# cvYouTian/Dedark-YOLO

Hardware: AMD Instinct MI355X
Metric: training img/s at 640x640 (higher is better)
Workload: dtype bf16

## Files before the change

dedark_yolo_amd/_C.py:

```python
import ctypes as C
import os

_HERE = os.path.dirname(os.path.abspath(__file__))
LIB_PATH = os.path.join(os.environ.get("DY_LIB_DIR") or os.path.join(_HERE, "lib"), "libdedark_yolo.so")

DY_F32, DY_BF16, DY_F16 = 0, 1, 2
ACT_NONE, ACT_SILU, ACT_LEAKY = 0, 1, 2
OPT_RULES = dict(Adam=0, Adamax=1, NAdam=2, RAdam=3, RMSProp=4)
STATS_REPLICAS = 64
BN_BWD_REPLICAS = 8

vp, i32, i64, f32, f64 = C.c_void_p, C.c_int, C.c_int64, C.c_float, C.c_double


class ConvDesc(C.Structure):
    _fields_ = [("src", vp), ("src_ld", i64), ("N", i32), ("Hs", i32), ("Ws", i32), ("Cs", i32), ("w", vp), ("dst", vp),
                ("dst_ld", i64), ("Hd", i32), ("Wd", i32), ("Cd", i32), ("KH", i32), ("KW", i32), ("stride", i32),
                ("pad", i32), ("dil", i32), ("scale", vp), ("shift", vp), ("act", i32), ("stats", vp), ("accumulate", i32),
                ("dtype", i32), ("dst_row_stride", i64), ("dst_img_stride", i64), ("KHf", i32), ("KWf", i32), ("kh0", i32),
                ("kh_step", i32), ("kw0", i32), ("kw_step", i32), ("dst_valid_channels", i32), ("dst_planar", vp),
                ("add_src", vp), ("add_src_ld", i64)]


class PackItem(C.Structure):
    _fields_ = [("w", vp), ("packed", vp), ("Cout", i32), ("Cout_pad", i32), ("Cin", i32), ("Cin_pad", i32), ("KH", i32),
                ("KW", i32), ("transposed", i32), ("dtype", i32), ("first_block", i64)]


class DetMaps(C.Structure):
    _fields_ = [("map", vp * 3), ("map_ld", i64 * 3), ("h", i32 * 3), ("w", i32 * 3), ("stride", f32 * 3), ("B", i32),
                ("nc", i32), ("n_levels", i32), ("dtype", i32)]


class DetMaps4(DetMaps):
    _fields_ = [("map3", vp), ("map_ld3", i64), ("h3", i32), ("w3", i32), ("stride3", f32)]


class AugSample(C.Structure):
    _fields_ = [("src", vp * 4), ("sh", i32 * 4), ("sw", i32 * 4), ("pitch", i64 * 4), ("rect", (i32 * 6) * 4), ("n_src", i32),
                ("canvas_h", i32), ("canvas_w", i32), ("hsv", i32), ("flipud", i32), ("fliplr", i32), ("minv", C.c_double * 6),
                ("lut", (C.c_uint8 * 256) * 3)]


class AugMixSample(C.Structure):
    _fields_ = [("a", AugSample), ("b", AugSample), ("r", C.c_double), ("r1", C.c_double), ("mix", i32)]


class SegDesc(C.Structure):
    _fields_ = [("mc", vp), ("mc_ld", i64), ("proto", vp), ("proto_ld", i64), ("B", i32), ("A", i32), ("nm", i32), ("mh", i32),
                ("mw", i32), ("target_gt_idx", vp), ("fg_mask", vp), ("target_box", vp), ("masks", vp), ("mask_dtype", i32),
                ("mask_h", i32), ("mask_w", i32), ("overlap", i32), ("gt_rows", vp), ("n_max", i32), ("img_h", f32), ("img_w", f32),
                ("pos", vp), ("npos", vp), ("dtype", i32)]


BIAS_GRAD_CHUNKS = 2048
LN_MAX_C = 2048
LN_MAX_PARTS = 512

POSE_MAX_LEVELS = 4


class PoseDesc(C.Structure):
    _fields_ = [("kpt", vp * POSE_MAX_LEVELS), ("kpt_ld", i64 * POSE_MAX_LEVELS), ("h", i32 * POSE_MAX_LEVELS), ("w", i32 * POSE_MAX_LEVELS),
                ("stride", f32 * POSE_MAX_LEVELS), ("n_levels", i32), ("B", i32), ("A", i32), ("K", i32), ("ndim", i32), ("dtype", i32),
                ("target_gt_idx", vp), ("fg_mask", vp), ("target_box", vp), ("keypoints", vp), ("n_targets", i32), ("gt_rows", vp),
                ("n_max", i32), ("img_h", f32), ("img_w", f32), ("sigma", vp), ("pos", vp), ("npos", vp)]


_SIGS = {
    "dy_version": [],
    "dy_frontend_init": [],
    "dy_conv2d_fwd": [C.POINTER(ConvDesc), vp],
    "dy_conv2d_dgrad": [C.POINTER(ConvDesc), vp],
    "dy_conv2d_wgrad": [vp, i64, i32, i32, i32, i32, vp, i64, i32, i32, i32, i32, i32, i32, i32, i32, i32, i32, vp, i64, vp,
                        i32, vp],
    "dy_conv2d_wgrad_forked": [vp, vp, i64, i32, i32, i32, i32, vp, i64, i32, i32, i32, i32, i32, i32, i32, i32, i32, i32, vp, i64,
                               vp, i32, vp],
    "dy_conv2d_bn_act_fwd": [C.POINTER(ConvDesc), i64, vp, vp, vp, vp, f32, f32, vp, i32, vp, i64, vp, i64, vp],
    "dy_bn_act_bwd": [vp, i64, vp, i64, vp, vp, i32, vp, vp, i64, vp, vp, i64, i32, i32, vp],
    "dy_conv2d_bn_act_fwd_valid": [C.POINTER(ConvDesc), i64, vp, vp, vp, vp, f32, f32, vp, i32, vp, i64, vp, i64, i32, vp],
    "dy_bn_act_bwd_valid": [vp, i64, vp, i64, vp, vp, i32, vp, vp, i64, vp, vp, i64, i32, i32, i32, vp],
    "dy_pack_weight": [vp, vp, i32, i32, i32, i32, i32, i32, i32, i32, vp],
    "dy_pack_item_blocks": [i32, i32, i32, i32],
    "dy_pack_weights_multi": [vp, i32, i64, vp],
    "dy_bn_finalize": [vp, i64, vp, vp, vp, vp, f32, f32, vp, vp, vp, vp, i32, vp],
    "dy_bn_fold_eval": [vp, vp, vp, vp, f32, vp, vp, i32, vp],
    "dy_bn_finalize_valid": [vp, i64, vp, vp, vp, vp, f32, f32, vp, vp, vp, vp, i32, i32, vp],
    "dy_bn_fold_eval_valid": [vp, vp, vp, vp, f32, vp, vp, i32, i32, vp],
    "dy_bn_act_fwd": [vp, i64, vp, vp, i32, vp, i64, vp, i64, i64, i32, i32, vp],
    "dy_bn_act_bwd_reduce": [vp, i64, vp, i64, vp, vp, vp, vp, i32, i32, vp, i64, i32, i32, vp],
    "dy_bn_act_bwd_apply": [vp, i64, vp, i64, vp, vp, vp, vp, vp, i32, i32, vp, vp, i64, vp, vp, i64, i32, i32, vp],
    "dy_bn_act_bwd_apply_valid": [vp, i64, vp, i64, vp, vp, vp, vp, vp, i32, i32, vp, vp, i64, vp, vp, i64, i32, i32, i32, vp],
    "dy_bn2_act_fwd": [vp, i64, vp, i64, vp, vp, vp, vp, i32, vp, i64, i64, i32, i32, vp],
    "dy_bn2_act_bwd_workspace": [i64, i32, i32],
    "dy_bn2_act_bwd": [vp, i64, vp, i64, vp, i64, vp, vp, vp, vp, vp, vp, vp, vp, vp, vp, i32, vp, i64, vp, i64, vp, vp, vp, vp, vp, i64,
                       i64, i32, i32, vp],
    "dy_maxpool_fwd": [vp, i64, vp, i64, vp, i32, i32, i32, i32, i32, i32, i32, i32, i32, i32, vp],
    "dy_maxpool_bwd": [vp, i64, vp, vp, i64, i32, i32, i32, i32, i32, i32, i32, i32, i32, i32, i32, vp],
    "dy_upsample_nearest_fwd": [vp, i64, vp, i64, i32, i32, i32, i32, i32, i32, vp],
    "dy_upsample_nearest_bwd": [vp, i64, vp, i64, i32, i32, i32, i32, i32, i32, i32, vp],
    "dy_copy2d": [vp, i64, vp, i64, i64, i32, i32, i32, vp],
    "dy_cast": [vp, i32, vp, i32, i64, vp],
    "dy_pconv_pack": [vp, vp, i32, i32, i32, vp],
    "dy_pconv_fwd": [vp, i64, vp, i64, vp, vp, i32, i32, i32, i32, i32, i32, vp],
    "dy_pconv_dgrad": [vp, i64, vp, i64, vp, vp, i32, i32, i32, i32, i32, i32, vp, i64, i32, vp],
    "dy_pconv_wgrad": [vp, i64, vp, i64, vp, i32, i32, i32, i32, vp, i64, i32, vp],
    "dy_dwconv_fwd": [vp, i64, vp, i64, vp, i32, i32, i32, i32, i32, i32, vp, vp, i32, vp, i32, i32, vp],
    "dy_dwconv_dgrad": [vp, i64, vp, i64, vp, i32, i32, i32, i32, i32, i32, i32, vp, i64, i32, vp],
    "dy_dwconv_wgrad": [vp, i64, vp, i64, vp, i32, i32, i32, i32, i32, i32, vp, i64, i32, vp],
    "dy_copy2d_exact": [vp, i64, vp, i64, i64, i32, i32, i32, vp],
    "dy_asff_fuse_fwd": [vp, i64, vp, i64, vp, i64, vp, i64, vp, i64, i64, i32, i32, vp],
    "dy_asff_fuse_bwd": [vp, i64, vp, i64, vp, i64, vp, i64, vp, i64, vp, i64, vp, i64, vp, i64, vp, i64, i64, i32, i32, i32,
                         i32, i32, vp],
    "dy_image_to_nhwc8": [vp, i32, i32, i32, vp, i32, i32, i32, vp],
    "dy_resize_bwd": [vp, i32, i32, i32, i32, i32, i32, vp, vp],
    "dy_filter_params_fwd": [vp, i32, vp, i32, vp],
    "dy_filter_params_bwd": [vp, i32, vp, vp, i32, vp],
    "dy_filters_pointwise_fwd": [vp, vp, vp, vp, vp, i32, i32, i32, i32, vp],
    "dy_filters_pointwise_bwd": [vp, vp, vp, vp, vp, vp, vp, i32, i32, i32, i32, i32, vp],
    "dy_usm_fwd": [vp, vp, vp, vp, vp, i32, i32, i32, i32, vp],
    "dy_usm_bwd": [vp, vp, i32, vp, vp, vp, vp, i32, i32, i32, i32, vp],
    "dy_loss_prepare_targets": [vp, vp, vp, i32, i32, i32, f32, f32, vp, vp, vp],
    "dy_loss_decode": [C.POINTER(DetMaps), vp, vp],
    "dy_tal_assign": [C.POINTER(DetMaps), vp, vp, vp, i32, vp, vp, vp, vp, vp, vp, vp, vp, vp],
    "dy_tal_assign_decoded": [vp, vp, vp, vp, vp, i32, i32, i32, i32, vp, vp, vp, vp, vp, vp, vp, vp, vp],
    "dy_chan_moments": [vp, i64, i32, i64, i32, vp, i32, vp],
    "dy_sru_fwd": [vp, i64, vp, i64, i32, i64, i32, i32, vp, vp, vp, f32, i32, vp],
    "dy_sru_bwd": [vp, i64, vp, i64, vp, i64, i32, i64, i32, i32, vp, vp, vp, f32, vp, i32, vp],
    "dy_cru_fuse_fwd": [vp, i64, vp, i64, i32, i64, i32, vp, i32, vp],
    "dy_cru_fuse_bwd": [vp, i64, vp, i64, vp, i64, i32, i64, i32, vp, vp, i32, vp],
    "dy_cru_conv_pack": [vp, vp, vp, i32, i32, i32, i32, i32, i32, vp],
    "dy_cru_conv_fwd": [vp, i64, vp, vp, vp, i64, i32, i32, i32, i32, i32, i32, i32, i32, vp],
    "dy_cru_conv_dgrad": [vp, i64, vp, vp, i64, i32, i32, i32, i32, i32, i32, i32, i32, i32, vp],
    "dy_cru_conv_wgrad": [vp, i64, vp, i64, vp, vp, vp, i32, i32, i32, i32, i32, i32, i32, vp, i64, i32, vp],
    "dy_attn_fwd": [vp, i64, vp, i64, vp, i64, vp, i64, vp, i32, i32, i32, i32, f32, i32, vp],
    "dy_attn_bwd": [vp, i64, vp, i64, vp, i64, vp, i64, vp, i64, vp, vp, i64, vp, i64, vp, i64, i32, i32, i32, i32, f32, i32, vp],
    "dy_add_layernorm_fwd": [vp, i64, vp, i64, vp, vp, vp, i64, vp, i64, i32, f32, i32, vp],
    "dy_add_layernorm_bwd": [vp, i64, vp, i64, vp, vp, vp, i64, vp, i64, i32, vp, vp, vp, i64, i64, i32, i32, vp],
    "dy_gelu_fwd": [vp, i64, vp, i64, i64, i32, i32, vp],
    "dy_gelu_bwd": [vp, i64, vp, i64, vp, i64, i64, i32, i32, vp],
    "dy_add_pos": [vp, i64, vp, vp, i64, i32, i32, i32, i32, vp],
    "dy_bbox_ciou": [vp, vp, i64, vp, vp, vp],
    "dy_bbox_iou": [vp, vp, i64, i32, i32, f32, vp, vp, vp],
    "dy_aug_resize_u8": [vp, i32, i32, i64, vp, i32, i32, i64, vp],
    "dy_aug_resize_area_u8": [vp, i32, i32, i64, vp, i32, i32, i64, vp],
    "dy_aug_letterbox": [vp, i32, i32, i64, i32, i32, i32, i32, i32, i32, vp, vp],
    "dy_aug_mosaic_warp": [vp, i32, i32, i32, vp, vp],
    "dy_aug_mosaic_warp_mix": [vp, i32, i32, i32, vp, vp],
    "dy_dark_channel_prior": [vp, i32, i32, i32, vp, vp, vp],
    "dy_dfl_loss": [vp, vp, i64, vp, vp, vp],
    "dy_loss_fwd": [C.POINTER(DetMaps), vp, vp, vp, vp, vp, vp, vp],
    "dy_loss_finish": [vp, vp, f32, f32, f32, f32, i32, vp, vp, vp],
    "dy_loss_bwd": [C.POINTER(DetMaps), C.POINTER(vp), C.POINTER(i64), vp, vp, vp, vp, vp, vp, vp, f32, f32, f32, vp],
    "dy_detect_decode": [C.POINTER(DetMaps), vp, vp],
    "dy_detect_decode_rows": [C.POINTER(DetMaps), vp, i32, vp],
    "dy_detect_decode_tta": [C.POINTER(DetMaps), vp, i64, i32, i32, i32, f32, i32, f32, f32, vp],
    "dy_tta_scale_img": [vp, i32, i32, i32, i32, i32, i32, i32, i32, i32, vp, vp],
    "dy_nms_candidates": [vp, i32, i32, i32, f32, i32, vp, vp, i64, vp],
    "dy_nms_sort": [vp, vp, vp, i32, i64, vp, vp, vp],
    "dy_nms_greedy": [vp, vp, vp, i32, i32, i32, i64, C.c_double, i32, i32, f32, i32, vp, vp, vp, vp, vp, vp],
    "dy_preprocess_batch": [vp, vp, vp, f32, i32, i32, vp, i64, vp],
    "dy_sumsq": [vp, i64, vp, vp],
    "dy_sgd_step": [vp, vp, vp, vp, vp, f32, f32, f32, f32, f32, f32, f32, i32, f32, vp, f32, f32, i64, vp],
    "dy_sgd_step_scaled": [vp, vp, vp, vp, vp, f32, f32, f32, f32, f32, f32, f32, i32, f32, vp, f32, f32, vp, i64, vp],
    "dy_adamw_step_scaled": [vp, vp, vp, vp, vp, vp, f32, f32, f32, f32, f32, f32, f32, f32, f32, i32, f32, vp, f32, f32, vp, i64, vp],
    "dy_loss_scale_update": [vp, vp, f32, f32, i32, vp],
    "dy_optim_step": [i32, vp, vp, vp, vp, vp, vp, f32, f32, f32, f32, f32, f32, f64, f64, f64, f64, f32, vp, f32, f32, vp, vp, i64, vp],
    "dy_adamw_step": [vp, vp, vp, vp, vp, vp, f32, f32, f32, f32, f32, f32, f32, f32, f32, i32, f32, vp, f32, f32, i64, vp],
    "dy_ema_lerp": [vp, vp, f32, i64, vp],
    "dy_grad_accumulate": [vp, vp, i64, vp],
    "dy_stream_fork": [vp, vp],
    "dy_seg_positives": [vp, i32, i32, vp, vp, vp],
    "dy_seg_gt_rows": [vp, i32, i32, i32, vp, vp],
    "dy_seg_loss_fwd": [C.POINTER(SegDesc), f32, vp, vp, vp, vp],
    "dy_seg_loss_bwd": [C.POINTER(SegDesc), vp, f32, vp, i64, vp, i64, vp],
    "dy_bias_add": [vp, i64, vp, i64, i32, i32, vp],
    "dy_bias_grad": [vp, i64, i64, i32, i32, vp, i64, vp, vp],
    "dy_seg_mask_decode": [vp, i64, i32, i32, i32, vp, i64, vp, i32, f32, f32, i32, vp, vp],
    "dy_seg_crop_mask": [vp, vp, i32, i32, i32, vp],
    "dy_seg_mask_iou": [vp, i32, vp, i32, i32, i32, i64, vp, vp, vp],
    "dy_seg_mask_upsample": [vp, i64, i32, i32, i32, i32, vp, i64, vp, vp, i32, i32, i32, i32, f32, f32, i32, i32, i32, i32, i32, i32, i32,
                             vp, vp],
    "dy_mask_resize": [vp, i32, i32, i32, i32, i32, i32, i32, i32, vp, i32, i32, i32, vp],
    "dy_pose_loss_fwd": [C.POINTER(PoseDesc), f32, f32, vp, vp, vp, vp],
    "dy_pose_loss_bwd": [C.POINTER(PoseDesc), vp, vp, f32, f32, C.POINTER(vp), i64, vp],
    "dy_pose_kpt_decode": [C.POINTER(PoseDesc), i32, vp, vp],
    "dy_kpt_oks": [vp, i32, vp, i32, i32, vp, vp, i32, f32, vp, vp],
    "dy_polymask_raster": [vp, i32, i32, i32, i32, i32, vp, vp, vp],
    "dy_polymask_compose": [vp, vp, vp, i32, i32, i32, i32, vp, vp, vp, vp, vp],
    "dy_gap_fwd": [vp, i64, i32, i32, i32, i32, vp, i64, vp],
    "dy_gap_bwd": [vp, i64, i32, i32, i32, i32, vp, i64, vp],
    "dy_cls_xent_fwd": [vp, i64, i32, vp, i32, i32, vp, vp, vp],
    "dy_cls_xent_bwd": [vp, i64, i32, vp, vp, vp, i32, i32, vp, i64, vp],
    "dy_cls_softmax": [vp, i64, i32, i32, i32, vp, vp],
    "dy_cls_topk": [vp, i64, i32, i32, i32, i32, vp, vp],
    "dy_cls_metrics_update": [vp, i32, vp, i32, i32, vp, vp, vp],
    "dy_val_box_match": [vp, i32, vp, i32, i32, vp, vp, vp, i32, i32, i32, vp, vp, i32, i32, f32, f32, i32, vp, vp, vp, vp, vp, vp],
    "dy_val_iou_match": [vp, i64, vp, vp, i32, vp, i32, i32, vp, vp, i32, vp, i32, i32, vp, vp, vp],
}

_lib = None


def lib():
    global _lib
    if _lib is None:
        if not os.path.exists(LIB_PATH):
            raise RuntimeError(f"dedark_yolo_amd: HIP library not built: {LIB_PATH} (run __graft_entry__.build()); "
                               "there is no CPU fallback")
        L = C.CDLL(LIB_PATH)
        L.dy_last_error.restype = C.c_char_p
        L.dy_last_error.argtypes = []
        L.dy_last_kernel.restype = C.c_char_p
        L.dy_last_kernel.argtypes = []
        L.dy_clear_last_kernel.restype = None
        L.dy_clear_last_kernel.argtypes = []
        for name, sig in _SIGS.items():
            fn = getattr(L, name)
            fn.argtypes = sig
            fn.restype = C.c_int64 if name in ("dy_pack_item_blocks", "dy_bn2_act_bwd_workspace") else C.c_int
        _lib = L
    return _lib


def exported_symbols():
    return ["dy_last_error", "dy_last_kernel", "dy_clear_last_kernel"] + list(_SIGS)


_prof = None
_next_meta = None
_UNTIMED = frozenset(["dy_stream_fork"])


def call(name, *args):
    global _next_meta
    L = lib()
    if _prof is None or name in _UNTIMED:
        rc = getattr(L, name)(*args)
    else:
        import torch
        e0, e1 = torch.cuda.Event(enable_timing=True), torch.cuda.Event(enable_timing=True)
        L.dy_clear_last_kernel()
        e0.record()
        rc = getattr(L, name)(*args)
        e1.record()
        kern = L.dy_last_kernel().decode()
        _prof.append((name, e0, e1, _next_meta, kern))
        _next_meta = None
    if rc != 0:
        raise RuntimeError(f"{name} failed (rc={rc}): {L.dy_last_error().decode()}")


def set_meta(**kw):
    global _next_meta
    if _prof is not None:
        _next_meta = kw
```

dedark_yolo_amd/csrc/conv.hip:

```cpp
#include <stdlib.h>
#include "dy_host.h"
#include "conv_epilogue.h"
#include "../../include/dedark_yolo.h"
#include "conv_route.h"

namespace {

constexpr int ROWB = 144;
constexpr int NTHREADS = 256;

struct ConvP {
  const char* src;
  long src_ld;
  int N, Hs, Ws, Cs;
  const char* w;
  char* dst;
  long dst_ld;
  int Hd, Wd, Cd;
  int KH, KW, stride, pad, dil;
  const float* scale;
  const float* shift;
  int act;
  double* stats;
  int accumulate;
// ... 696 lines not shown
    if (!it.transposed) {
      const int co = co0 + a, ci = ci0 + g * VE;
#pragma unroll
      for (int e = 0; e < 8; ++e) v[e] = e < VE ? tile[a][(g * VE + e) * PACK_TAPS + t] : 0.f;
      ok = co < it.Cout_pad && ci < it.Cin_pad;
      o = ((long)co * T + t0 + t) * it.Cin_pad + ci;
    } else {
      const int ci = ci0 + a, co = co0 + g * VE;
#pragma unroll
      for (int e = 0; e < 8; ++e) v[e] = e < VE ? tile[g * VE + e][a * PACK_TAPS + t] : 0.f;
      ok = co < it.Cout_pad && ci < it.Cin_pad;
      o = ((long)ci * T + t0 + t) * it.Cout_pad + co;
    }
    if (!ok) continue;
    if (it.dtype == DY_F32) stvec<float>((float*)it.packed + o, v);
    else if (it.dtype == DY_F16) stvec<f16_t>((f16_t*)it.packed + o, v);
    else stvec<bf16_t>((bf16_t*)it.packed + o, v);
  }
  __syncthreads();
}

__global__ __launch_bounds__(256) void pack_multi_kernel(const dy_pack_item* __restrict__ items, int n_items) {
  __shared__ float tile[PACK_TILE][PACK_TILE * PACK_TAPS + 1];
  __shared__ long fb[1024];
  const long b = blockIdx.x;
  const bool cached = n_items <= 1024;
  if (cached) {
    for (int i = threadIdx.x; i < n_items; i += 256) fb[i] = items[i].first_block;
    __syncthreads();
  }
  int lo = 0, hi = n_items - 1;
  while (lo < hi) {
    const int mid = (lo + hi + 1) >> 1;
    if ((cached ? fb[mid] : items[mid].first_block) <= b) lo = mid; else hi = mid - 1;
  }
  const dy_pack_item it = items[lo];
  const int tiles_ci = (it.Cin_pad + PACK_TILE - 1) / PACK_TILE;
  const int tb = (int)(b - it.first_block);
  const int co0 = (tb / tiles_ci) * PACK_TILE, ci0 = (tb % tiles_ci) * PACK_TILE;
  const int T = it.KH * it.KW;
  if (T == 9) pack_chunk<9>(it, tile, co0, ci0, 9, 0, 9);
  else if (T == 1) pack_chunk<1>(it, tile, co0, ci0, 1, 0, 1);
  else
    for (int t0 = 0; t0 < T; t0 += PACK_TAPS) pack_chunk<0>(it, tile, co0, ci0, T, t0, T - t0 < PACK_TAPS ? T - t0 : PACK_TAPS);
}

template <typename T, int MODE>
int launch_conv(const dy_conv_desc* d, hipStream_t st, const dy_conv_desc* classes, int ncls) {
  ConvP p;
  dy_route::fill_parity_classes(p, classes, ncls);
  dy_route::fill_gather(p, d);
  constexpr int BM = 128;
  const int tiles_m = dy_cdiv(p.M, BM);
  auto blocks = [&](int bn) {
    p.tiles_n = dy_cdiv(d->Cd, bn);
    p.nblk = tiles_m * p.tiles_n;
    if (p.ncls > 1) p.nblk = dy_route::number_parity_blocks(p, BM, dy_route::CLS_SEQUENTIAL);
  };
  dy_note_kernel(d->Cd <= 32 ? "conv_igemm_kernel<BN=32>" : (d->Cd <= 64 ? "conv_igemm_kernel<BN=64>" : "conv_igemm_kernel<BN=128>"));
  if (d->Cd <= 32) {
    blocks(32);
    conv_igemm_kernel<T, BM, 32, 4, 1, MODE><<<p.nblk, NTHREADS, 0, st>>>(p);
  } else if (d->Cd <= 64) {
    blocks(64);
    conv_igemm_kernel<T, BM, 64, 2, 2, MODE><<<p.nblk, NTHREADS, 0, st>>>(p);
  } else {
    blocks(128);
    conv_igemm_kernel<T, BM, 128, 2, 2, MODE><<<p.nblk, NTHREADS, 0, st>>>(p);
  }
  DY_LAUNCH_CHECK();
  return 0;
}

bool thin_eligible(const dy_conv_desc* d, int mode, bool parity_class = false) {
  static const bool off = dy_env("DY_NO_CONV_THIN") != nullptr;
  static const bool all_shapes = getenv("DY_CONV_THIN_ALL") != nullptr;
  if (off || d->dtype != DY_BF16) return false;
  if (!all_shapes && !parity_class && !(d->Cs == 16 && d->KH * d->KW > 1)) return false;
  if (!(d->Cs == 16 || d->Cs == 32 || d->Cs == 48) || d->Cd > 32 || d->Cd % 8 != 0) return false;
  if (d->KH > 3 || d->KW > 3 || d->dil != 1 || (mode == 1 && d->stride != 1)) return false;
  if ((d->src_ld * 2) % 16 != 0 || (d->dst_ld * 2) % 16 != 0 || (long)d->N * d->Hd * d->Wd < 1024) return false;
  return true;
}

int launch_thin(const dy_conv_desc* d, int mode, hipStream_t st, const dy_conv_desc* classes = nullptr, int ncls = 0) {
  ConvP p;
  dy_route::fill_parity_classes(p, classes, ncls);
  dy_route::fill_gather(p, d);
  p.tiles_n = 1;
  p.nblk = dy_cdiv(p.M, THIN_BM);
  if (p.ncls > 1) p.nblk = dy_route::number_parity_blocks(p, THIN_BM, dy_route::CLS_SEQUENTIAL);
  dy_note_kernel("conv_thin_kernel");
#define THIN(C_, M_) conv_thin_kernel<C_, M_><<<p.nblk, NTHREADS, 0, st>>>(p)
  const int c16 = d->Cs / 16;
  if (mode == 0) { if (c16 == 1) THIN(1, 0); else if (c16 == 2) THIN(2, 0); else THIN(3, 0); }
  else { if (c16 == 1) THIN(1, 1); else if (c16 == 2) THIN(2, 1); else THIN(3, 1); }
#undef THIN
  DY_LAUNCH_CHECK();
  return 0;
}

int launch_generic(const dy_conv_desc* d, int mode, hipStream_t st, const dy_conv_desc* classes = nullptr, int ncls = 0) {
  if (mode == 0)
    return d->dtype == DY_F32 ? launch_conv<float, 0>(d, st, classes, ncls)
                              : (d->dtype == DY_F16 ? launch_conv<f16_t, 0>(d, st, classes, ncls) : launch_conv<bf16_t, 0>(d, st, classes, ncls));
  return d->dtype == DY_F32 ? launch_conv<float, 1>(d, st, classes, ncls)
                            : (d->dtype == DY_F16 ? launch_conv<f16_t, 1>(d, st, classes, ncls) : launch_conv<bf16_t, 1>(d, st, classes, ncls));
}

int check_conv(const dy_conv_desc* d, const char* who) {
  DY_CHECK(d && d->src && d->w && (d->dst || d->dst_planar), "%s: null pointer", who);
  DY_CHECK(d->dtype == DY_F32 || d->dtype == DY_BF16 || d->dtype == DY_F16, "%s: bad dtype %d", who, d->dtype);
  const int ve = d->dtype == DY_F32 ? 4 : 8, es = d->dtype == DY_F32 ? 4 : 2;
  DY_CHECK(d->Cs > 0 && d->Cs % ve == 0, "%s: Cs=%d must be a positive multiple of %d", who, d->Cs, ve);
  DY_CHECK(d->src_ld >= d->Cs && (d->src_ld * es) % 16 == 0, "%s: src_ld=%ld not 16-byte aligned", who, (long)d->src_ld);
  DY_CHECK(((uintptr_t)d->src) % 16 == 0 && ((uintptr_t)d->w) % 16 == 0, "%s: src/w pointer not 16-byte aligned", who);
  DY_CHECK(d->dst_ld >= d->Cd && d->Cd > 0, "%s: dst_ld=%ld < Cd=%d", who, (long)d->dst_ld, d->Cd);
  DY_CHECK(d->N > 0 && d->Hs > 0 && d->Ws > 0 && d->Hd > 0 && d->Wd > 0, "%s: empty geometry", who);
  DY_CHECK(d->KH > 0 && d->KW > 0 && d->stride > 0 && d->dil > 0 && d->pad >= 0, "%s: bad window", who);
  DY_CHECK(d->act >= 0 && d->act <= 2, "%s: bad act", who);
  return 0;
}

enum : unsigned {
  SITE_FWD = 1,
  SITE_DGRAD_HEAD = 2,
  SITE_DGRAD = 4,
  SITE_CLASS = 8,
};

struct Route {
  bool (*eligible)(const dy_conv_desc* d, int mode);
  int (*launch)(const dy_conv_desc* d, int mode, void* stream);
  unsigned sites;
  bool fuses_add;
};

const Route kRoutes[] = {
    {dy_dense_fwd_eligible, dy_dense_fwd_launch, SITE_FWD, false},
    {dy_conv_stem_fwd_eligible, dy_conv_stem_fwd_launch, SITE_FWD, false},
    {dy_dense_dgrad_eligible, dy_dense_dgrad_launch, SITE_DGRAD_HEAD, false},
    {dy_conv_small_dgrad_eligible, dy_conv_small_dgrad_launch, SITE_DGRAD_HEAD, false},
    {dy_conv_px_eligible, dy_conv_px_launch, SITE_FWD | SITE_DGRAD, true},
    {dy_conv_v4_eligible, dy_conv_v4_launch, SITE_FWD | SITE_DGRAD | SITE_CLASS, true},
    {dy_conv_v5_eligible, dy_conv_v5_launch, SITE_FWD | SITE_DGRAD | SITE_CLASS, true},
    {dy_conv_v3_eligible, dy_conv_v3_launch, SITE_FWD | SITE_DGRAD, false},
    {dy_conv_v2_eligible, dy_conv_v2_launch, SITE_FWD | SITE_DGRAD | SITE_CLASS, false},
    {[](const dy_conv_desc* d, int mode) { return thin_eligible(d, mode); },
     [](const dy_conv_desc* d, int mode, void* stream) { return launch_thin(d, mode, (hipStream_t)stream); }, SITE_FWD | SITE_DGRAD, false},
    {[](const dy_conv_desc*, int) { return true; },
     [](const dy_conv_desc* d, int mode, void* stream) { return launch_generic(d, mode, (hipStream_t)stream); },
     SITE_FWD | SITE_DGRAD | SITE_CLASS, false},
};

const Route* pick_route(const dy_conv_desc* d, unsigned site) {
  const int mode = (site & (SITE_DGRAD_HEAD | SITE_DGRAD)) ? 1 : 0;
  for (const Route& r : kRoutes)
    if ((r.sites & site) && r.eligible(d, mode)) return &r;
  return nullptr;
}

}

extern "C" int dy_conv2d_fwd(const dy_conv_desc* d, void* stream) {
  if (int e = check_conv(d, "dy_conv2d_fwd")) return e;
  const int ho = (d->Hs + 2 * d->pad - d->dil * (d->KH - 1) - 1) / d->stride + 1;
  const int wo = (d->Ws + 2 * d->pad - d->dil * (d->KW - 1) - 1) / d->stride + 1;
  DY_CHECK(ho == d->Hd && wo == d->Wd, "dy_conv2d_fwd: dst %dx%d does not match conv output %dx%d", d->Hd, d->Wd, ho, wo);
  return pick_route(d, SITE_FWD)->launch(d, 0, stream);
}

static int dgrad_dispatch(const dy_conv_desc* d, void* stream, bool* added) {
  if (int e = check_conv(d, "dy_conv2d_dgrad")) return e;
  const int ho = (d->Hd + 2 * d->pad - d->dil * (d->KH - 1) - 1) / d->stride + 1;
  const int wo = (d->Wd + 2 * d->pad - d->dil * (d->KW - 1) - 1) / d->stride + 1;
  DY_CHECK(ho == d->Hs && wo == d->Ws, "dy_conv2d_dgrad: dz %dx%d does not match conv output %dx%d", d->Hs, d->Ws, ho, wo);
  DY_CHECK(d->stats == nullptr, "dy_conv2d_dgrad: stats unsupported");
  DY_CHECK(d->KHf == 0 && d->dst_row_stride == 0, "dy_conv2d_dgrad: tap subsets / strided destinations are forward-only");
  if (const Route* r = pick_route(d, SITE_DGRAD_HEAD)) return r->launch(d, 1, stream);
  DY_CHECK(d->dst_planar == nullptr, "dy_conv2d_dgrad: dst_planar is only supported by the direct stem kernel (bf16, 3x3 s2 p1, Cd == 8)");
  static const bool no_parity = dy_env("DY_NO_PARITY_DGRAD") != nullptr;
  if (d->stride == 2 && d->dil == 1 && !no_parity) {
    dy_conv_desc c[4];
    int nc = 0;
    bool ok = true;
    for (int ph = 0; ph < 2 && ok; ++ph)
      for (int pw = 0; pw < 2 && ok; ++pw) {
        int geo[2][4];
        for (int ax = 0; ax < 2; ++ax) {
          const int par = ax == 0 ? ph : pw, K = ax == 0 ? d->KH : d->KW, ext = ax == 0 ? d->Hd : d->Wd;
          const int first = (par + d->pad) & 1;
          const int n = first < K ? (K - 1 - first) / 2 + 1 : 0;
          const int last = first + 2 * (n - 1);
          const int omin = (par + d->pad - last) / 2;
          geo[ax][0] = n; geo[ax][1] = last; geo[ax][2] = -omin; geo[ax][3] = (ext - par + 1) / 2;
        }
        if (geo[0][3] <= 0 || geo[1][3] <= 0) continue;
        if (geo[0][0] == 0 || geo[1][0] == 0 || geo[0][2] != geo[1][2] || geo[0][2] < 0) { ok = false; break; }
        dy_conv_desc& q = c[nc++];
        q = *d;
        const long es = d->dtype == DY_F32 ? 4 : 2;
        q.dst = (char*)d->dst + ((long)ph * d->Wd + pw) * d->dst_ld * es;
        q.dst_ld = 2 * d->dst_ld;
        q.dst_row_stride = 2L * d->Wd * d->dst_ld;
        q.dst_img_stride = (long)d->Hd * d->Wd * d->dst_ld;
        q.Hd = geo[0][3]; q.Wd = geo[1][3];
        q.KHf = d->KH; q.KWf = d->KW;
        q.KH = geo[0][0]; q.KW = geo[1][0];
        q.kh0 = geo[0][1]; q.kh_step = -2; q.kw0 = geo[1][1]; q.kw_step = -2;
        q.stride = 1; q.pad = geo[0][2];
      }
    if (ok) {
      static const bool multi = !(dy_env("DY_PARITY_MULTI") && atoi(dy_env("DY_PARITY_MULTI")) == 0);
      if (multi && nc > 1) {
        dy_conv_desc r[4];
        bool all_v2 = true, none_v2 = true;
        for (int i = 0; i < nc; ++i) {
          r[i] = c[nc - 1 - i];
          const bool e2 = dy_conv_v2_eligible(&r[i], 0);
          all_v2 = all_v2 && e2;
          none_v2 = none_v2 && !e2;
        }
        const long class_tiles = dy_cdiv((long)r[0].N * r[0].Hd * r[0].Wd, 256);
        if (dy_conv_v4_classes_eligible(r, nc)) return dy_conv_v4_launch_classes(r, nc, stream);
        if (dy_conv_v5_classes_eligible(r, nc)) return dy_conv_v5_launch_classes(r, nc, stream);
        if (all_v2 && class_tiles <= 256) return dy_conv_v2_launch_classes(r, nc, stream);
        if (none_v2) {
          bool thin = true;
          for (int i = 0; i < nc; ++i) thin = thin && thin_eligible(&r[i], 0, true);
          if (thin) return launch_thin(&r[0], 0, (hipStream_t)stream, r, nc);
          if (class_tiles <= 256) return launch_generic(&r[0], 0, (hipStream_t)stream, r, nc);
        }
      }
      for (int i = nc - 1; i >= 0; --i) {
        if (int e = pick_route(&c[i], SITE_CLASS)->launch(&c[i], 0, stream)) return e;
      }
      return 0;
    }
  }
  const Route* r = pick_route(d, SITE_DGRAD);
  *added = r->fuses_add;
  return r->launch(d, 1, stream);
}

extern "C" int dy_conv2d_dgrad(const dy_conv_desc* d, void* stream) {
  bool added = false;
  if (int e = dgrad_dispatch(d, stream, &added)) return e;
  if (d->add_src && !added) {
    DY_CHECK(d->dst && d->dst_planar == nullptr, "dy_conv2d_dgrad: add_src needs an NHWC destination");
    return dy_copy2d(d->add_src, d->add_src_ld, d->dst, d->dst_ld, (int64_t)d->N * d->Hd * d->Wd, d->Cd, 1, d->dtype, stream);
  }
  return 0;
}

namespace {
template <typename T>
int launch_wgrad(const DyWgradArgs& a, hipStream_t st) {
  WgP p;
  dy_route::fill_wgrad_problem(p, a);
  constexpr int MK = 8 * DT<T>::VE;
  int bm, bn;
  bn = p.Ktot <= 32 ? 32 : (p.Ktot <= 64 ? 64 : 128);
  if (bn == 32) bm = 128;
  else if (bn == 64) bm = p.Cout <= 64 ? 64 : 128;
  else bm = p.Cout <= 32 ? 32 : (p.Cout <= 64 ? 64 : 128);
  const int tiles_c = dy_cdiv(p.Cout, bm);
  p.tiles_k = dy_cdiv(p.Ktot, bn);
  const int tiles = tiles_c * p.tiles_k;
  p.tiles = tiles;
  static const int env_blocks = dy_env("DY_WGRAD_BLOCKS") ? atoi(dy_env("DY_WGRAD_BLOCKS")) : 0;
  static const int env_steps = dy_env("DY_WGRAD_STEPS") ? atoi(dy_env("DY_WGRAD_STEPS")) : 0;
  const long fit = a.scratch_elems / ((long)tiles * bm * bn);
  DY_CHECK(fit >= 1, "dy_conv2d_wgrad: scratch too small (%ld floats, need %ld)", a.scratch_elems, (long)tiles * bm * bn);
  const long want = ((env_blocks > 0 ? env_blocks : 2048) + tiles - 1) / tiles;
  const dy_route::WgradSplits plan =
      dy_route::plan_wgrad_splits(p.M, want, (long)(env_steps > 0 ? env_steps : 4) * MK, MK, fit, dy_route::kGridDimYCap);
  p.chunk = plan.chunk;
  dim3 grid(tiles, (unsigned)plan.splits);
  dy_note_kernel("conv_wgrad_kernel+wgrad_reduce_kernel");
#define WG(BM_, BN_, WM_, WN_) conv_wgrad_kernel<T, BM_, BN_, WM_, WN_><<<grid, NTHREADS, 0, st>>>(p)
  if (bm == 128 && bn == 128) WG(128, 128, 2, 2);
  else if (bm == 64 && bn == 128) WG(64, 128, 1, 4);
  else if (bm == 32 && bn == 128) WG(32, 128, 1, 4);
  else if (bm == 128 && bn == 64) WG(128, 64, 4, 1);
  else if (bm == 64 && bn == 64) WG(64, 64, 2, 2);
  else WG(128, 32, 4, 1);
#undef WG
  DY_LAUNCH_CHECK();
  wgrad_reduce_kernel<<<dim3(a.Cout, dy_cdiv(p.Ktot, 32)), 256, 0, st>>>(a.scratch, (int)plan.splits, tiles, p.tiles_k, bm, bn, a.Cin, p.Cin,
                                                                         p.KH, p.KW, p.Ktot, a.g_oihw);
  DY_LAUNCH_CHECK();
  return 0;
}

int wgrad_generic(const DyWgradArgs& a, void* stream) {
  int rc = 0;
  DY_DISPATCH_DTYPE("dy_conv2d_wgrad", a.dtype, rc = launch_wgrad<T>(a, (hipStream_t)stream));
  return rc;
}

struct WgradRoute {
  bool (*eligible)(const DyWgradArgs& a);
  int (*launch)(const DyWgradArgs& a, void* stream);
};

const WgradRoute kWgradRoutes[] = {
    {dy_dense_wgrad_eligible, dy_dense_wgrad_launch},
    {dy_wgrad_v3_eligible, dy_wgrad_v3_launch},
    {dy_wgrad_v4_eligible, dy_wgrad_v4_launch},
    {dy_wgrad_v2_eligible, dy_wgrad_v2_launch},
    {[](const DyWgradArgs&) { return true; }, wgrad_generic},
};
}

int dy_wgrad_reduce_co_slabs(const float* part, int splits, const DyCoSlabs& L, int Cout, int Cin, float* g_oihw, void* stream) {
  wgrad_reduce_co_kernel<<<dim3(dy_cdiv(Cout, 32), L.KH * L.KW * L.Cin_pad), 256, 0, (hipStream_t)stream>>>(
      part, splits, L.co_tile, L.k_tile, L.Cin_pad, L.KH, L.KW, Cout, Cin, L.co_stride, L.k_stride, L.split_stride, g_oihw);
  DY_LAUNCH_CHECK();
  return 0;
}

extern "C" int dy_conv2d_wgrad(const void* x, int64_t x_ld, int N, int Hi, int Wi, int Cin_pad, const void* dz, int64_t dz_ld,
                               int Ho, int Wo, int Cout_pad, int KH, int KW, int stride, int pad, int dil, int Cout, int Cin,
                               float* scratch, int64_t scratch_elems, float* g_oihw, int dtype, void* stream) {
  DY_CHECK(x && dz && scratch && g_oihw, "dy_conv2d_wgrad: null pointer");
  DY_CHECK(dtype == DY_F32 || dtype == DY_BF16 || dtype == DY_F16, "dy_conv2d_wgrad: bad dtype");
  const int ve = dtype == DY_F32 ? 4 : 8, es = dtype == DY_F32 ? 4 : 2;
  DY_CHECK(Cin_pad % ve == 0 && Cout_pad % ve == 0, "dy_conv2d_wgrad: Cin=%d / Cout=%d must be multiples of %d", Cin_pad, Cout_pad, ve);
  DY_CHECK(Cout > 0 && Cout <= Cout_pad && Cin > 0 && Cin <= Cin_pad, "dy_conv2d_wgrad: bad real channel counts");
  DY_CHECK((x_ld * es) % 16 == 0 && (dz_ld * es) % 16 == 0, "dy_conv2d_wgrad: ld not 16-byte aligned");
  DY_CHECK(((uintptr_t)x) % 16 == 0 && ((uintptr_t)dz) % 16 == 0, "dy_conv2d_wgrad: pointer not 16-byte aligned");
  const int ho = (Hi + 2 * pad - dil * (KH - 1) - 1) / stride + 1, wo = (Wi + 2 * pad - dil * (KW - 1) - 1) / stride + 1;
  DY_CHECK(ho == Ho && wo == Wo, "dy_conv2d_wgrad: dz %dx%d does not match conv output %dx%d", Ho, Wo, ho, wo);
  const DyWgradArgs a = {x, x_ld, N, Hi, Wi, Cin_pad, dz, dz_ld, Ho, Wo, Cout_pad, KH, KW, stride, pad, dil, Cout, Cin,
                         scratch, scratch_elems, g_oihw, dtype};
  for (const WgradRoute& r : kWgradRoutes)
    if (r.eligible(a)) return r.launch(a, stream);
  return 0;
}

extern "C" int dy_pack_weight(const float* w, void* packed, int Cout, int Cout_pad, int Cin, int Cin_pad, int KH, int KW,
                              int transposed, int dtype, void* stream) {
  DY_CHECK(w && packed && Cin_pad >= Cin && Cout_pad >= Cout, "dy_pack_weight: bad args");
  long total = (long)Cout_pad * KH * KW * Cin_pad;
  int blocks = (int)((total + 255) / 256);
  if (blocks > 4096) blocks = 4096;
  hipStream_t st = (hipStream_t)stream;
  DY_DISPATCH_DTYPE("dy_pack_weight", dtype,
                    pack_weight_kernel<T><<<blocks, 256, 0, st>>>(w, (T*)packed, Cout, Cout_pad, Cin, Cin_pad, KH, KW, transposed));
  DY_LAUNCH_CHECK();
  return 0;
}

extern "C" int64_t dy_pack_item_blocks(int Cout_pad, int Cin_pad, int KH, int KW) {
  (void)KH; (void)KW;
  return (int64_t)((Cout_pad + PACK_TILE - 1) / PACK_TILE) * ((Cin_pad + PACK_TILE - 1) / PACK_TILE);
}

extern "C" int dy_pack_weights_multi(const dy_pack_item* items_dev, int n_items, int64_t n_blocks, void* stream) {
  DY_CHECK(items_dev && n_items > 0 && n_blocks > 0 && n_blocks < (1LL << 31), "dy_pack_weights_multi: bad args");
  pack_multi_kernel<<<(unsigned)n_blocks, 256, 0, (hipStream_t)stream>>>(items_dev, n_items);
  DY_LAUNCH_CHECK();
  return 0;
}

extern "C" int dy_conv2d_bn_act_fwd_valid(const dy_conv_desc* d, int64_t count, const float* gamma, const float* beta,
                                          float* running_mean, float* running_var, float momentum, float eps, float* aff, int act,
                                          const void* residual, int64_t res_ld, void* y, int64_t y_ld, int C_valid, void* stream) {
  DY_CHECK(d && d->stats && d->dst && aff, "dy_conv2d_bn_act_fwd: needs a raw-output buffer, statistics and the affine buffer");
  DY_CHECK(C_valid > 0 && C_valid <= d->Cd, "dy_conv2d_bn_act_fwd: C_valid=%d outside 1..Cd=%d", C_valid, d->Cd);
  if (int e = dy_conv2d_fwd(d, stream)) return e;
  const int C = d->Cd;
  if (int e = dy_bn_finalize_valid(d->stats, count, gamma, beta, running_mean, running_var, momentum, eps, aff, aff + C, aff + 2 * C,
                                   aff + 3 * C, C, C_valid, stream))
    return e;
  return dy_bn_act_fwd(d->dst, d->dst_ld, aff, aff + C, act, residual, res_ld, y, y_ld, (int64_t)d->N * d->Hd * d->Wd, C, d->dtype, stream);
}

extern "C" int dy_conv2d_bn_act_fwd(const dy_conv_desc* d, int64_t count, const float* gamma, const float* beta, float* running_mean,
                                    float* running_var, float momentum, float eps, float* aff, int act, const void* residual,
                                    int64_t res_ld, void* y, int64_t y_ld, void* stream) {
  DY_CHECK(d, "dy_conv2d_bn_act_fwd: null descriptor");
  return dy_conv2d_bn_act_fwd_valid(d, count, gamma, beta, running_mean, running_var, momentum, eps, aff, act, residual, res_ld, y, y_ld,
                                    d->Cd, stream);
}

extern "C" int dy_conv2d_wgrad_forked(void* wait_for, const void* x, int64_t x_ld, int N, int Hi, int Wi, int Cin_pad, const void* dz,
                                      int64_t dz_ld, int Ho, int Wo, int Cout_pad, int KH, int KW, int stride, int pad, int dil,
                                      int Cout, int Cin, float* scratch, int64_t scratch_elems, float* g_oihw, int dtype,
                                      void* stream) {
  if (wait_for != stream)
    if (int e = dy_stream_fork(wait_for, stream)) return e;
  return dy_conv2d_wgrad(x, x_ld, N, Hi, Wi, Cin_pad, dz, dz_ld, Ho, Wo, Cout_pad, KH, KW, stride, pad, dil, Cout, Cin, scratch,
                         scratch_elems, g_oihw, dtype, stream);
}
```

dedark_yolo_amd/csrc/conv_route.h:

```cpp
#pragma once
#include <type_traits>
#include <utility>
#include "dy_common.h"
#include "../../include/dedark_yolo.h"

namespace dy_route {

__device__ inline int xcd_remap(int bid, int nblk) {
  int q = nblk >> 3, r = nblk & 7, x = bid & 7;
  int base = (x < r) ? x * (q + 1) : r * (q + 1) + (x - r) * q;
  return base + (bid >> 3);
}

template <typename P>
__device__ inline long dst_offset(const P& p, long m) {
  if (p.dst_row == 0) return m * p.dst_ld;
  const long HWd = (long)p.Hd * p.Wd;
  const long img = m / HWd;
  const int rem = (int)(m - img * HWd);
  const int oh = rem / p.Wd, ow = rem - oh * p.Wd;
  return img * p.dst_img + (long)oh * p.dst_row + (long)ow * p.dst_ld;
}

template <typename P>
inline void fill_weight_taps(P& p, const dy_conv_desc* d) {
  if (d->KHf > 0) {
    p.kh0 = d->kh0; p.khs = d->kh_step; p.kw0 = d->kw0; p.kws = d->kw_step; p.KWf = d->KWf;
    p.w_row = (long)d->KHf * d->KWf * d->Cs;
  } else {
    p.kh0 = 0; p.khs = 1; p.kw0 = 0; p.kws = 1; p.KWf = d->KW;
    p.w_row = (long)d->KH * d->KW * d->Cs;
  }
}

template <typename P>
inline void fill_dst_strides(P& p, const dy_conv_desc* d) {
  p.dst_row = d->dst_row_stride;
  p.dst_img = d->dst_img_stride ? d->dst_img_stride : (long)d->Hd * d->dst_row_stride;
}

template <typename P>
inline void fill_gather(P& p, const dy_conv_desc* d) {
  p.src = (const char*)d->src; p.src_ld = d->src_ld; p.N = d->N; p.Hs = d->Hs; p.Ws = d->Ws; p.Cs = d->Cs;
  p.w = (const char*)d->w; p.dst = (char*)d->dst; p.dst_ld = d->dst_ld; p.Hd = d->Hd; p.Wd = d->Wd; p.Cd = d->Cd;
  p.KH = d->KH; p.KW = d->KW; p.stride = d->stride; p.pad = d->pad; p.dil = d->dil;
  p.scale = d->scale; p.shift = d->shift; p.act = d->act; p.stats = d->stats; p.accumulate = d->accumulate;
  p.M = (long)d->N * d->Hd * d->Wd;
  p.Ktot = d->KH * d->KW * d->Cs;
  static const int ablate = dy_env("DY_ABLATE") ? atoi(dy_env("DY_ABLATE")) : 0;
  p.ablate = ablate;
  fill_dst_strides(p, d);
  fill_weight_taps(p, d);
}

template <typename P>
inline void fill_taps_extents(P& p, const dy_conv_desc* d, int mode) {
  p.src = (const char*)d->src; p.w = (const char*)d->w; p.dst = (char*)d->dst;
  p.src_ld = d->src_ld; p.dst_ld = d->dst_ld;
  p.src_bytes = (unsigned)((((long)d->N * d->Hs * d->Ws - 1) * d->src_ld + d->Cs) * 2);
  p.Hs = d->Hs; p.Ws = d->Ws; p.Cs = d->Cs; p.Hd = d->Hd; p.Wd = d->Wd; p.Cd = d->Cd;
  p.KH = d->KH; p.KW = d->KW;
  if (mode == 0) {
    p.stride = d->stride; p.dh0 = -d->pad; p.dhs = d->dil; p.dw0 = -d->pad; p.dws = d->dil;
  } else {
    p.stride = 1; p.dh0 = d->pad; p.dhs = -d->dil; p.dw0 = d->pad; p.dws = -d->dil;
  }
  fill_weight_taps(p, d);
  p.w_bytes = (unsigned)((long)d->Cd * p.w_row * 2);
  {
    const int dh_lo = p.dhs < 0 ? p.dh0 + p.dhs * (p.KH - 1) : p.dh0, dw_lo = p.dws < 0 ? p.dw0 + p.dws * (p.KW - 1) : p.dw0;
    const long lo = ((long)dh_lo * p.Ws + dw_lo) * p.src_ld * 2;
    p.a_min = lo < 0 ? (int)lo : 0;
  }
  p.scale = d->scale; p.shift = d->shift; p.act = d->act; p.stats = d->stats; p.accumulate = d->accumulate;
  if ((long)d->N * d->Hd * d->Wd * d->Cd * 2 > (128L << 20)) p.accumulate |= 2;
  p.M = (long)d->N * d->Hd * d->Wd;
  p.add_src = mode == 1 ? (const char*)d->add_src : nullptr; p.add_src_ld = d->add_src_ld;
  fill_dst_strides(p, d);
}

template <typename P>
inline void fill_parity_classes(P& p, const dy_conv_desc* classes, int ncls) {
  p.ncls = ncls > 1 ? ncls : 0;
  for (int c = 0; c < p.ncls; ++c) {
    const dy_conv_desc& q = classes[c];
    DyParityCls& k = p.cls[c];
    k.dst = (char*)q.dst; k.M = (long)q.N * q.Hd * q.Wd; k.Hd = q.Hd; k.Wd = q.Wd; k.KH = q.KH; k.KW = q.KW; k.pad = q.pad;
    k.kh0 = q.kh0; k.kw0 = q.kw0; k.Ktot = q.KH * q.KW * q.Cs; k.blk0 = 0; k._r = 0;
  }
}

enum ClsOrder { CLS_SEQUENTIAL, CLS_XCD_SLOTS };
template <typename P>
inline int number_parity_blocks(P& p, int bm, ClsOrder order) {
  int next = 0;
  for (int c = 0; c < p.ncls; ++c) {
    DyParityCls& k = p.cls[c];
    const int tiles = dy_cdiv(k.M, bm) * p.tiles_n;
    k.blk0 = next;
    k._r = order == CLS_XCD_SLOTS ? dy_cdiv(tiles, 8) : 0;
    next += order == CLS_XCD_SLOTS ? k._r : tiles;
  }
  return order == CLS_XCD_SLOTS ? 8 * next : next;
}

inline bool dma_extents_ok(const dy_conv_desc* d, int KH, int KW, int dil) {
  const long src_bytes = (((long)d->N * d->Hs * d->Ws - 1) * d->src_ld + d->Cs) * 2;
  const long w_row = d->KHf > 0 ? (long)d->KHf * d->KWf * d->Cs : (long)d->KH * d->KW * d->Cs;
  const long w_bytes = (long)d->Cd * w_row * 2;
  const long halo = ((long)KH * dil * d->Ws + (long)KW * dil) * d->src_ld * 2;
  return src_bytes + halo <= 0x7fffffffL && w_bytes <= 0x3fffffffL;
}

inline bool parity_classes_uniform(const dy_conv_desc* c, int ncls) {
  const dy_conv_desc* d = &c[0];
  for (int i = 0; i < ncls; ++i) {
    const dy_conv_desc& q = c[i];
    if (q.src != d->src || q.w != d->w || q.Cs != d->Cs || q.Cd != d->Cd || q.dtype != d->dtype || q.stride != 1 || q.dil != 1 || q.KHf != d->KHf ||
        q.KWf != d->KWf || q.kh_step != d->kh_step || q.kw_step != d->kw_step || q.dst_ld != d->dst_ld || q.dst_row_stride != d->dst_row_stride ||
        q.dst_img_stride != d->dst_img_stride || q.src_ld != d->src_ld || q.accumulate != d->accumulate || q.scale || q.shift || q.stats ||
        q.act != DY_ACT_NONE)
      return false;
    if ((q.dst_ld * 2) % 16 != 0 || ((uintptr_t)q.dst) % 16 != 0 || (q.src_ld * 2) % 16 != 0) return false;
  }
  return true;
}

}

bool dy_dense_fwd_eligible(const dy_conv_desc* d, int mode);
int dy_dense_fwd_launch(const dy_conv_desc* d, int mode, void* stream);
bool dy_dense_dgrad_eligible(const dy_conv_desc* d, int mode);
int dy_dense_dgrad_launch(const dy_conv_desc* d, int mode, void* stream);
bool dy_conv_stem_fwd_eligible(const dy_conv_desc* d, int mode);
int dy_conv_stem_fwd_launch(const dy_conv_desc* d, int mode, void* stream);
bool dy_conv_small_dgrad_eligible(const dy_conv_desc* d, int mode);
int dy_conv_small_dgrad_launch(const dy_conv_desc* d, int mode, void* stream);
bool dy_conv_px_eligible(const dy_conv_desc* d, int mode);
int dy_conv_px_launch(const dy_conv_desc* d, int mode, void* stream);
bool dy_conv_v4_eligible(const dy_conv_desc* d, int mode);
int dy_conv_v4_launch(const dy_conv_desc* d, int mode, void* stream);
bool dy_conv_v4_classes_eligible(const dy_conv_desc* classes, int ncls);
int dy_conv_v4_launch_classes(const dy_conv_desc* classes, int ncls, void* stream);
bool dy_conv_v5_eligible(const dy_conv_desc* d, int mode);
int dy_conv_v5_launch(const dy_conv_desc* d, int mode, void* stream);
bool dy_conv_v5_classes_eligible(const dy_conv_desc* classes, int ncls);
int dy_conv_v5_launch_classes(const dy_conv_desc* classes, int ncls, void* stream);
bool dy_conv_v3_eligible(const dy_conv_desc* d, int mode);
int dy_conv_v3_launch(const dy_conv_desc* d, int mode, void* stream);
bool dy_conv_v2_eligible(const dy_conv_desc* d, int mode);
int dy_conv_v2_launch(const dy_conv_desc* d, int mode, void* stream);
int dy_conv_v2_launch_classes(const dy_conv_desc* classes, int ncls, void* stream);
bool dy_conv_prefers_256(const dy_conv_desc* d);

struct DyWgradArgs {
  const void* x;
  long x_ld;
  int N, Hi, Wi, Cin_pad;
  const void* dz;
  long dz_ld;
  int Ho, Wo, Cout_pad, KH, KW, stride, pad, dil, Cout, Cin;
  float* scratch;
  long scratch_elems;
  float* g_oihw;
  int dtype;
};

namespace dy_route {

template <typename P, typename = void> struct HasPointwise : std::false_type {};
template <typename P> struct HasPointwise<P, std::void_t<decltype(std::declval<P&>().pointwise)>> : std::true_type {};

template <typename P>
inline void fill_wgrad_problem(P& p, const DyWgradArgs& a) {
  p.x = (const char*)a.x; p.x_ld = a.x_ld; p.N = a.N; p.Hi = a.Hi; p.Wi = a.Wi; p.Cin = a.Cin_pad;
  p.dz = (const char*)a.dz; p.dz_ld = a.dz_ld; p.Ho = a.Ho; p.Wo = a.Wo; p.Cout = a.Cout_pad;
  p.KH = a.KH; p.KW = a.KW; p.stride = a.stride; p.pad = a.pad; p.dil = a.dil; p.part = a.scratch;
  p.M = (long)a.N * a.Ho * a.Wo;
  p.Ktot = a.KH * a.KW * a.Cin_pad;
  if constexpr (HasPointwise<P>::value) p.pointwise = (a.KH == 1 && a.KW == 1 && a.stride == 1 && a.pad == 0) ? 1 : 0;
}

struct WgradSplits {
  long splits, chunk;
};
constexpr long kGridDimYCap = 65535, kNoGridCap = 1L << 40;
inline WgradSplits plan_wgrad_splits(long M, long want, long min_pixels, long step, long fit, long grid_cap) {
  const long max_splits = (M + min_pixels - 1) / min_pixels;
  long splits = want < max_splits ? want : max_splits;
  if (splits > fit) splits = fit;
  if (splits < 1) splits = 1;
  if (splits > grid_cap) splits = grid_cap;
  long chunk = (M + splits - 1) / splits;
  chunk = (chunk + step - 1) / step * step;
  return {(M + chunk - 1) / chunk, chunk};
}

}

struct DyCoSlabs {
  int co_tile;
  long co_stride;
  int k_tile;
  long k_stride;
  long split_stride;
  int Cin_pad, KH, KW;
};
int dy_wgrad_reduce_co_slabs(const float* part, int splits, const DyCoSlabs& L, int Cout, int Cin, float* g_oihw, void* stream);

bool dy_dense_wgrad_eligible(const DyWgradArgs& a);
int dy_dense_wgrad_launch(const DyWgradArgs& a, void* stream);
bool dy_wgrad_v3_eligible(const DyWgradArgs& a);
int dy_wgrad_v3_launch(const DyWgradArgs& a, void* stream);
bool dy_wgrad_v4_eligible(const DyWgradArgs& a);
int dy_wgrad_v4_launch(const DyWgradArgs& a, void* stream);
bool dy_wgrad_v2_eligible(const DyWgradArgs& a);
int dy_wgrad_v2_launch(const DyWgradArgs& a, void* stream);
```

dedark_yolo_amd/csrc/wgrad_v4.hip:

```cpp
#include <stdlib.h>
#include <type_traits>
#include "dy_host.h"
#include "../../include/dedark_yolo.h"
#include "conv_route.h"

namespace wg4 {

constexpr int BP = 256, BQ = 256, BKP = 64;
constexpr int UNIT = 64 * 256;
constexpr int OFF_A0 = 0, OFF_A1 = UNIT, OFF_B0 = 2 * UNIT, OFF_B1 = 3 * UNIT, BUF = 4 * UNIT;
constexpr unsigned A_OOB = 0x80000000u;
constexpr unsigned B_COL_OOB = 0x40000000u;

typedef __attribute__((address_space(3))) void* lds_ptr_t;
typedef __attribute__((ext_vector_type(4))) short s16x4;
typedef __attribute__((ext_vector_type(8))) short s16x8;
typedef __attribute__((address_space(3))) s16x4* lds_s16x4_ptr;
typedef __attribute__((ext_vector_type(8))) __bf16 bf16x8;

struct P {
  const char* x;
  const char* dz;
  unsigned x_bytes, dz_bytes;
  long x_ld, dz_ld;
  int N, Hi, Wi, Cin;
  int Ho, Wo, Cout;
  int KH, KW, stride, pad, dil;
  float* part;
  long M;
  int Ktot, tiles_q, tiles, nblk;
  long chunk;
  int q64_w, r64_w;
  int q_h, r_h;
};

using dy_route::xcd_remap;

template <bool POINTWISE, typename T = bf16_t>
__global__ __launch_bounds__(512) void wgrad_kernel(const P p) {
  extern __shared__ __attribute__((aligned(16))) char smem[];
  const int tid = threadIdx.x, lane = tid & 63;
  const int wave = __builtin_amdgcn_readfirstlane(tid >> 6);
  const int wr = wave >> 2, wc = wave & 3;
  const int bid = xcd_remap(blockIdx.x, p.nblk);
  const int split = bid / p.tiles, tile = bid - split * p.tiles;
  const int tile_p = tile / p.tiles_q, tile_q = tile - tile_p * p.tiles_q;
  const int kp0 = tile_p * BP, q0 = tile_q * BQ;
  const bool has_b1 = q0 + 128 < p.Cout;
  const bool has_a1 = kp0 + 128 < p.Ktot;
  const long m_begin = (long)split * p.chunk;
  const long m_end = (m_begin + p.chunk < p.M) ? m_begin + p.chunk : p.M;
  const int nk = m_begin < m_end ? (int)((m_end - m_begin + BKP - 1) / BKP) : 0;

  unsigned nrec_a = nk > 0 ? p.x_bytes : 0, nrec_b = nk > 0 ? p.dz_bytes : 0;

  const int lrow = lane >> 4, slot = lane & 15;
  const int chunk = slot ^ ((lrow << 2) | (wave & 3));
  int a_dh[2], a_dw[2];
  unsigned a_tap[2];
#pragma unroll
  for (int u = 0; u < 2; ++u) {
    const int k = kp0 + 128 * u + 8 * chunk;
    const bool kok = k < p.Ktot;
    const int kk = kok ? k : 0;
    const int tap = kk / p.Cin, ci = kk - tap * p.Cin;
    const int kh = tap / p.KW, kw = tap - kh * p.KW;
    a_dh[u] = kh * p.dil - p.pad;
    a_dw[u] = kw * p.dil - p.pad;
    a_tap[u] = (unsigned)(((long)a_dh[u] * p.Wi + a_dw[u]) * p.x_ld * 2 + ci * 2);
    if (!kok) a_dh[u] = 0x40000000;
  }
  int ph[2], pw[2];
  unsigned a_pix[2];
#pragma unroll
  for (int j = 0; j < 2; ++j) {
    const long m = m_begin + 4 * (wave + 8 * j) + lrow;
    if (POINTWISE) {
      a_pix[j] = (unsigned)(m * p.x_ld * 2);
      ph[j] = pw[j] = 0;
    } else {
      const unsigned mu = (unsigned)m;
      const unsigned HWo = (unsigned)(p.Ho * p.Wo);
      const int pn = (int)(mu / HWo);
      const unsigned rem = mu - (unsigned)pn * HWo;
      const int oh = (int)(rem / (unsigned)p.Wo), ow = (int)(rem - (unsigned)oh * (unsigned)p.Wo);
      ph[j] = oh * p.stride;
      pw[j] = ow * p.stride;
      a_pix[j] = (unsigned)((((long)pn * p.Hi + ph[j]) * p.Wi + pw[j]) * p.x_ld * 2);
    }
  }
  unsigned b_off[2][2];
#pragma unroll
  for (int u = 0; u < 2; ++u) {
    const int co = q0 + 128 * u + 8 * chunk;
#pragma unroll
    for (int j = 0; j < 2; ++j)
      b_off[u][j] = co < p.Cout ? (unsigned)((long)(4 * (wave + 8 * j) + lrow) * p.dz_ld * 2 + co * 2) : B_COL_OOB;
  }
  int b_koff = nk > 0 ? (int)(m_begin * p.dz_ld * 2) : 0;
  if (nk > 0) nrec_b -= (unsigned)b_koff;
  int sk = 0;
  auto advance_scalar = [&]() {
    ++sk;
    b_koff += (int)(BKP * p.dz_ld * 2);
    const unsigned step = (unsigned)(BKP * p.dz_ld * 2);
    nrec_b = nrec_b > step ? nrec_b - step : 0;
    if (sk >= nk) { nrec_a = 0; nrec_b = 0; b_koff = 0; }
  };
  const int e_w = p.stride * (int)p.x_ld * 2, e_h = p.stride * p.Wi * (int)p.x_ld * 2, e_n = p.Hi * p.Wi * (int)p.x_ld * 2;
  const int d_base = p.q_h * e_n + p.r_h * e_h + p.r64_w * e_w, d_cw = e_h - p.Wo * e_w, d_ch = e_n - p.Ho * e_h;
  const int s_rw = p.r64_w * p.stride, s_rh = p.r_h * p.stride, s_Wo = p.Wo * p.stride, s_Ho = p.Ho * p.stride;
  auto advance_rows = [&]() {
    if (POINTWISE) {
#pragma unroll
      for (int j = 0; j < 2; ++j) a_pix[j] += (unsigned)(BKP * p.x_ld * 2);
      return;
    }
#pragma unroll
    for (int j = 0; j < 2; ++j) {
      int w = pw[j] + s_rw, h = ph[j] + s_rh;
      const bool cw = w >= s_Wo;
      w -= cw ? s_Wo : 0;
      h += cw ? p.stride : 0;
      int d = d_base + (cw ? d_cw : 0);
      const bool c1 = h >= s_Ho;
      h -= c1 ? s_Ho : 0;
      d += c1 ? d_ch : 0;
      const bool c2 = h >= s_Ho;
      h -= c2 ? s_Ho : 0;
      d += c2 ? d_ch : 0;
      pw[j] = w; ph[j] = h;
      a_pix[j] += (unsigned)d;
    }
  };
  unsigned a_v[2][2];
  auto offsets_of = [&](int u) {
#pragma unroll
    for (int j = 0; j < 2; ++j) {
      bool ok = a_dh[u] < 0x40000000;
      if (!POINTWISE) {
        const int ih = ph[j] + a_dh[u], iw = pw[j] + a_dw[u];
        ok = ((unsigned)ih < (unsigned)p.Hi) & ((unsigned)iw < (unsigned)p.Wi);
      }
      a_v[u][j] = ok ? a_pix[j] + a_tap[u] : A_OOB;
    }
  };
  auto stage_a = [&](int buf, int u) {
    const __amdgpu_buffer_rsrc_t rs = __builtin_amdgcn_make_buffer_rsrc((void*)p.x, 0, nrec_a, 0x00020000);
#pragma unroll
    for (int j = 0; j < 2; ++j)
      __builtin_amdgcn_raw_ptr_buffer_load_lds(rs, (lds_ptr_t)(smem + buf * BUF + (u ? OFF_A1 : OFF_A0) + (wave + 8 * j) * 1024), 16,
                                               (int)a_v[u][j], 0, 0, 0);
  };
  auto stage_b = [&](int buf, int u) {
    const __amdgpu_buffer_rsrc_t rs = __builtin_amdgcn_make_buffer_rsrc((void*)(p.dz + b_koff), 0, nrec_b, 0x00020000);
#pragma unroll
    for (int j = 0; j < 2; ++j)
      __builtin_amdgcn_raw_ptr_buffer_load_lds(rs, (lds_ptr_t)(smem + buf * BUF + (u ? OFF_B1 : OFF_B0) + (wave + 8 * j) * 1024), 16,
                                               (int)b_off[u][j], 0, 0, 0);
  };

  const int gg = lane >> 4, tq = (lane & 15) >> 2, tp = lane & 3;
  int a_adr[2][4], b_adr[2][2];
#pragma unroll
  for (int t = 0; t < 2; ++t) {
    const int row = 8 * gg + 4 * t + tq;
    const int key = (tq << 2) | ((2 * gg + t) & 3);
    const int base = row * 256 + 8 * (tp & 1);
#pragma unroll
    for (int i = 0; i < 4; ++i) a_adr[t][i] = base + 16 * ((2 * (4 * wr + i) + (tp >> 1)) ^ key);
#pragma unroll
    for (int j = 0; j < 2; ++j) b_adr[t][j] = base + 16 * ((2 * (2 * wc + j) + (tp >> 1)) ^ key);
  }

  f32x4 acc[2][2][4][2];
#pragma unroll
  for (int a = 0; a < 2; ++a)
#pragma unroll
    for (int b = 0; b < 2; ++b)
#pragma unroll
      for (int i = 0; i < 4; ++i)
#pragma unroll
        for (int j = 0; j < 2; ++j) acc[a][b][i][j] = f32x4{0.f, 0.f, 0.f, 0.f};
  u32x4 afr[4][2], bfr[2][2][2];

  const unsigned lds0 = (unsigned)(uintptr_t)(lds_ptr_t)smem;
  unsigned a_vad[2][4], b_vad[2][2];
#pragma unroll
  for (int t = 0; t < 2; ++t) {
#pragma unroll
    for (int i = 0; i < 4; ++i) a_vad[t][i] = lds0 + (unsigned)a_adr[t][i];
#pragma unroll
    for (int j = 0; j < 2; ++j) b_vad[t][j] = lds0 + (unsigned)b_adr[t][j];
  }
#define WG4_TR(dst, vaddr, OFF) asm volatile("ds_read_b64_tr_b16 %0, %1 offset:%2" : "=v"(dst) : "v"(vaddr), "n"(OFF) : "memory")
#define WG4_FRAG(fr, vad0, vad1, OFF)                      \
  do {                                                      \
    uint2 lo_, hi_;                                         \
    WG4_TR(lo_, vad0, OFF);                                 \
    WG4_TR(hi_, vad1, OFF);                                 \
    fr = u32x4{lo_.x, lo_.y, hi_.x, hi_.y};                 \
  } while (0)
#define WG4_READ_A2(BASE, I0)                                                         \
  do {                                                                                \
    WG4_FRAG(afr[I0][0], a_vad[0][I0], a_vad[1][I0], (BASE));                          \
    WG4_FRAG(afr[I0][1], a_vad[0][I0], a_vad[1][I0], (BASE) + 8192);                   \
    WG4_FRAG(afr[I0 + 1][0], a_vad[0][I0 + 1], a_vad[1][I0 + 1], (BASE));              \
    WG4_FRAG(afr[I0 + 1][1], a_vad[0][I0 + 1], a_vad[1][I0 + 1], (BASE) + 8192);       \
  } while (0)
#define WG4_READ_B(BASE, U)                                                           \
  do {                                                                                \
    WG4_FRAG(bfr[U][0][0], b_vad[0][0], b_vad[1][0], (BASE));                          \
    WG4_FRAG(bfr[U][0][1], b_vad[0][0], b_vad[1][0], (BASE) + 8192);                   \
    WG4_FRAG(bfr[U][1][0], b_vad[0][1], b_vad[1][1], (BASE));                          \
    WG4_FRAG(bfr[U][1][1], b_vad[0][1], b_vad[1][1], (BASE) + 8192);                   \
  } while (0)
  auto mma = [&](int ah, int bh, auto livec, auto gapc, auto mid) {
    constexpr bool LIVE = decltype(livec)::value;
    constexpr int GAP = decltype(gapc)::value;
    asm volatile("s_waitcnt lgkmcnt(0)" ::: "memory");
    __builtin_amdgcn_sched_barrier(0);
    __builtin_amdgcn_s_setprio(1);
    if constexpr (LIVE) {
#pragma unroll
      for (int kb = 0; kb < 2; ++kb) {
#pragma unroll
        for (int i = 0; i < 4; ++i)
#pragma unroll
          for (int j = 0; j < 2; ++j)
            acc[ah][bh][i][j] = mfma_16x16x32<T>(afr[i][kb], bfr[bh][j][kb], acc[ah][bh][i][j]);
        if (kb == 0) mid();
      }
      if constexpr (GAP > 0) {
#pragma unroll
        for (int g = 0; g < 16; ++g) {
          __builtin_amdgcn_sched_group_barrier(0x008, 1, 0);
          __builtin_amdgcn_sched_group_barrier(0x002, GAP, 0);
        }
      }
    } else {
      mid();
    }
    __builtin_amdgcn_s_setprio(0);
    __builtin_amdgcn_sched_barrier(0);
  };
  auto pin_rows = [&]() {
#pragma unroll
    for (int j = 0; j < 2; ++j) asm volatile("" : "+v"(pw[j]), "+v"(ph[j]), "+v"(a_pix[j]));
  };
  auto pin_offsets = [&](int u) {
#pragma unroll
    for (int j = 0; j < 2; ++j) asm volatile("" : "+v"(a_v[u][j]));
  };

  offsets_of(0); offsets_of(1);
  stage_b(0, 0); stage_a(0, 0); stage_b(0, 1); stage_a(0, 1);
  advance_scalar();
  advance_rows();
  offsets_of(0); offsets_of(1);
  stage_b(1, 0); stage_a(1, 0); stage_b(1, 1);
  asm volatile("s_waitcnt vmcnt(6)" ::: "memory");
  __builtin_amdgcn_s_barrier();
  if (wr == 1) __builtin_amdgcn_s_barrier();

  int cur = 0;
  using yes = std::true_type;
  auto kloop = [&](auto a1c, auto b1c) {
  constexpr bool A1 = decltype(a1c)::value, B1 = decltype(b1c)::value;
  for (int kt = 0; kt < nk; ++kt) {
    const int b = cur, bo = cur ^ 1;
    WG4_READ_B(OFF_B0, 0);
    WG4_READ_A2(OFF_A0, 0);
    __builtin_amdgcn_sched_barrier(0);
    stage_a(bo, 1);
    __builtin_amdgcn_sched_barrier(0);
    asm volatile("s_waitcnt lgkmcnt(8)" ::: "memory");
    __builtin_amdgcn_sched_barrier(0);
    WG4_READ_A2(OFF_A0, 2);
    __builtin_amdgcn_sched_barrier(0);
    __builtin_amdgcn_s_barrier();
    mma(0, 0, yes{}, std::integral_constant<int, 0>{}, [&]() { advance_scalar(); });
    __builtin_amdgcn_s_barrier();
    if (B1) WG4_READ_B(OFF_B1, 1);
    __builtin_amdgcn_sched_barrier(0);
    stage_b(b, 0);
    __builtin_amdgcn_sched_barrier(0);
    __builtin_amdgcn_s_barrier();
    mma(0, 1, std::bool_constant<B1>{}, std::integral_constant<int, POINTWISE ? 1 : 3>{},
        [&]() { pin_rows(); advance_rows(); offsets_of(0); pin_rows(); pin_offsets(0); });
    __builtin_amdgcn_s_barrier();
    if (A1) {
      WG4_READ_A2(OFF_A1, 0);
      WG4_READ_A2(OFF_A1, 2);
    }
    __builtin_amdgcn_sched_barrier(0);
    stage_a(b, 0);
    __builtin_amdgcn_sched_barrier(0);
    __builtin_amdgcn_s_barrier();
    mma(1, 1, std::bool_constant<A1 && B1>{}, std::integral_constant<int, 1>{}, [&]() { pin_rows(); offsets_of(1); pin_offsets(1); });
    __builtin_amdgcn_s_barrier();
    stage_b(b, 1);
    __builtin_amdgcn_sched_barrier(0);
    asm volatile("s_waitcnt vmcnt(6)" ::: "memory");
    __builtin_amdgcn_s_barrier();
    {
      const int delta = cur ? -BUF : BUF;
      auto mid = [&]() {
#pragma unroll
        for (int t = 0; t < 2; ++t) {
#pragma unroll
          for (int i = 0; i < 4; ++i) { a_vad[t][i] += delta; asm volatile("" : "+v"(a_vad[t][i])); }
#pragma unroll
          for (int j = 0; j < 2; ++j) { b_vad[t][j] += delta; asm volatile("" : "+v"(b_vad[t][j])); }
        }
      };
      mma(1, 0, std::bool_constant<A1>{}, std::integral_constant<int, 1>{}, mid);
    }
    __builtin_amdgcn_s_barrier();
    cur ^= 1;
  }
  };
  if (has_a1) {
    if (has_b1) kloop(std::true_type{}, std::true_type{});
    else kloop(std::true_type{}, std::false_type{});
  } else {
    if (has_b1) kloop(std::false_type{}, std::true_type{});
    else kloop(std::false_type{}, std::false_type{});
  }
  if (wr == 0) __builtin_amdgcn_s_barrier();

  float* out = p.part + (long)bid * (BP * BQ);
  const int cl = lane & 15, g = lane >> 4;
#pragma unroll
  for (int bh = 0; bh < 2; ++bh)
#pragma unroll
    for (int j = 0; j < 2; ++j) {
      if (bh == 1 && !has_b1) continue;
      const int co = 128 * bh + 32 * wc + 16 * j + cl;
#pragma unroll
      for (int ah = 0; ah < 2; ++ah)
#pragma unroll
        for (int i = 0; i < 4; ++i) {
          if (ah == 1 && !has_a1) continue;
          const int k = 128 * ah + 64 * wr + 16 * i + 4 * g;
          *reinterpret_cast<f32x4*>(out + (long)co * BP + k) = acc[ah][bh][i][j];
        }
    }
}

__global__ __launch_bounds__(256) void reduce_kernel(const float* __restrict__ part, int splits, int tiles, int tiles_q, int Cout, int Cin,
                                                     int Cin_pad, int taps, float* __restrict__ g) {
  const int ci = blockIdx.x * 256 + threadIdx.x;
  const int co = blockIdx.y;
  const int t = blockIdx.z;
  if (ci >= Cin) return;
  const int tq = co / BQ, cq = co - tq * BQ;
  const long sstride = (long)tiles * BP * BQ;
  const int k = t * Cin_pad + ci;
  const float* src = part + ((long)((k / BP) * tiles_q + tq) * BQ + cq) * BP + (k % BP);
  float a0 = 0.f, a1 = 0.f, a2 = 0.f, a3 = 0.f;
  int s = 0;
  for (; s + 3 < splits; s += 4) {
    a0 += src[(long)s * sstride];
    a1 += src[(long)(s + 1) * sstride];
    a2 += src[(long)(s + 2) * sstride];
    a3 += src[(long)(s + 3) * sstride];
  }
  for (; s < splits; ++s) a0 += src[(long)s * sstride];
  g[((long)co * Cin + ci) * taps + t] = (a0 + a1) + (a2 + a3);
}

}

bool dy_wgrad_v4_eligible(const DyWgradArgs& a) {
  const long M = (long)a.N * a.Ho * a.Wo;
  static const bool off = dy_env("DY_NO_WGRAD_V4") != nullptr;
  if (off || (a.dtype != DY_BF16 && a.dtype != DY_F16)) return false;
  if (a.Cin_pad % 8 != 0 || a.Cout_pad % 8 != 0 || (a.x_ld * 2) % 16 != 0 || (a.dz_ld * 2) % 16 != 0) return false;
  const long Ktot = (long)a.KH * a.KW * a.Cin_pad;
  const long tq = (a.Cout_pad + 255) / 256, tp = (Ktot + 255) / 256;
  const bool tight = a.Cout_pad >= 192 && tq * 256 * 4 <= (long)a.Cout_pad * 5 && tp * 256 * 4 <= Ktot * 5;
  const bool long_loop = a.Cout_pad >= 64 && M >= 65536 && Ktot * a.Cout_pad * 4 >= tp * 256 * tq * 256;
  if (!(Ktot >= 192 && (tight || long_loop))) return false;
  if (M < 16384 || M >= (1L << 31)) return false;
  const long x_bytes = (((long)a.N * a.Hi * a.Wi - 1) * a.x_ld + a.Cin_pad) * 2, dz_bytes = ((M - 1) * a.dz_ld + a.Cout_pad) * 2;
  if (x_bytes > 0x7fffffffL || dz_bytes > 0x3fffffffL) return false;
  return a.scratch_elems >= tp * tq * 65536L * 2;
}

int dy_wgrad_v4_launch(const DyWgradArgs& a, void* stream) {
  using namespace wg4;
  P p;
  dy_route::fill_wgrad_problem(p, a);
  p.x_bytes = (unsigned)((((long)a.N * a.Hi * a.Wi - 1) * a.x_ld + a.Cin_pad) * 2);
  p.dz_bytes = (unsigned)(((p.M - 1) * a.dz_ld + a.Cout_pad) * 2);
  p.tiles_q = dy_cdiv(a.Cout_pad, BQ);
  p.tiles = dy_cdiv(p.Ktot, BP) * p.tiles_q;
  const long fit = a.scratch_elems / ((long)p.tiles * BP * BQ);
  const dy_route::WgradSplits plan = dy_route::plan_wgrad_splits(p.M, 256 / p.tiles, 8L * BKP, BKP, fit, dy_route::kNoGridCap);
  p.chunk = plan.chunk;
  p.nblk = (int)(plan.splits * p.tiles);
  p.q64_w = BKP / a.Wo; p.r64_w = BKP % a.Wo;
  p.q_h = p.q64_w / a.Ho; p.r_h = p.q64_w % a.Ho;
  const bool pointwise = a.KH == 1 && a.KW == 1 && a.stride == 1 && a.pad == 0;
  constexpr int SHMEM = 2 * BUF;
  if (int e = dy_raise_lds_limit("wgrad_v4", {{&wgrad_kernel<false, bf16_t>, SHMEM}, {&wgrad_kernel<true, bf16_t>, SHMEM},
                                              {&wgrad_kernel<false, f16_t>, SHMEM}, {&wgrad_kernel<true, f16_t>, SHMEM}}))
    return e;
  hipStream_t st = (hipStream_t)stream;
  dy_note_kernel("wg4::wgrad_kernel+reduce_kernel");
  if (int e = dy_dispatch_16bit("wgrad_v4", a.dtype, [&](auto tag) {
        using T = typename decltype(tag)::type;
        if (pointwise) wgrad_kernel<true, T><<<p.nblk, 512, SHMEM, st>>>(p);
        else wgrad_kernel<false, T><<<p.nblk, 512, SHMEM, st>>>(p);
        DY_LAUNCH_CHECK();
        return 0;
      }))
    return e;
  reduce_kernel<<<dim3(dy_cdiv(a.Cin, 256), a.Cout, a.KH * a.KW), 256, 0, st>>>(a.scratch, (int)plan.splits, p.tiles, p.tiles_q, a.Cout, a.Cin, a.Cin_pad, a.KH * a.KW, a.g_oihw);
  DY_LAUNCH_CHECK();
  return 0;
}
```

dedark_yolo_amd/engine/trainer.py:

```python
import contextlib
import math
import os
from pathlib import Path
from types import SimpleNamespace

import torch
import torch.distributed as dist
import yaml

from .. import ops
from .._C import OPT_RULES, call
from ..nn.modules import DyModule
from ..nn.tasks import DetectionModel, all_tasks, guess_model_task
from ..ops import ptr, stream

DEFAULT_CFG_PATH = Path(__file__).resolve().parent.parent / "cfg" / "default.yaml"


def get_cfg(overrides=None):
    with open(DEFAULT_CFG_PATH) as f:
        d = yaml.safe_load(f)
    for k, v in (overrides or {}).items():
        d[k] = v
    return SimpleNamespace(**d)


OPTIMIZERS = ("SGD", "Adam", "Adamax", "AdamW", "NAdam", "RAdam", "RMSProp")
ADAM_FAMILY = ("Adam", "Adamax", "NAdam", "RAdam")
STATE_KEYS = dict(SGD=("momentum_buffer", None), AdamW=("exp_avg", "exp_avg_sq"), Adam=("exp_avg", "exp_avg_sq"),
                  Adamax=("exp_avg", "exp_inf"), NAdam=("exp_avg", "exp_avg_sq"), RAdam=("exp_avg", "exp_avg_sq"),
                  RMSProp=("square_avg", "momentum_buffer"))


def resolve_optimizer(name, lr0, momentum, nc=10, total_iterations=None):
    if name == "auto":
        lr_fit = round(0.002 * 5 / (4 + nc), 6)
        iters = total_iterations if total_iterations is not None else 1e9
        return ("SGD", 0.01, 0.9) if iters > 10000 else ("AdamW", lr_fit, 0.9)
    if name not in OPTIMIZERS:
        raise NotImplementedError(f"Optimizer '{name}' not found in list of available optimizers [{', '.join(OPTIMIZERS)}, auto].")
    return name, lr0, momentum


def optimizer_of_state_dict(opt, opt_name=None):
    keys = set()
    for st in opt.get("state", {}).values():
        keys |= set(st)
    grp = (opt.get("param_groups") or [{}])[0]
    if not keys:
        keys = ({"momentum_buffer"} if "nesterov" in grp else {"square_avg"} if "alpha" in grp else {"mu_product"} if "momentum_decay" in grp
                else {"exp_avg_sq"} if "amsgrad" in grp or "decoupled_weight_decay" in grp else {"exp_inf"} if "betas" in grp else set())
        if not keys:
            return set(OPTIMIZERS)
    if "exp_inf" in keys:
        return {"Adamax"}
    if "mu_product" in keys:
        return {"NAdam"}
    if "square_avg" in keys:
        return {"RMSProp"}
    if "exp_avg_sq" in keys:
        if opt_name in ("Adam", "RAdam", "AdamW"):
            return {opt_name}
        if "amsgrad" not in grp:
            return {"RAdam"}
        if "decoupled_weight_decay" not in grp:
            return {"Adam", "AdamW"}
        return {"AdamW"} if grp["decoupled_weight_decay"] else {"Adam"}
    return {"SGD"} if "momentum_buffer" in keys else set()


class FlatState:

    def __init__(self, model, with_ema=True):
        import torch.nn as nn
        params, gids = [], []
        bn_types = tuple(v for k, v in nn.__dict__.items() if "Norm" in k and isinstance(v, type))
        seen = set()
        self.layer_ranges = []
        off = 0
        slots = []
        for li, layer in enumerate(model.model):
            start = off
            for mod in layer.modules():
                for name, p in mod.named_parameters(recurse=False):
                    if not p.requires_grad or id(p) in seen:
                        continue
                    seen.add(id(p))
                    g = 2 if "bias" in name else (1 if isinstance(mod, bn_types) else 0)
                    n = p.numel()
                    slots.append((p, off, n, g))
                    off += ops.round_up(n, 4)
            self.layer_ranges.append((li, start, off))
        self.n = off
        dev = next(model.parameters()).device
        f32 = torch.float32
        self.p = torch.zeros(off, dtype=f32, device=dev)
        self.g = torch.zeros(off, dtype=f32, device=dev)
        self.m = torch.zeros(off, dtype=f32, device=dev)
        self.m2 = None
        self.opt_state = None
        self.gid = torch.zeros(off, dtype=torch.uint8, device=dev)
        for p, o, n, g in slots:
            self.p[o:o + n].copy_(p.data.reshape(-1))
            p.data = self.p[o:o + n].view(p.shape)
            p.grad = self.g[o:o + n].view(p.shape)
            p._dy_direct = True
            self.gid[o:o + n] = g
        self.slots = slots
        self.ema = self.p.clone() if with_ema else None
        bufs = [b for b in model.buffers() if b.dtype.is_floating_point and b.numel() > 0 and b.is_cuda]
        self.buf_list = bufs
        nb = sum(ops.round_up(b.numel(), 4) for b in bufs)
        self.buf_flat = torch.zeros(nb, dtype=f32, device=dev)
        o = 0
        for b in bufs:
            n = b.numel()
            self.buf_flat[o:o + n].copy_(b.reshape(-1))
            b.data = self.buf_flat[o:o + n].view(b.shape)
            o += ops.round_up(n, 4)
        self.buf_ema = self.buf_flat.clone() if with_ema else None
        self.sumsq = torch.zeros(1, dtype=torch.float64, device=dev)
        ops.bump_weights_epoch()

    def alloc_optimizer(self, name):
        if STATE_KEYS[name][1] is not None:
            self.m2 = torch.zeros_like(self.m)
        if name in OPT_RULES:
            self.opt_state = torch.zeros(8, dtype=torch.float64, device=self.m.device)
            self.opt_state[1] = 1.0

    def ema_state_dict(self, model):
        sd = {}
        names = {id(p): k for k, p in model.named_parameters()}
        for p, o, n, _ in self.slots:
            sd[names[id(p)]] = self.ema[o:o + n].view(p.shape).clone()
        bnames = {id(b): k for k, b in model.named_buffers()}
        o = 0
        for b in self.buf_list:
            n = b.numel()
            sd[bnames[id(b)]] = self.buf_ema[o:o + n].view(b.shape).clone()
            o += ops.round_up(n, 4)
        return sd


class EarlyStopping:

    def __init__(self, patience=50):
        self.best_fitness, self.best_epoch = 0.0, 0
        self.patience = patience or float("inf")
        self.possible_stop = False

    def __call__(self, epoch, fitness):
        if fitness is None:
            return False
        if fitness >= self.best_fitness:
            self.best_epoch, self.best_fitness = epoch, fitness
        delta = epoch - self.best_epoch
        self.possible_stop = delta >= (self.patience - 1)
        return delta >= self.patience


class GradBuckets:

    def __init__(self, flat, model, bucket_bytes=None):
        if bucket_bytes is None:
            bucket_bytes = min(32 << 20, max(1 << 20, flat.n * 4 // 6))
        self.flat = flat
        self.works = []
        self.buckets = []
        cur_end, layers = flat.n, []
        for li, s, e in reversed(flat.layer_ranges):
            if e > s:
                layers.append(li)
            if (cur_end - s) * 4 >= bucket_bytes or li == 0:
                if cur_end > s:
                    self.buckets.append(dict(start=s, end=cur_end, layers=set(layers)))
                cur_end, layers = s, []
        self.owner = {li: b for b in self.buckets for li in b["layers"]}
        self._reset()
        for li, layer in enumerate(model.model):
            if li in self.owner:
                layer._dy_after_backward = (lambda idx: (lambda: self._layer_done(idx)))(li)

    def _reset(self):
        for b in self.buckets:
            b["left"] = len(b["layers"])

    def _layer_done(self, li):
        b = self.owner[li]
        b["left"] -= 1
        if b["left"] == 0:
            g = self.flat.g[b["start"]:b["end"]]
            side = ops.wgrad_side_stream() if ops.wgrad_pending() else None
            if side is None:
                self.works.append(dist.all_reduce(g, op=dist.ReduceOp.SUM, async_op=True))
            else:
                ops._side_wait_main()
                with torch.cuda.stream(side):
                    self.works.append(dist.all_reduce(g, op=dist.ReduceOp.SUM, async_op=True))

    def finish(self):
        for b in self.buckets:
            if b["left"] > 0:
                self.works.append(dist.all_reduce(self.flat.g[b["start"]:b["end"]], op=dist.ReduceOp.SUM, async_op=True))
        ev = self.exposed_events
        if ev is not None:
            e0, e1 = torch.cuda.Event(enable_timing=True), torch.cuda.Event(enable_timing=True)
            e0.record()
        for w in self.works:
            w.wait()
        if ev is not None:
            e1.record()
            ev.append((e0, e1))
        self.works.clear()
        self._reset()

    exposed_events = None


class DevicePrefetcher:

    def __init__(self, loader, device):
        self.it = iter(loader)
        self.device = device
        self.stream = torch.cuda.Stream(device=device)
        self.nxt = None
        self._load()

    def _load(self):
        try:
            b = next(self.it)
        except StopIteration:
            self.nxt = None
            return
        bi = b.get("batch_idx")
        if "n_max" not in b and torch.is_tensor(bi) and not bi.is_cuda and torch.is_tensor(b.get("img")):
            from ..utils.loss import n_max_of
            b = dict(b, n_max=n_max_of(bi, int(b["img"].shape[0])))
        with torch.cuda.stream(self.stream):
            self.nxt = {k: (v.to(self.device, non_blocking=True) if torch.is_tensor(v) and not v.is_cuda else v) for k, v in b.items()}

    def __iter__(self):
        return self

    def __next__(self):
        if self.nxt is None:
            raise StopIteration
        cur = torch.cuda.current_stream()
        cur.wait_stream(self.stream)
        b = self.nxt
        for v in b.values():
            if torch.is_tensor(v) and v.is_cuda:
                v.record_stream(cur)
        self._load()
        return b


class DetectionTrainer:

    def __init__(self, cfg=None, overrides=None):
        self.args = cfg if cfg is not None else get_cfg(overrides)
        self.rank = int(os.environ.get("RANK", -1))
        self.local_rank = int(os.environ.get("LOCAL_RANK", 0))
        self.world_size = int(os.environ.get("WORLD_SIZE", 1))
        self.device = torch.device("cuda", self.local_rank)
        self.model = None
        self.validator = None
        self.flat = None
        self.buckets = None
        self.updates = 0
        self.step_count = 0
        self.mse_acc = None
        self.pack_plan = ops.PackPlan()

    def get_model(self, cfg=None, weights=None, nc=None):
        model = DetectionModel(cfg or self.args.model, nc=nc)
        if weights is not None:
            model.load(weights)
        return model

    resolve_optimizer = staticmethod(resolve_optimizer)

    def setup(self, model=None, nc=None, total_iterations=None):
        torch.cuda.set_device(self.device)
        dt = str(getattr(self.args, "dtype", "fp32"))
        self.compute_dtype = (torch.bfloat16 if dt in ("bf16", "bfloat16") else
                              torch.float16 if dt in ("fp16", "float16", "half") else torch.float32)
        ops.set_compute_dtype(self.compute_dtype)
        self.loss_scale = (torch.tensor([65536.0, 0.0, 0.0], dtype=torch.float32, device=self.device)
                           if self.compute_dtype == torch.float16 else None)
        self.model = (model if model is not None else self.get_model(nc=nc)).to(self.device)
        self.model.args = self.args
        self.classify = guess_model_task(self.model) == "classify"
        if self.classify:
            if float(getattr(self.args, "dropout", 0.0) or 0.0) > 0.0:
                raise NotImplementedError("classify: dropout > 0 is not implemented (torch's Philox order cannot be matched)")
        self.model.train()
        if self.world_size > 1:
            if not dist.is_initialized():
                dist.init_process_group(os.environ.get("DY_DIST_BACKEND", "nccl" if dist.is_nccl_available() else "gloo"))
            for t in list(self.model.parameters()) + list(self.model.buffers()):
                dist.broadcast(t.data, src=0)
        self.flat = FlatState(self.model, with_ema=True)
        det = bool(getattr(self.args, "deterministic", False))
        ops.enable_wgrad_stream(not det)
        ops.enable_branch_streams(not det)
        if self.world_size > 1:
            self.buckets = GradBuckets(self.flat, self.model)
        a = self.args
        self.opt_name, self.lr0, self.momentum = self.resolve_optimizer(a.optimizer, a.lr0, a.momentum,
                                                                        getattr(self.model.model[-1], "nc", 10), total_iterations)
        if a.optimizer == "auto":
            a.warmup_bias_lr = 0.0
        self.flat.alloc_optimizer(self.opt_name)
        self.mse_acc = torch.zeros(1, dtype=torch.float64, device=self.device)
        nbs, bs = float(getattr(a, "nbs", 64)), max(int(getattr(a, "batch", 64)), 1)
        self.accumulate = max(round(nbs / bs), 1)
        self.weight_decay = a.weight_decay * bs * self.accumulate / nbs
        self.last_opt_step = -1
        self.acc_count = 0
        return self

    def preprocess_batch(self, batch):
        a = self.args
        img = batch["img"]
        if getattr(self, "classify", False):
            return self._preprocess_classify(batch)
        if img.dtype != torch.uint8:
            raise RuntimeError("preprocess_batch expects the dataloader's uint8 image tensor")
        bi = batch.get("batch_idx")
        if "n_max" not in batch and torch.is_tensor(bi) and not bi.is_cuda:
            from ..utils.loss import n_max_of
            batch["n_max"] = n_max_of(bi, int(img.shape[0]))
        img = img.to(self.device, non_blocking=True).contiguous()
        n = img.numel()
        out = torch.empty(img.shape, dtype=torch.float32, device=self.device)
        low, ded = bool(getattr(a, "lowlight_FLAG", False)), bool(getattr(a, "dedark_FLAG", False))
        both = low and ded
        clean = out if both else torch.empty_like(out)
        self.mse_acc.zero_()
        call("dy_preprocess_batch", ptr(img), ptr(out), None if both else ptr(clean), float(a.dark_param), int(low), int(ded),
             ptr(self.mse_acc), n, stream())
        batch["img"] = out
        batch["clean_img"] = clean
        batch["recovery_loss_batch"] = (self.mse_acc / n).float().reshape(())
        if both and getattr(a, "dark_channel_prior", False):
            from ..data.augment import dark_channel_prior
            batch["dedark_A"], batch["IcA"] = dark_channel_prior(out)
        return batch

    def _preprocess_classify(self, batch):
        from ..utils.loss import classify_batch_to_device
        return classify_batch_to_device(batch, self.device, self.mse_acc, nc=int(self.model.yaml["nc"]))

    def lr_factors(self, ni, nw, epoch, epochs):
        a = self.args
        lf = ((1 - math.cos(epoch * math.pi / epochs)) / 2) * (a.lrf - 1) + 1 if a.cos_lr else (1 - epoch / epochs) * (1.0 - a.lrf) + a.lrf
        lr = [self.lr0 * lf] * 3
        mom = self.momentum
        if ni <= nw:
            xi = ni / max(nw, 1)
            lr = [self.lr0 * lf * xi, self.lr0 * lf * xi, a.warmup_bias_lr + (self.lr0 * lf - a.warmup_bias_lr) * xi]
            if getattr(self, "opt_name", None) not in ADAM_FAMILY:
                mom = a.warmup_momentum + (self.momentum - a.warmup_momentum) * xi
        return lr, mom

    def optimizer_step(self, lr, mom):
        f = self.flat
        st = stream()
        g = f.g
        if self.acc_count > 0:
            call("dy_grad_accumulate", ptr(f.g_acc), ptr(f.g), f.n, st)
            g = f.g_acc
        f.sumsq.zero_()
        call("dy_sumsq", ptr(g), f.n, ptr(f.sumsq), st)
        self.updates += 1
        d = 0.9999 * (1 - math.exp(-self.updates / 2000))
        wd = self.weight_decay
        ls = getattr(self, "loss_scale", None)
        if self.opt_name == "AdamW":
            call("dy_adamw_step_scaled", ptr(f.p), ptr(g), ptr(f.m), ptr(f.m2), ptr(f.ema), ptr(f.gid), lr[0], lr[1], lr[2], wd, 0.0, 0.0,
                 mom, 0.999, 1e-8, self.updates, d, ptr(f.sumsq), 10.0, 1.0, ptr(ls), f.n, st)
        elif self.opt_name == "SGD":
            call("dy_sgd_step_scaled", ptr(f.p), ptr(g), ptr(f.m), ptr(f.ema), ptr(f.gid), lr[0], lr[1], lr[2], wd, 0.0, 0.0, mom, 1, d,
                 ptr(f.sumsq), 10.0, 1.0, ptr(ls), f.n, st)
        else:
            call("dy_optim_step", OPT_RULES[self.opt_name], ptr(f.p), ptr(g), ptr(f.m), ptr(f.m2), ptr(f.ema), ptr(f.gid), lr[0], lr[1],
                 lr[2], wd, 0.0, 0.0, mom, 0.99 if self.opt_name == "RMSProp" else 0.999, 1e-8, 0.004, d, ptr(f.sumsq), 10.0, 1.0, ptr(ls),
                 ptr(f.opt_state), f.n, st)
        if ls is not None:
            call("dy_loss_scale_update", ptr(ls), ptr(f.sumsq), 2.0, 0.5, 2000, st)
        if f.buf_ema is not None and f.buf_flat.numel():
            call("dy_ema_lerp", ptr(f.buf_ema), ptr(f.buf_flat), d, f.buf_flat.numel(), st)
        if self.acc_count > 0:
            f.g_acc.zero_()
            self.acc_count = 0
        ops.bump_weights_epoch()
        self.pack_plan.repack(self.model)

    def accumulate_gradients(self):
        f = self.flat
        if getattr(f, "g_acc", None) is None:
            f.g_acc = torch.zeros_like(f.g)
        call("dy_grad_accumulate", ptr(f.g_acc), ptr(f.g), f.n, stream())
        self.acc_count += 1

    def train_step(self, batch, lr=None, mom=None, step_optimizer=True):
        batch = self.preprocess_batch(batch)
        loss, items = self.model(batch)
        if getattr(self, "loss_scale", None) is not None:
            (loss * self.loss_scale[0]).backward()
        else:
            loss.backward()
        ops.wgrad_join()
        if self.buckets is not None:
            self.buckets.finish()
        if lr is None:
            lr, mom = [self.lr0] * 3, self.momentum
        if step_optimizer:
            self.optimizer_step(lr, mom)
        else:
            self.accumulate_gradients()
        self.step_count += 1
        return loss.detach(), items

    def _param_order(self):
        f = self.flat
        order = [[], [], []]
        for p, o, n, g in f.slots:
            order[{2: 0, 0: 1, 1: 2}[g]].append((o, n, tuple(p.shape)))
        return order[0] + order[1] + order[2], [len(x) for x in order]

    def optimizer_state_dict(self):
        f = self.flat
        name = self.opt_name
        flat, sizes = self._param_order()
        m, m2 = f.m.detach().cpu(), None if f.m2 is None else f.m2.detach().cpu()
        k1, k2 = STATE_KEYS[name]
        fused = name in OPT_RULES
        if fused:
            step, mu_product = (float(v) for v in f.opt_state[:2].cpu())
            if name == "RMSProp" and not float(self.momentum) > 0:
                k2 = None
        state = {}
        for i, (o, n, shape) in enumerate(flat):
            if name == "AdamW":
                state[i] = dict(step=torch.tensor(float(self.updates)), exp_avg=m[o:o + n].view(shape).clone(),
                                exp_avg_sq=m2[o:o + n].view(shape).clone())
            elif name == "SGD":
                state[i] = dict(momentum_buffer=m[o:o + n].view(shape).clone())
            elif step > 0:
                st = dict(step=torch.tensor(step, dtype=torch.float32))
                if name == "NAdam":
                    st["mu_product"] = torch.tensor(mu_product, dtype=torch.float32)
                st[k1] = m[o:o + n].view(shape).clone()
                if k2 is not None:
                    st[k2] = m2[o:o + n].view(shape).clone()
                state[i] = st
        groups, k = [], 0
        betas = dict(betas=(float(self.momentum), 0.999), eps=1e-8)
        extra = dict(SGD=dict(momentum=float(self.momentum), dampening=0, nesterov=True, fused=None),
                     AdamW=dict(betas, amsgrad=False, capturable=False, fused=None),
                     Adam=dict(betas, amsgrad=False, capturable=False, fused=None, decoupled_weight_decay=False),
                     Adamax=dict(betas, capturable=False),
                     NAdam=dict(betas, momentum_decay=0.004, decoupled_weight_decay=False, capturable=False),
                     RAdam=dict(betas, capturable=False, decoupled_weight_decay=False),
                     RMSProp=dict(momentum=float(self.momentum), alpha=0.99, eps=1e-8, centered=False, capturable=False))[name]
        for gi, cnt in enumerate(sizes):
            common = dict(lr=float(self.lr0), initial_lr=float(self.lr0), weight_decay=float(self.weight_decay) if gi == 1 else 0.0,
                          maximize=False, foreach=None, differentiable=False, params=list(range(k, k + cnt)))
            common.update(extra)
            groups.append(common)
            k += cnt
        return dict(state=state, param_groups=groups)

    def load_optimizer_state_dict(self, opt, opt_name=None):
        f = self.flat
        flat, sizes = self._param_order()
        groups = opt.get("param_groups", [])
        if [len(g["params"]) for g in groups] != sizes:
            raise RuntimeError(f"resume: optimizer groups {[len(g['params']) for g in groups]} do not match this model's {sizes}")
        name = self.opt_name
        if name not in optimizer_of_state_dict(opt, opt_name):
            raise RuntimeError(f"resume: checkpoint optimizer state does not belong to {name}")
        k1, k2 = STATE_KEYS[name]
        f.m.zero_()
        if f.m2 is not None:
            f.m2.zero_()
        step, mu_product = 0.0, 1.0
        for i, (o, n, shape) in enumerate(flat):
            st = opt["state"].get(i)
            if not st:
                continue
            if st.get(k1) is not None:
                f.m[o:o + n].copy_(st[k1].reshape(-1).float())
# ... 142 lines not shown
```

dedark_yolo_amd/ops.py:

```python
import ctypes as C
import math
import os
import weakref

import torch

from . import _C
from ._C import ACT_LEAKY, ACT_NONE, ACT_SILU, ConvDesc, DetMaps, DetMaps4, call

_compute_dtype = torch.float32
_pack_generation = 0
_weights_epoch = 0


def set_compute_dtype(dt):
    global _compute_dtype
    if dt not in (torch.float32, torch.bfloat16, torch.float16):
        raise ValueError(f"dedark_yolo_amd: unsupported compute dtype {dt}")
    _compute_dtype = dt


def get_compute_dtype():
    return _compute_dtype


_emulate_storage = None


def set_storage_emulation(dt):
    global _emulate_storage
    if dt not in (None, torch.bfloat16, torch.float16):
        raise ValueError("storage emulation: bf16 / fp16 / None")
    _emulate_storage = dt


def emu_round(*tensors):
    if _emulate_storage is not None:
        for t in tensors:
            if t is not None and t.dtype == torch.float32:
                t.copy_(t.to(_emulate_storage))


def bump_weights_epoch():
    global _weights_epoch
    _weights_epoch += 1


def dt_id(dtype):
    if dtype == torch.float32:
        return _C.DY_F32
    if dtype == torch.bfloat16:
        return _C.DY_BF16
    if dtype == torch.float16:
        return _C.DY_F16
    raise RuntimeError(f"dedark_yolo_amd: unsupported dtype {dtype}")


def vec_elems(dtype):
    return 4 if dtype == torch.float32 else 8


def round_up(c, m):
    return (c + m - 1) // m * m


_raw_stream = getattr(torch._C, "_cuda_getCurrentRawStream", None)
_cur_device = getattr(torch._C, "_cuda_getDevice", None)


def stream():
    if _raw_stream is not None and _cur_device is not None:
        return _raw_stream(_cur_device())
    return torch.cuda.current_stream().cuda_stream


def ptr(t):
    return None if t is None else t.data_ptr()


def require_gpu(t):
    if not t.is_cuda:
        raise RuntimeError("dedark_yolo_amd: the HIP path needs tensors on the GPU (there is no CPU fallback)")


def empty_nhwc(B, C_, H, W, dtype, device):
    return torch.empty((B, C_, H, W), dtype=dtype, device=device, memory_format=torch.channels_last)


def zeros_nhwc(B, C_, H, W, dtype, device):
    return torch.zeros((B, H, W, C_), dtype=dtype, device=device).permute(0, 3, 1, 2)


def ld_of(t):
    B, Cc, H, W = t.shape
    sb, sc, sh, sw = t.stride()
    if Cc > 1 and sc != 1:
        raise RuntimeError(f"dedark_yolo_amd: expected an NHWC (channels_last) view, got strides {t.stride()} for {tuple(t.shape)}")
    if W > 1:
        ld = sw
    elif H > 1:
        ld = sh
    elif B > 1:
        ld = sb
    else:
        ld = Cc
    if not (ld >= Cc and (W == 1 or sw == ld) and (H == 1 or sh == W * ld) and (B == 1 or sb == H * W * ld)):
        raise RuntimeError(f"dedark_yolo_amd: not a dense NHWC view: shape {tuple(t.shape)} strides {t.stride()}")
    return ld


def is_nhwc_view(t):
    try:
        ld_of(t)
        return True
    except RuntimeError:
        return False


def as_nhwc(t, dtype=None):
    dtype = dtype or _compute_dtype
    require_gpu(t)
    if t.dtype != dtype:
        t = t.to(dtype)
    ve = vec_elems(dtype)
    if is_nhwc_view(t) and (ld_of(t) >= round_up(t.shape[1], ve)) and (ld_of(t) * t.element_size()) % 16 == 0 \
            and t.data_ptr() % 16 == 0:
        return t
    Cc = t.shape[1]
    Cp = round_up(Cc, ve)
    if Cp == Cc:
        return t.contiguous(memory_format=torch.channels_last)
    buf = torch.zeros((t.shape[0], t.shape[2], t.shape[3], Cp), dtype=dtype, device=t.device)
    buf[..., :Cc] = t.permute(0, 2, 3, 1)
    return buf.permute(0, 3, 1, 2)[:, :Cc]


def padded_channels(t):
    ve = vec_elems(t.dtype)
    Cp = round_up(t.shape[1], ve)
    if Cp != t.shape[1] and ld_of(t) < Cp:
        raise RuntimeError("dedark_yolo_amd: channel count needs zero padding to a 16-byte multiple")
    return Cp


def vec_ok(t):
    return t.shape[1] % vec_elems(t.dtype) == 0 and t.data_ptr() % 16 == 0 and (ld_of(t) * t.element_size()) % 16 == 0


def copy_exact(src, dst, accumulate=False):
    B, Cc, H, W = src.shape
    if tuple(dst.shape) != (B, Cc, H, W) or dst.dtype != src.dtype:
        raise RuntimeError("copy_exact: views differ in shape or dtype")
    call("dy_copy2d_exact", ptr(src), ld_of(src), ptr(dst), ld_of(dst), B * H * W, Cc, 1 if accumulate else 0, dt_id(src.dtype), stream())


class _Arena:

    def __init__(self):
        self.buf = None
        self.off = 0
        self.used = 0
        self.chunks = 0
        self.retired = []
        self.main_raw = None

    def _new_chunk(self, cap, device):
        cur = stream()
        main_raw = self.main_raw if self.main_raw is not None else cur
        if cur == main_raw:
            buf = torch.zeros(cap, dtype=torch.float64, device=device)
        else:
            with torch.cuda.stream(torch.cuda.ExternalStream(main_raw, device=device)):
                buf = torch.zeros(cap, dtype=torch.float64, device=device)
        others = [s.cuda_stream for s in _branch["streams"]]
        if _wg_side.raw is not None:
            others.append(_wg_side.raw)
        if cur != main_raw and cur not in others:
            others.append(cur)
        for raw in others:
            call("dy_stream_fork", main_raw, raw)
        return buf

    def alloc(self, n, device):
        n = round_up(n, 2)
        self.used += n
        if self.buf is None or self.buf.device != device or self.off + n > self.buf.numel():
            cap = max(1 << 18, 4 * n)
            if self.buf is not None:
                self.retired.append(self.buf)
            self.buf = self._new_chunk(cap, device)
            self.off = 0
            self.chunks += 1
        out = self.buf[self.off:self.off + n]
        self.off += n
        return out

    def reset(self):
        self.main_raw = stream() if torch.cuda.is_available() else None
        self.retired.clear()
        if self.chunks > 1 and self.buf is not None:
            self.buf = torch.zeros(int(self.used * 1.25) + 1024, dtype=torch.float64, device=self.buf.device)
        elif self.buf is not None and self.off:
            self.buf[:self.off].zero_()
        self.off = 0
        self.used = 0
        self.chunks = 1 if self.buf is not None else 0


arena = _Arena()


def _w32(weight):
    w = weight.detach()
    if w.dtype != torch.float32 or not w.is_contiguous():
        w = w.float().contiguous()
    return w


def _pack(weight, cout_pad, cin_pad, transposed, dtype):
    key = (cout_pad, cin_pad, transposed, dtype)
    cache = weight.__dict__.setdefault("_dy_pack", {})
    hit = cache.get(key)
    tag = (_weights_epoch, weight._version)
    if hit is not None and hit[0] == tag:
        return hit[1]
    Co, Ci, KH, KW = weight.shape
    if hit is None:
        global _pack_generation
        _pack_generation += 1
    out = hit[1] if hit is not None else torch.empty(cout_pad * KH * KW * cin_pad, dtype=dtype, device=weight.device)
    w32 = _w32(weight)
    call("dy_pack_weight", ptr(w32), ptr(out), Co, cout_pad, Ci, cin_pad, KH, KW, 1 if transposed else 0, dt_id(dtype), stream())
    cache[key] = (tag, out)
    return out


_extra_pack_views = []


def register_pack_view(t):
    _extra_pack_views.append(weakref.ref(t))


class PackPlan:

    def __init__(self):
        self.sig = None
        self.table = None
        self.n_blocks = 0
        self._ent_key = None
        self._ent = []
        self._ent_sig = ()

    def _collect(self, model):
        ent = []
        _extra_pack_views[:] = [r for r in _extra_pack_views if r() is not None]
        for w in list(model.parameters()) + [r() for r in _extra_pack_views]:
            cache = w.__dict__.get("_dy_pack")
            if not cache or w.dtype != torch.float32 or not w.is_contiguous() or w.dim() != 4:
                continue
            for key, (tag, out) in cache.items():
                ent.append((w, key, out))
        return ent

    def repack(self, model):
        key = (id(model), _pack_generation)
        if key != self._ent_key:
            self._ent = self._collect(model)
            self._ent_sig = tuple((w.data_ptr(), out.data_ptr(), k) for w, k, out in self._ent)
            self._ent_key = key
        ent = self._ent
        if not ent:
            return
        sig = self._ent_sig
        if any(w.data_ptr() != sg[0] for (w, _, _), sg in zip(ent[:4], sig[:4])):
            self._ent_key = None
            return self.repack(model)
        if sig != self.sig:
            items = (_C.PackItem * len(ent))()
            blk = 0
            lib = _C.lib()
            for it, (w, (cout_pad, cin_pad, transposed, dtype), out) in zip(items, ent):
                Co, Ci, KH, KW = w.shape
                it.w, it.packed = w.data_ptr(), out.data_ptr()
                it.Cout, it.Cout_pad, it.Cin, it.Cin_pad, it.KH, it.KW = Co, cout_pad, Ci, cin_pad, KH, KW
                it.transposed, it.dtype, it.first_block = int(transposed), dt_id(dtype), blk
                blk += lib.dy_pack_item_blocks(cout_pad, cin_pad, KH, KW)
            raw = torch.frombuffer(bytearray(bytes(items)), dtype=torch.uint8)
            self.table = raw.to(ent[0][0].device)
            self.n_blocks, self.sig = blk, sig
        call("dy_pack_weights_multi", ptr(self.table), len(ent), self.n_blocks, stream())
        for w, key, out in ent:
            w.__dict__["_dy_pack"][key] = ((_weights_epoch, w._version), out)


def _padded_vec(v, n):
    if v is None:
        return None
    v = v.detach()
    if v.numel() == n and v.dtype == torch.float32:
        return v
    out = torch.zeros(n, dtype=torch.float32, device=v.device)
    out[:v.numel()] = v
    return out


def bn_fold(bn, cout_pad):
    tag = (_weights_epoch, bn.weight._version, bn.bias._version, bn.running_mean._version, bn.running_var._version,
           bn.weight.data_ptr(), bn.running_mean.data_ptr(), cout_pad)
    hit = bn.__dict__.get("_dy_fold")
    if hit is not None and hit[0] == tag:
        return hit[1]
    aff = hit[1] if (hit is not None and hit[1].shape[1] == cout_pad and hit[1].device == bn.weight.device) else \
        torch.empty((2, cout_pad), dtype=torch.float32, device=bn.weight.device)
    call("dy_bn_fold_eval_valid", ptr(bn.weight), ptr(bn.bias), ptr(bn.running_mean), ptr(bn.running_var), float(bn.eps),
         ptr(aff[0]), ptr(aff[1]), cout_pad, bn.weight.numel(), stream())
    bn.__dict__["_dy_fold"] = (tag, aff)
    return aff


def bn_fold_is_current(bn):
    hit = bn.__dict__.get("_dy_fold")
    return hit is not None and hit[0][:7] == (_weights_epoch, bn.weight._version, bn.bias._version, bn.running_mean._version,
                                               bn.running_var._version, bn.weight.data_ptr(), bn.running_mean.data_ptr())


class ConvCtx:
    __slots__ = ("x", "z", "aff", "weight", "bias", "bn", "act", "k", "stride", "pad", "dil", "cout", "cout_pad", "cin_pad",
                 "has_bn", "y", "owner", "shared")


def _conv_desc(src, w, dst, N, Hs, Ws, Cs, Hd, Wd, Cd, KH, KW, stride, pad, dil, scale, shift, act, stats, accumulate, dtype):
    if dst is not None:
        dptr, dld = dst.data_ptr(), ld_of(dst)
    else:
        dptr, dld = None, Cd
    return ConvDesc(src.data_ptr(), ld_of(src), N, Hs, Ws, Cs, w.data_ptr(), dptr, dld, Hd, Wd, Cd, KH, KW, stride, pad, dil,
                    None if scale is None else scale.data_ptr(), None if shift is None else shift.data_ptr(), act,
                    None if stats is None else stats.data_ptr(), 1 if accumulate else 0, dt_id(dtype))


_bn_pending = {}


def flush_bn_counters():
    for bn, n in _bn_pending.items():
        bn.num_batches_tracked += n
    _bn_pending.clear()


def _conv_meta(Cin, Cout, KH, KW, stride, B, H, W, pixels, note=""):
    return dict(shape=f"{Cin}->{Cout} k{KH} s{stride} in {B}x{H}x{W}{note}", flops=2.0 * pixels * Cout * KH * KW * Cin)


def _bn_train_begin(bn, C, dev):
    _bn_pending[bn] = _bn_pending.get(bn, 0) + 1
    bn.__dict__.pop("_dy_fold", None)
    return torch.empty((4, C), dtype=torch.float32, device=dev)


def _bn_train_tail(z, stats, bn, act, residual, y, pixels, C, C_valid, did, st):
    aff = _bn_train_begin(bn, C, z.device)
    pa, sa = aff.data_ptr(), 4 * C
    call("dy_bn_finalize_valid", ptr(stats), pixels, ptr(bn.weight), ptr(bn.bias), ptr(bn.running_mean), ptr(bn.running_var),
         float(bn.momentum), float(bn.eps), pa, pa + sa, pa + 2 * sa, pa + 3 * sa, C, C_valid, st)
    rp, rld = (residual.data_ptr(), ld_of(residual)) if residual is not None else (None, 0)
    _C._prof is not None and _C.set_meta(kind="bn_act_fwd", shape=f"{C}ch {y.shape[0]}x{y.shape[2]}x{y.shape[3]}", dtype=str(z.dtype), flops=0.0,
                                         bytes=float(pixels * C * z.element_size() * (3 if residual is not None else 2)))
    call("dy_bn_act_fwd", ptr(z), ld_of(z), pa, pa + sa, act, rp, rld, ptr(y), ld_of(y), pixels, C, did, st)
    emu_round(y)
    return aff


def conv_forward(tape, x, weight, bias=None, bn=None, act=ACT_NONE, stride=1, pad=0, dil=1, training=False, out=None,
                 residual=None, owner=None, shared=False):
    dtype = x.dtype
    B, Cin, H, W = x.shape
    Cout, Cw, KH, KW = weight.shape
    if Cw != Cin:
        raise RuntimeError(f"conv: weight expects {Cw} input channels, got {Cin}")
    ve = vec_elems(dtype)
    cin_pad = padded_channels(x)
    cout_pad = round_up(Cout, ve)
    Ho = (H + 2 * pad - dil * (KH - 1) - 1) // stride + 1
    Wo = (W + 2 * pad - dil * (KW - 1) - 1) // stride + 1
    wp = _pack(weight, cout_pad, cin_pad, False, dtype)
    dev = x.device
    has_bn = bn is not None
    batch_stats = has_bn and training
    ctx = None
    if tape is not None:
        ctx = ConvCtx()
        ctx.x, ctx.weight, ctx.bias, ctx.bn, ctx.act = x, weight, bias, bn, act
        ctx.owner = owner if owner is not None else weight
        ctx.shared = shared
        ctx.k, ctx.stride, ctx.pad, ctx.dil = (KH, KW), stride, pad, dil
        ctx.cout, ctx.cout_pad, ctx.cin_pad, ctx.has_bn = Cout, cout_pad, cin_pad, has_bn
    if batch_stats:
        z = empty_nhwc(B, cout_pad, Ho, Wo, dtype, dev)
        stats = arena.alloc(2 * cout_pad * _C.STATS_REPLICAS, dev)
        d = _conv_desc(x, wp, z, B, H, W, cin_pad, Ho, Wo, cout_pad, KH, KW, stride, pad, dil, None, None, ACT_NONE, stats,
                       False, dtype)
        pixels = B * Ho * Wo
        y = out if out is not None else empty_nhwc(B, cout_pad, Ho, Wo, dtype, dev)
        st = stream()
        if _C._prof is None and _emulate_storage is None:
            aff = _bn_train_begin(bn, cout_pad, dev)
            rp, rld = (residual.data_ptr(), ld_of(residual)) if residual is not None else (None, 0)
            bp = bn._parameters
            call("dy_conv2d_bn_act_fwd_valid", C.byref(d), pixels, ptr(bp["weight"]), ptr(bp["bias"]), ptr(bn.running_mean), ptr(bn.running_var),
                 float(bn.momentum), float(bn.eps), aff.data_ptr(), act, rp, rld, y.data_ptr(), ld_of(y), Cout, st)
        else:
            _C._prof is not None and _C.set_meta(kind="conv_fwd", dtype=str(dtype), **_conv_meta(Cin, Cout, KH, KW, stride, B, H, W, pixels),
                                                 bytes=float((B * H * W * Cin + pixels * Cout + Cout * KH * KW * Cin) * x.element_size()))
            call("dy_conv2d_fwd", C.byref(d), st)
            emu_round(z)
            aff = _bn_train_tail(z, stats, bn, act, residual, y, pixels, cout_pad, Cout, dt_id(dtype), st)
        if ctx is not None:
            ctx.z, ctx.aff, ctx.y = z, aff, None
    else:
        if has_bn:
            aff = bn_fold(bn, cout_pad)
            scale, shift = aff[0], aff[1]
        else:
            scale, shift = None, _padded_vec(bias, cout_pad)
        direct = residual is None
        y = out if (out is not None and direct) else empty_nhwc(B, cout_pad, Ho, Wo, dtype, dev)
        d = _conv_desc(x, wp, y, B, H, W, cin_pad, Ho, Wo, cout_pad, KH, KW, stride, pad, dil, scale, shift, act, None, False,
                       dtype)
        _C._prof is not None and _C.set_meta(kind="conv_fwd", dtype=str(dtype), **_conv_meta(Cin, Cout, KH, KW, stride, B, H, W, B * Ho * Wo),
                                             bytes=float((B * H * W * Cin + B * Ho * Wo * Cout + Cout * KH * KW * Cin) * x.element_size()))
        call("dy_conv2d_fwd", C.byref(d), stream())
        if not direct:
            tgt = out if out is not None else y
            if tgt is not y:
                call("dy_copy2d", ptr(y), ld_of(y), ptr(tgt), ld_of(tgt), B * Ho * Wo, cout_pad, 0, dt_id(dtype), stream())
            call("dy_copy2d", ptr(residual), ld_of(residual), ptr(tgt), ld_of(tgt), B * Ho * Wo, cout_pad, 1, dt_id(dtype),
                 stream())
            y = tgt
        emu_round(y)
        if ctx is not None:
            if has_bn:
                raise RuntimeError("conv: gradients through an eval-mode BatchNorm are not supported")
            ctx.z, ctx.aff, ctx.y = None, None, y
    if tape is not None:
        tape.push(ctx)
    return y if cout_pad == Cout else y[:, :Cout]


def _add_pgrad(tape, p, g):
    if p is None or not p.requires_grad:
        return
    if p in tape.pgrads:
        tape.pgrads[p] = tape.pgrads[p] + g
    else:
        tape.pgrads[p] = g


_wg_scratch = {}


def wgrad_scratch(device, elems=32 << 20, tag=0):
    t = _wg_scratch.get((device, tag))
    if t is None or t.numel() < elems:
        t = torch.empty(elems, dtype=torch.float32, device=device)
        _wg_scratch[(device, tag)] = t
    return t


class _WgradSide:
    GROUP = 8

    def __init__(self):
        self.on = False
        self.stream = None
        self.raw = None
        self.cur = []
        self.groups = []
        self.free_events = []
        self.cb_queued = False


_wg_side = _WgradSide()


def enable_wgrad_stream(on=True):
    _wg_side.on = bool(on) and os.environ.get("DY_WGRAD_STREAM", "1") != "0"


def wgrad_stream_enabled():
    return bool(_wg_side.on)


def wgrad_side_stream(device=None):
    s = _wg_side
    if not s.on:
        return None
    if s.stream is None:
        prio = int(os.environ.get("DY_WGRAD_PRIO", "0"))
        s.stream = torch.cuda.Stream(device=device, priority=prio)
        s.raw = s.stream.cuda_stream
    return s.stream


def _side_wait_main():
    call("dy_stream_fork", stream(), _wg_side.raw)


def _wg_track(x, dz):
    s = _wg_side
    s.cur.append((x, dz))
    if len(s.cur) < s.GROUP or torch.cuda.is_current_stream_capturing():
        return
    ev = s.free_events.pop() if s.free_events else torch.cuda.Event()
    ev.record(s.stream)
    s.groups.append((ev, s.cur))
    s.cur = []
    while s.groups and s.groups[0][0].query():
        s.free_events.append(s.groups.pop(0)[0])


def wgrad_pending():
    return bool(_wg_side.cur or _wg_side.groups)


def wgrad_join():
    s = _wg_side
    if s.cur or s.groups:
        call("dy_stream_fork", s.raw, stream())
        s.free_events.extend(g[0] for g in s.groups)
        s.groups.clear()
        s.cur = []
    s.cb_queued = False


_branch = {"on": False, "streams": [], "by_device": {}}


def enable_branch_streams(on=True):
    _branch["on"] = bool(on) and os.environ.get("DY_BRANCH_STREAMS", "1") != "0"


def branch_streams(n, device):
    if not _branch["on"] or n <= 0:
        return None
    dev = torch.device(device)
    key = dev.index if dev.index is not None else torch.cuda.current_device()
    mine = _branch["by_device"].setdefault(key, [])
    while len(mine) < n:
        s = torch.cuda.Stream(device=device)
        mine.append(s)
        _branch["streams"].append(s)
    return mine[:n]


def _grad_dst(p):
    if p is not None and p.requires_grad and getattr(p, "_dy_direct", False) and p.grad is not None:
        return p.grad
    return None


def _grad_sink(p, shape, dev, shared=False):
    gd = None if shared else _grad_dst(p)
    if gd is not None:
        return gd, True
    return torch.empty(shape, dtype=torch.float32, device=dev), False


def _bn_backward(tape, dy, z, aff, bn, act, dz, pixels, C, C_valid, did, st, dev, shared):
    sums = arena.alloc(2 * C * _C.BN_BWD_REPLICAS, dev)
    pa = aff.data_ptr()
    gb_ = None if shared else _grad_dst(bn.bias)
    gw_, direct = _grad_sink(bn.weight, (2, C_valid), dev, gb_ is None)
    if not direct:
        gw_, gb_ = gw_[0], gw_[1]
    if _C._prof is None or _emulate_storage is not None:
        call("dy_bn_act_bwd_valid", dy.data_ptr(), ld_of(dy), z.data_ptr(), ld_of(z), pa, ptr(bn._parameters["weight"]), act,
             sums.data_ptr(), dz.data_ptr(), ld_of(dz), gw_.data_ptr(), gb_.data_ptr(), pixels, C, C_valid, did, st)
    else:
        sa, nb = 4 * C, float(pixels * C * dy.element_size())
        _C.set_meta(kind="bn_act_bwd_reduce", shape=f"{C}ch {pixels}px", dtype=str(dy.dtype), flops=0.0, bytes=nb * 2)
        call("dy_bn_act_bwd_reduce", ptr(dy), ld_of(dy), ptr(z), ld_of(z), pa, pa + sa, pa + 2 * sa, pa + 3 * sa,
             act, 1, ptr(sums), pixels, C, did, st)
        _C.set_meta(kind="bn_act_bwd_apply", shape=f"{C}ch {pixels}px", dtype=str(dy.dtype), flops=0.0, bytes=nb * 3)
        call("dy_bn_act_bwd_apply_valid", ptr(dy), ld_of(dy), ptr(z), ld_of(z), pa, pa + sa, pa + 2 * sa, pa + 3 * sa,
             ptr(bn.weight), act, 1, ptr(sums), ptr(dz), ld_of(dz), ptr(gw_), ptr(gb_), pixels, C, C_valid, did, st)
    emu_round(dz)
    if not direct:
        _add_pgrad(tape, bn.weight, gw_)
        _add_pgrad(tape, bn.bias, gb_)


def _act_backward(tape, dy, y, bias, act, dz, pixels, C, C_valid, did, st, dev, shared):
    need_bias = bias is not None and bias.requires_grad
    if dz is dy and not need_bias:
        return
    sums = arena.alloc(2 * C * _C.BN_BWD_REPLICAS, dev)
    pdy, ldy, py, ly = dy.data_ptr(), ld_of(dy), y.data_ptr(), ld_of(y)
    call("dy_bn_act_bwd_reduce", pdy, ldy, py, ly, None, None, None, None, act, 0, ptr(sums), pixels, C, did, st)
    db, direct = _grad_sink(bias, C, dev, shared or C != C_valid)
    pdz, ldz, n = (pdy, ldy, 0) if dz is dy else (dz.data_ptr(), ld_of(dz), pixels)
    call("dy_bn_act_bwd_apply_valid", pdy, ldy, py, ly, None, None, None, None, None, act, 0, ptr(sums), pdz, ldz, None, ptr(db),
         n, C, C_valid, did, st)
    if dz is not dy:
        emu_round(dz)
    if need_bias and not direct:
        gd = None if shared else _grad_dst(bias)
        if gd is not None:
            gd.copy_(db[:C_valid])
        else:
            _add_pgrad(tape, bias, db[:C_valid])


def conv_backward(tape, dy, need_dx=True, dx_out=None, accumulate=False, add_src=None):
    ctx = tape.pop()
    x = ctx.x
    dtype = x.dtype
    dev = x.device
    B, Cin, H, W = x.shape
    KH, KW = ctx.k
    Cout, cout_pad, cin_pad = ctx.cout, ctx.cout_pad, ctx.cin_pad
    Ho, Wo = dy.shape[2], dy.shape[3]
    if cout_pad != Cout:
        if padded_channels(dy) != cout_pad:
            raise RuntimeError("conv_backward: gradient view lacks zero padding")
    pixels = B * Ho * Wo
    did = dt_id(dtype)
    st = stream()
    if ctx.has_bn:
        dz = empty_nhwc(B, cout_pad, Ho, Wo, dtype, dev)
        _bn_backward(tape, dy, ctx.z, ctx.aff, ctx.bn, ctx.act, dz, pixels, cout_pad, Cout, did, st, dev, ctx.shared)
    else:
        dz = empty_nhwc(B, cout_pad, Ho, Wo, dtype, dev) if ctx.act != ACT_NONE else dy
        _act_backward(tape, dy, ctx.y, ctx.bias, ctx.act, dz, pixels, cout_pad, Cout, did, st, dev, ctx.shared)
    return _conv_grads(tape, ctx, dz, need_dx, dx_out, accumulate, add_src)


def _conv_grads(tape, ctx, dz, need_dx=True, dx_out=None, accumulate=False, add_src=None):
    x = ctx.x
    dtype = x.dtype
    dev = x.device
    B, Cin, H, W = x.shape
    KH, KW = ctx.k
    Cout, cout_pad, cin_pad = ctx.cout, ctx.cout_pad, ctx.cin_pad
    Ho, Wo = dz.shape[2], dz.shape[3]
    pixels = B * Ho * Wo
    did = dt_id(dtype)
    st = stream()
    if ctx.owner.requires_grad:
        gw, direct = _grad_sink(ctx.owner, ctx.weight.shape, dev, ctx.shared)
        side = wgrad_side_stream(dev) if direct else None
        st_w = st
        if side is not None:
            if _C._prof is not None:
                _side_wait_main()
            if not _wg_side.cb_queued:
                try:
                    torch.autograd.Variable._execution_engine.queue_callback(wgrad_join)
                    _wg_side.cb_queued = True
                except RuntimeError:
                    pass
            st_w = side.cuda_stream
        scratch = wgrad_scratch(dev, tag=st_w)
        _C._prof is not None and _C.set_meta(kind="conv_wgrad", dtype=str(dtype), **_conv_meta(Cin, Cout, KH, KW, ctx.stride, B, H, W, pixels),
                    bytes=float((B * H * W * Cin + pixels * Cout) * x.element_size() + Cout * KH * KW * Cin * 4))
        wargs = (ptr(x), ld_of(x), B, H, W, cin_pad, ptr(dz), ld_of(dz), Ho, Wo, cout_pad, KH, KW, ctx.stride, ctx.pad, ctx.dil, Cout, Cin,
                 ptr(scratch), scratch.numel(), ptr(gw), did)
        if side is not None and _C._prof is not None:
            with torch.cuda.stream(side):
                call("dy_conv2d_wgrad", *wargs, st_w)
        elif side is not None:
            call("dy_conv2d_wgrad_forked", st, *wargs, st_w)
        else:
            call("dy_conv2d_wgrad", *wargs, st_w)
        if side is not None:
            _wg_track(x, dz)
        if not direct:
            _add_pgrad(tape, ctx.owner, gw.view(ctx.owner.shape))
    if not need_dx:
        return None
    wt = _pack(ctx.weight, cout_pad, cin_pad, True, dtype)
    planar = (dx_out is None and add_src is None and dtype in (torch.bfloat16, torch.float16) and cin_pad == 8 and Cin <= 4 and (KH, KW) == (3, 3) and ctx.stride == 2
              and ctx.pad == 1 and ctx.dil == 1 and cout_pad in (16, 32, 64) and os.environ.get("DY_NO_CONV_SMALL") is None)
    if planar:
        dxp = torch.empty((B, Cin, H, W), dtype=dtype, device=dev)
        d = _conv_desc(dz, wt, None, B, Ho, Wo, cout_pad, H, W, cin_pad, KH, KW, ctx.stride, ctx.pad, ctx.dil, None, None, ACT_NONE,
                       None, False, dtype)
        d.dst_valid_channels = Cin
        d.dst_planar = dxp.data_ptr()
        _C._prof is not None and _C.set_meta(kind="conv_dgrad", dtype=str(dtype), **_conv_meta(Cin, Cout, KH, KW, ctx.stride, B, H, W, pixels, " (planar)"),
                    bytes=float((B * H * W * Cin + pixels * Cout) * x.element_size()))
        call("dy_conv2d_dgrad", C.byref(d), st)
        return dxp
    if dx_out is None:
        dxb = empty_nhwc(B, cin_pad, H, W, dtype, dev)
        accumulate = False
    else:
        dxb = dx_out
        if padded_channels(dxb) != cin_pad:
            raise RuntimeError("conv_backward: dx_out view too narrow")
    d = _conv_desc(dz, wt, dxb, B, Ho, Wo, cout_pad, H, W, cin_pad, KH, KW, ctx.stride, ctx.pad, ctx.dil, None, None, ACT_NONE,
                   None, accumulate, dtype)
    d.dst_valid_channels = Cin
    if add_src is not None:
        if tuple(add_src.shape) != (B, Cin, H, W) or add_src.dtype != dtype or padded_channels(add_src) != cin_pad:
            raise RuntimeError("conv_backward: add_src must be an NHWC view of dx's shape and dtype")
        d.add_src, d.add_src_ld = add_src.data_ptr(), ld_of(add_src)
    _C._prof is not None and _C.set_meta(kind="conv_dgrad", dtype=str(dtype), **_conv_meta(Cin, Cout, KH, KW, ctx.stride, B, H, W, pixels),
                bytes=float((B * H * W * Cin * (2 if accumulate else 1) + pixels * Cout + Cout * KH * KW * Cin) * x.element_size()))
    call("dy_conv2d_dgrad", C.byref(d), st)
    emu_round(dxb)
    if dx_out is not None:
        return dx_out
    return dxb if cin_pad == Cin else dxb[:, :Cin]


def conv_bn_stats_forward(x, weight, bn, stride=1, pad=0, dil=1, owner=None):
    dtype = x.dtype
    B, Cin, H, W = x.shape
    Cout, Cw, KH, KW = weight.shape
    if Cw != Cin:
        raise RuntimeError(f"conv: weight expects {Cw} input channels, got {Cin}")
    ve = vec_elems(dtype)
    cin_pad = padded_channels(x)
    cout_pad = round_up(Cout, ve)
    Ho = (H + 2 * pad - dil * (KH - 1) - 1) // stride + 1
    Wo = (W + 2 * pad - dil * (KW - 1) - 1) // stride + 1
    dev = x.device
    wp = _pack(weight, cout_pad, cin_pad, False, dtype)
    z = empty_nhwc(B, cout_pad, Ho, Wo, dtype, dev)
    stats = arena.alloc(2 * cout_pad * _C.STATS_REPLICAS, dev)
    d = _conv_desc(x, wp, z, B, H, W, cin_pad, Ho, Wo, cout_pad, KH, KW, stride, pad, dil, None, None, ACT_NONE, stats, False, dtype)
    pixels = B * Ho * Wo
    st = stream()
    _C._prof is not None and _C.set_meta(kind="conv_fwd", dtype=str(dtype), **_conv_meta(Cin, Cout, KH, KW, stride, B, H, W, pixels),
                                         bytes=float((B * H * W * Cin + pixels * Cout + Cout * KH * KW * Cin) * x.element_size()))
    call("dy_conv2d_fwd", C.byref(d), st)
    emu_round(z)
    aff = _bn_train_begin(bn, cout_pad, dev)
    pa, sa = aff.data_ptr(), 4 * cout_pad
    call("dy_bn_finalize_valid", ptr(stats), pixels, ptr(bn.weight), ptr(bn.bias), ptr(bn.running_mean), ptr(bn.running_var),
         float(bn.momentum), float(bn.eps), pa, pa + sa, pa + 2 * sa, pa + 3 * sa, cout_pad, Cout, st)
    ctx = ConvCtx()
    ctx.x, ctx.weight, ctx.bias, ctx.bn, ctx.act = x, weight, None, bn, ACT_NONE
    ctx.owner, ctx.shared = owner if owner is not None else weight, False
    ctx.k, ctx.stride, ctx.pad, ctx.dil = (KH, KW), stride, pad, dil
    ctx.cout, ctx.cout_pad, ctx.cin_pad, ctx.has_bn = Cout, cout_pad, cin_pad, True
    ctx.z, ctx.aff, ctx.y = z, aff, None
    return z, aff, ctx


def bn2_act_bwd_workspace(pixels, C_, dtype):
    return int(_C.lib().dy_bn2_act_bwd_workspace(pixels, C_, dt_id(dtype)))


def repconv_forward(tape, x, conv1, conv2, act, training, out=None):
    dtype = x.dtype
    B, Cin, H, W = x.shape
    Cout = conv1.conv.weight.shape[0]
    if Cout % vec_elems(dtype) or Cin % vec_elems(dtype):
        raise NotImplementedError(f"RepConv: {Cin} -> {Cout} channels are not whole 16-byte vectors in {dtype}")
    uv = []
    for m in (conv1, conv2):
        c = m.conv
        if training:
            uv.append(conv_bn_stats_forward(x, c.weight, m.bn, c.stride[0], c.padding[0], c.dilation[0]))
        else:
            if tape is not None:
                raise RuntimeError("repconv: gradients through an eval-mode BatchNorm are not supported")
            z = conv_forward(None, x, c.weight, None, None, ACT_NONE, c.stride[0], c.padding[0], c.dilation[0])
            uv.append((z, bn_fold(m.bn, Cout), None))
    (u, au, cu), (v, av, cv) = uv
    if u.shape != v.shape:
        raise RuntimeError(f"repconv: the branches disagree in shape, {tuple(u.shape)} and {tuple(v.shape)}")
    y = out if out is not None else empty_nhwc(B, Cout, u.shape[2], u.shape[3], dtype, x.device)
    pixels = B * u.shape[2] * u.shape[3]
    _C._prof is not None and _C.set_meta(kind="bn2_act_fwd", shape=f"{Cout}ch {pixels}px", dtype=str(dtype), flops=0.0,
                                         bytes=float(3 * pixels * Cout * x.element_size()))
    call("dy_bn2_act_fwd", ptr(u), ld_of(u), ptr(v), ld_of(v), ptr(au[0]), ptr(au[1]), ptr(av[0]), ptr(av[1]), act, ptr(y), ld_of(y),
         pixels, Cout, dt_id(dtype), stream())
    emu_round(y)
    if tape is not None:
        tape.push((cu, cv, act))
    return y


def repconv_backward(tape, dy, need_dx=True, dx_out=None, accumulate=False, add_src=None):
    cu, cv, act = tape.pop()
    u, v = cu.z, cv.z
    B, Cc, Ho, Wo = u.shape
    dtype, dev = u.dtype, u.device
    pixels = B * Ho * Wo
    du, dv = empty_nhwc(B, Cc, Ho, Wo, dtype, dev), empty_nhwc(B, Cc, Ho, Wo, dtype, dev)
    ws = torch.empty(bn2_act_bwd_workspace(pixels, Cc, dtype), dtype=torch.float32, device=dev)
    sinks = []
    for c in (cu, cv):
        gb_ = _grad_dst(c.bn.bias)
        gw_, direct = _grad_sink(c.bn.weight, (2, Cc), dev, gb_ is None)
        if not direct:
            gw_, gb_ = gw_[0], gw_[1]
        sinks.append((gw_, gb_, direct))
    pu, pv, s = cu.aff.data_ptr(), cv.aff.data_ptr(), 4 * Cc
    _C._prof is not None and _C.set_meta(kind="bn2_act_bwd", shape=f"{Cc}ch {pixels}px", dtype=str(dtype), flops=0.0,
                                         bytes=float(8 * pixels * Cc * u.element_size()))
    call("dy_bn2_act_bwd", ptr(dy), ld_of(dy), ptr(u), ld_of(u), ptr(v), ld_of(v), pu, pu + s, pu + 2 * s, pu + 3 * s, ptr(cu.bn.weight),
         pv, pv + s, pv + 2 * s, pv + 3 * s, ptr(cv.bn.weight), act, ptr(du), ld_of(du), ptr(dv), ld_of(dv), ptr(sinks[0][0]),
         ptr(sinks[0][1]), ptr(sinks[1][0]), ptr(sinks[1][1]), ptr(ws), ws.numel(), pixels, Cc, dt_id(dtype), stream())
    emu_round(du, dv)
    for c, (gw_, gb_, direct) in zip((cu, cv), sinks):
        if not direct:
            _add_pgrad(tape, c.bn.weight, gw_)
            _add_pgrad(tape, c.bn.bias, gb_)
    dx = _conv_grads(tape, cu, du, need_dx, dx_out, accumulate, add_src)
    _conv_grads(tape, cv, dv, need_dx, dx, True)
    return dx


def _nhwc_like(B, Cc, H, W, dtype, device):
    Cp = round_up(Cc, vec_elems(dtype))
    if Cp == Cc:
        return empty_nhwc(B, Cc, H, W, dtype, device)
    return zeros_nhwc(B, Cp, H, W, dtype, device)[:, :Cc]


def _pconv_packed(weight, w32, transposed, dtype):
    c3 = weight.shape[0]
    if dtype == torch.float32 or c3 < 16:
        return None
    cache = weight.__dict__.setdefault("_dy_pconv_pack", {})
    key, tag = (bool(transposed), dtype), (_weights_epoch, weight._version, weight.data_ptr())
    hit = cache.get(key)
    if hit is not None and hit[0] == tag:
        return hit[1]
    out = hit[1] if hit is not None else torch.empty(9 * ((c3 + 31) // 32) * ((c3 + 15) // 16) * 512, dtype=dtype, device=weight.device)
    call("dy_pconv_pack", ptr(w32), ptr(out), c3, 1 if transposed else 0, dt_id(dtype), stream())
    cache[key] = (tag, out)
    return out


def pconv_forward(tape, x, weight, out=None):
    B, Cc, H, W = x.shape
    c3 = weight.shape[0]
    if tuple(weight.shape) != (c3, c3, 3, 3) or c3 > Cc:
        raise RuntimeError(f"pconv: weight {tuple(weight.shape)} does not fit {Cc} channels")
    y = out if out is not None else _nhwc_like(B, Cc, H, W, x.dtype, x.device)
    w32 = _w32(weight)
    es = x.element_size()
    _C._prof is not None and _C.set_meta(kind="pconv_fwd", shape=f"{c3}/{Cc} k3 in {B}x{H}x{W}", dtype=str(x.dtype),
                                         flops=2.0 * B * H * W * c3 * 9 * c3, bytes=float(2 * B * H * W * Cc * es + 9 * c3 * c3 * 4))
    wp = _pconv_packed(weight, w32, False, x.dtype)
    call("dy_pconv_fwd", ptr(x), ld_of(x), ptr(y), ld_of(y), ptr(w32), ptr(wp), B, H, W, Cc, c3, dt_id(x.dtype), stream())
    emu_round(y)
    if tape is not None:
        tape.push((x, weight))
    return y


def pconv_backward(tape, dy, dx_out=None, accumulate=False, add_src=None):
    x, weight = tape.pop()
    B, Cc, H, W = x.shape
    c3 = weight.shape[0]
    dtype, dev, st = x.dtype, x.device, stream()
    es = x.element_size()
    if tuple(dy.shape) != (B, Cc, H, W) or dy.dtype != dtype:
        raise RuntimeError("pconv_backward: gradient does not match the forward's output")
    if weight.requires_grad:
        gw, direct = _grad_sink(weight, weight.shape, dev)
        scratch = wgrad_scratch(dev, tag=st)
        _C._prof is not None and _C.set_meta(kind="pconv_wgrad", shape=f"{c3}/{Cc} k3 in {B}x{H}x{W}", dtype=str(dtype),
                                             flops=2.0 * B * H * W * c3 * 9 * c3, bytes=float(2 * B * H * W * c3 * es + 9 * c3 * c3 * 4))
        call("dy_pconv_wgrad", ptr(x), ld_of(x), ptr(dy), ld_of(dy), ptr(gw), B, H, W, c3, ptr(scratch), scratch.numel(), dt_id(dtype), st)
        if not direct:
            _add_pgrad(tape, weight, gw)
    if dx_out is None:
        dx, accumulate = _nhwc_like(B, Cc, H, W, dtype, dev), False
    else:
        dx = dx_out
    if add_src is not None and (tuple(add_src.shape) != (B, Cc, H, W) or add_src.dtype != dtype):
        raise RuntimeError("pconv_backward: add_src must be an NHWC view of dx's shape and dtype")
    w32 = _w32(weight)
    n_rw = 2 + (1 if accumulate else 0) + (1 if add_src is not None else 0)
    _C._prof is not None and _C.set_meta(kind="pconv_dgrad", shape=f"{c3}/{Cc} k3 in {B}x{H}x{W}", dtype=str(dtype),
                                         flops=2.0 * B * H * W * c3 * 9 * c3, bytes=float(n_rw * B * H * W * Cc * es + 9 * c3 * c3 * 4))
    wp = _pconv_packed(weight, w32, True, dtype)
    call("dy_pconv_dgrad", ptr(dy), ld_of(dy), ptr(dx), ld_of(dx), ptr(w32), ptr(wp), B, H, W, Cc, c3, 1 if accumulate else 0,
         ptr(add_src), 0 if add_src is None else ld_of(add_src), dt_id(dtype), st)
    emu_round(dx)
    return dx


def _cru_packed(w3, w1, G, transposed, dtype):
    GN, C1 = w1.shape[0], w1.shape[1]
    C3 = 0 if w3 is None else w3.shape[1]
    cache = w1.__dict__.setdefault("_dy_cru_pack", {})
    key = (bool(transposed), dtype)
    tag = (_weights_epoch, w1._version, w1.data_ptr(), None if w3 is None else (w3._version, w3.data_ptr()))
    hit = cache.get(key)
    if hit is not None and hit[0] == tag:
        return hit[1]
    out = hit[1] if hit is not None else torch.empty(GN * (9 * C3 + C1), dtype=dtype, device=w1.device)
    call("dy_cru_conv_pack", None if w3 is None else ptr(_w32(w3)), ptr(_w32(w1)), ptr(out), G, GN // G, C3, C1, 1 if transposed else 0,
         dt_id(dtype), stream())
    cache[key] = (tag, out)
    return out


def _cru_dims(x, w3, bias, w1, G):
    GN, C1 = w1.shape[0], w1.shape[1]
    C3 = 0 if w3 is None else w3.shape[1]
    if (tuple(w1.shape[2:]) != (1, 1) or GN % G or x.shape[1] != C1 or (bias is not None and tuple(bias.shape) != (GN,))
            or (w3 is not None and (tuple(w3.shape) != (GN, C3, 3, 3) or G * C3 != C1)) or (w3 is None and G != 1)):
        raise RuntimeError(f"cru_conv: weights {None if w3 is None else tuple(w3.shape)} / {tuple(w1.shape)} in {G} groups do not fit "
                           f"{x.shape[1]} channels")
    return GN // G, C3, C1


def cru_conv_forward(tape, x, w3, bias, w1, G=1, out=None):
    B, _, H, W = x.shape
    N, C3, C1 = _cru_dims(x, w3, bias, w1, G)
    y = out if out is not None else empty_nhwc(B, G * N, H, W, x.dtype, x.device)
    if tuple(y.shape) != (B, G * N, H, W) or y.dtype != x.dtype:
        raise RuntimeError("cru_conv_forward: out must be an NHWC view of the result's shape and dtype")
    wp = _cru_packed(w3, w1, G, False, x.dtype)
    es = x.element_size()
    _C._prof is not None and _C.set_meta(kind="cru_fwd", shape=f"{G}x{N} <- 9x{C3}+{C1} in {B}x{H}x{W}", dtype=str(x.dtype),
                                         flops=2.0 * B * H * W * G * N * (9 * C3 + C1), bytes=float(B * H * W * (C1 + G * N) * es))
    call("dy_cru_conv_fwd", ptr(x), ld_of(x), ptr(wp), None if bias is None else ptr(_w32(bias)), ptr(y), ld_of(y), B, H, W, G, N, C3, C1,
         dt_id(x.dtype), stream())
    emu_round(y)
    if tape is not None:
        tape.push((x, w3, bias, w1, G))
    return y


def cru_conv_backward(tape, dy, need_dx=True, dx_out=None, accumulate=False):
    x, w3, bias, w1, G = tape.pop()
    B, _, H, W = x.shape
    N, C3, C1 = _cru_dims(x, w3, bias, w1, G)
    dtype, dev, st = x.dtype, x.device, stream()
    es = x.element_size()
    if tuple(dy.shape) != (B, G * N, H, W) or dy.dtype != dtype:
        raise RuntimeError("cru_conv_backward: gradient does not match the forward's output")
    want = [p is not None and p.requires_grad for p in (w3, bias, w1)]
    if any(want):
        g3 = torch.empty(w3.shape, dtype=torch.float32, device=dev) if want[0] else None
        gb = torch.empty(bias.shape, dtype=torch.float32, device=dev) if want[1] else None
        g1 = torch.empty(w1.shape, dtype=torch.float32, device=dev) if want[2] else None
        scratch = wgrad_scratch(dev, tag=st)
        _C._prof is not None and _C.set_meta(kind="cru_wgrad", shape=f"{G}x{N} <- 9x{C3}+{C1} in {B}x{H}x{W}", dtype=str(dtype),
                                             flops=2.0 * B * H * W * G * N * (9 * C3 + C1), bytes=float(B * H * W * (C1 + G * N) * es))
        call("dy_cru_conv_wgrad", ptr(x), ld_of(x), ptr(dy), ld_of(dy), ptr(g3), ptr(gb), ptr(g1), B, H, W, G, N, C3, C1, ptr(scratch),
             scratch.numel(), dt_id(dtype), st)
        for p, g in ((w3, g3), (bias, gb), (w1, g1)):
            if g is not None:
                _add_pgrad(tape, p, g)
    if not need_dx:
        return None
    if dx_out is None:
        dx, accumulate = empty_nhwc(B, C1, H, W, dtype, dev), False
    else:
        dx = dx_out
        if tuple(dx.shape) != (B, C1, H, W) or dx.dtype != dtype:
            raise RuntimeError("cru_conv_backward: dx_out must be an NHWC view of the input's shape and dtype")
    wp = _cru_packed(w3, w1, G, True, dtype)
    _C._prof is not None and _C.set_meta(kind="cru_dgrad", shape=f"{G}x{N} <- 9x{C3}+{C1} in {B}x{H}x{W}", dtype=str(dtype),
                                         flops=2.0 * B * H * W * G * N * (9 * C3 + C1),
                                         bytes=float(B * H * W * ((2 if accumulate else 1) * C1 + G * N) * es))
    call("dy_cru_conv_dgrad", ptr(dy), ld_of(dy), ptr(wp), ptr(dx), ld_of(dx), B, H, W, G, N, C3, C1, 1 if accumulate else 0, dt_id(dtype), st)
    emu_round(dx)
    return dx


def _attn_dims(who, q, k, v, heads):
    B, Cc, H, W = q.shape
    if tuple(k.shape) != tuple(q.shape) or tuple(v.shape) != tuple(q.shape) or k.dtype != q.dtype or v.dtype != q.dtype:
        raise RuntimeError(f"{who}: q, k and v must be NHWC views of one shape and dtype")
    if heads < 1 or Cc % heads:
        raise RuntimeError(f"{who}: {Cc} channels do not split into {heads} heads")
# ... 574 lines not shown
```

include/dedark_yolo.h:

```cpp
#ifndef DEDARK_YOLO_H
#define DEDARK_YOLO_H
#include <stddef.h>
#include <stdint.h>
#ifdef __cplusplus
extern "C" {
#endif

#define DY_F32 0
#define DY_BF16 1
#define DY_F16 2
#define DY_ACT_NONE 0
#define DY_ACT_SILU 1
#define DY_ACT_LEAKY 2
#define DY_STATS_REPLICAS 64
#define DY_BN_BWD_REPLICAS 8

const char* dy_last_error(void);
int dy_version(void);
const char* dy_last_kernel(void);
void dy_clear_last_kernel(void);

typedef struct {
  const void* src;
  int64_t src_ld;
  int N, Hs, Ws, Cs;
  const void* w;
  void* dst;
  int64_t dst_ld;
  int Hd, Wd, Cd;
  int KH, KW, stride, pad, dil;
  const float* scale;
  const float* shift;
  int act;
  double* stats;
  int accumulate;
  int dtype;
  int64_t dst_row_stride;
  int64_t dst_img_stride;
  int KHf, KWf;
  int kh0, kh_step;
  int kw0, kw_step;
  int dst_valid_channels;
  void* dst_planar;
  const void* add_src;
  int64_t add_src_ld;
} dy_conv_desc;

int dy_conv2d_fwd(const dy_conv_desc* d, void* stream);
int dy_conv2d_dgrad(const dy_conv_desc* d, void* stream);
int dy_conv2d_wgrad(const void* x, int64_t x_ld, int N, int Hi, int Wi, int Cin_pad, const void* dz, int64_t dz_ld, int Ho,
                    int Wo, int Cout_pad, int KH, int KW, int stride, int pad, int dil, int Cout, int Cin, float* scratch,
                    int64_t scratch_elems, float* g_oihw, int dtype, void* stream);
int dy_pack_weight(const float* w_oihw, void* packed, int Cout, int Cout_pad, int Cin, int Cin_pad, int KH, int KW,
                   int transposed, int dtype, void* stream);
typedef struct {
  const float* w;
  void* packed;
  int Cout, Cout_pad, Cin, Cin_pad, KH, KW, transposed, dtype;
  int64_t first_block;
} dy_pack_item;
int64_t dy_pack_item_blocks(int Cout_pad, int Cin_pad, int KH, int KW);
int dy_pack_weights_multi(const dy_pack_item* items_dev, int n_items, int64_t n_blocks, void* stream);

int dy_bn_finalize(const double* stats, int64_t count, const float* gamma, const float* beta, float* running_mean,
                   float* running_var, float momentum, float eps, float* scale, float* shift, float* mean, float* invstd,
                   int C, void* stream);
int dy_bn_fold_eval(const float* gamma, const float* beta, const float* running_mean, const float* running_var, float eps,
                    float* scale, float* shift, int C, void* stream);
int dy_bn_finalize_valid(const double* stats, int64_t count, const float* gamma, const float* beta, float* running_mean,
                         float* running_var, float momentum, float eps, float* scale, float* shift, float* mean, float* invstd,
                         int C, int C_valid, void* stream);
int dy_bn_fold_eval_valid(const float* gamma, const float* beta, const float* running_mean, const float* running_var, float eps,
                          float* scale, float* shift, int C, int C_valid, void* stream);
int dy_bn_act_fwd(const void* z, int64_t z_ld, const float* scale, const float* shift, int act, const void* residual,
                  int64_t res_ld, void* y, int64_t y_ld, int64_t pixels, int C, int dtype, void* stream);
int dy_bn_act_bwd_reduce(const void* dy, int64_t dy_ld, const void* z, int64_t z_ld, const float* scale,
                         const float* shift, const float* mean, const float* invstd, int act, int has_bn, double* sums,
                         int64_t pixels, int C, int dtype, void* stream);
int dy_bn_act_bwd_apply(const void* dy, int64_t dy_ld, const void* z, int64_t z_ld, const float* scale, const float* shift,
                        const float* mean, const float* invstd, const float* gamma, int act, int has_bn,
                        const double* sums, void* dz, int64_t dz_ld, float* dgamma, float* dbeta, int64_t pixels, int C,
                        int dtype, void* stream);
int dy_bn_act_bwd_apply_valid(const void* dy, int64_t dy_ld, const void* z, int64_t z_ld, const float* scale, const float* shift,
                              const float* mean, const float* invstd, const float* gamma, int act, int has_bn,
                              const double* sums, void* dz, int64_t dz_ld, float* dgamma, float* dbeta, int64_t pixels, int C,
                              int C_valid, int dtype, void* stream);

int dy_bn2_act_fwd(const void* u, int64_t u_ld, const void* v, int64_t v_ld, const float* scale_u, const float* shift_u,
                   const float* scale_v, const float* shift_v, int act, void* y, int64_t y_ld, int64_t pixels, int C, int dtype,
                   void* stream);
#define DY_BN2_MAX_PARTS 1024
int64_t dy_bn2_act_bwd_workspace(int64_t pixels, int C, int dtype);
int dy_bn2_act_bwd(const void* dy, int64_t dy_ld, const void* u, int64_t u_ld, const void* v, int64_t v_ld, const float* scale_u,
                   const float* shift_u, const float* mean_u, const float* invstd_u, const float* gamma_u, const float* scale_v,
                   const float* shift_v, const float* mean_v, const float* invstd_v, const float* gamma_v, int act, void* du,
                   int64_t du_ld, void* dv, int64_t dv_ld, float* dgamma_u, float* dbeta_u, float* dgamma_v, float* dbeta_v,
                   float* workspace, int64_t workspace_elems, int64_t pixels, int C, int dtype, void* stream);

int dy_maxpool_fwd(const void* x, int64_t x_ld, void* y, int64_t y_ld, uint8_t* argmax, int N, int H, int W, int C, int k,
                   int stride, int pad, int Ho, int Wo, int dtype, void* stream);
int dy_maxpool_bwd(const void* dy, int64_t dy_ld, const uint8_t* argmax, void* dx, int64_t dx_ld, int N, int H, int W, int C,
                   int k, int stride, int pad, int Ho, int Wo, int accumulate, int dtype, void* stream);
int dy_upsample_nearest_fwd(const void* x, int64_t x_ld, void* y, int64_t y_ld, int N, int H, int W, int C, int scale,
                            int dtype, void* stream);
int dy_upsample_nearest_bwd(const void* dy, int64_t dy_ld, void* dx, int64_t dx_ld, int N, int H, int W, int C, int scale,
                            int accumulate, int dtype, void* stream);
int dy_copy2d(const void* src, int64_t src_ld, void* dst, int64_t dst_ld, int64_t pixels, int C, int accumulate, int dtype,
              void* stream);
int dy_cast(const void* src, int src_dtype, void* dst, int dst_dtype, int64_t n, void* stream);

int dy_pconv_pack(const float* w, void* wp, int c3, int transposed, int dtype, void* stream);
int dy_pconv_fwd(const void* x, int64_t x_ld, void* y, int64_t y_ld, const float* w, const void* wp, int N, int H, int W, int C, int c3,
                 int dtype, void* stream);
int dy_pconv_dgrad(const void* dy, int64_t dy_ld, void* dx, int64_t dx_ld, const float* w, const void* wp, int N, int H, int W, int C,
                   int c3, int accumulate, const void* add_src, int64_t add_ld, int dtype, void* stream);
int dy_pconv_wgrad(const void* x, int64_t x_ld, const void* dy, int64_t dy_ld, float* dw, int N, int H, int W, int c3, float* scratch,
                   int64_t scratch_elems, int dtype, void* stream);
int dy_dwconv_fwd(const void* x, int64_t x_ld, void* y, int64_t y_ld, const float* w, int N, int H, int W, int C, int k, int stride,
                  const float* scale, const float* shift, int act, double* stats, int stats_c, int dtype, void* stream);
int dy_dwconv_dgrad(const void* dz, int64_t dz_ld, void* dx, int64_t dx_ld, const float* w, int N, int H, int W, int C, int k, int stride,
                    int accumulate, const void* add_src, int64_t add_ld, int dtype, void* stream);
int dy_dwconv_wgrad(const void* x, int64_t x_ld, const void* dz, int64_t dz_ld, float* dw, int N, int H, int W, int C, int k, int stride,
                    float* scratch, int64_t scratch_elems, int dtype, void* stream);
int dy_copy2d_exact(const void* src, int64_t src_ld, void* dst, int64_t dst_ld, int64_t pixels, int C, int accumulate, int dtype,
                    void* stream);
int dy_asff_fuse_fwd(const void* x0, int64_t ld0, const void* x1, int64_t ld1, const void* x2, int64_t ld2,
                     const void* logits, int64_t ldl, void* out, int64_t ldo, int64_t pixels, int C, int dtype, void* stream);
int dy_asff_fuse_bwd(const void* dout, int64_t lddo, const void* x0, int64_t ld0, const void* x1, int64_t ld1,
                     const void* x2, int64_t ld2, const void* logits, int64_t ldl, void* dx0, int64_t ldd0, void* dx1,
                     int64_t ldd1, void* dx2, int64_t ldd2, void* dlogits, int64_t lddl, int64_t pixels, int C,
                     int acc0, int acc1, int acc2, int dtype, void* stream);

int dy_image_to_nhwc8(const float* x, int B, int H, int W, void* y, int Ho, int Wo, int dtype, void* stream);
int dy_resize_bwd(const float* dy_nhwc, int dy_ld, int B, int H, int W, int Ho, int Wo, float* dx, void* stream);
int dy_filter_params_fwd(const float* feat, int feat_ld, float* params, int B, void* stream);
int dy_filter_params_bwd(const float* feat, int feat_ld, const double* dparams, float* dfeat, int B, void* stream);
int dy_filters_pointwise_fwd(const float* x, const float* params, const float* A, const float* IcA, float* s4, int B,
                             int H, int W, int fast_math, void* stream);
int dy_usm_fwd(const float* s4, const float* params, float* out_nchw, void* out_nhwc8, float* hp, int B, int H, int W,
               int dtype, void* stream);
int dy_usm_bwd(const float* dout_nchw, const void* dout_nhwc, int dout_ld, const float* hp, const float* params, float* ds4,
               double* dparams, int B, int H, int W, int dtype, void* stream);
int dy_filters_pointwise_bwd(const float* x, const float* params, const float* A, const float* IcA, const float* ds4,
                             float* dx, double* dparams, int B, int H, int W, int accumulate, int fast_math, void* stream);

typedef struct {
  const void* map[3];
  int64_t map_ld[3];
  int h[3], w[3];
  float stride[3];
  int B, nc, n_levels, dtype;
} dy_det_maps;

#define DY_DET_MAX_LEVELS 4
typedef struct {
  dy_det_maps base;
  const void* map3;
  int64_t map_ld3;
  int h3, w3;
  float stride3;
} dy_det_maps4;

int dy_loss_prepare_targets(const float* batch_idx, const float* cls, const float* bboxes, int n_targets, int B,
                            int n_max, float img_w, float img_h, float* gt, int32_t* counts, void* stream);
int dy_loss_decode(const dy_det_maps* m, float* pred_boxes, void* stream);
int dy_tal_assign(const dy_det_maps* m, const float* pred_boxes, const float* gt, const int32_t* counts, int n_max,
                  float* work_f, int32_t* work_i, uint8_t* work_b, int32_t* target_gt_idx, uint8_t* fg_mask, float* norm,
                  int32_t* target_label, float* target_box, void* stream);
int dy_tal_assign_decoded(const float* pd_scores, const float* pd_bboxes, const float* anc_points, const float* gt,
                          const int32_t* counts, int B, int A, int nc, int n_max, float* work_f, int32_t* work_i, uint8_t* work_b,
                          int32_t* target_gt_idx, uint8_t* fg_mask, float* norm, int32_t* target_label, float* target_box,
                          void* stream);
int dy_chan_moments(const void* x, int64_t ld, int N, int64_t HW, int C, double* out, int dtype, void* stream);
int dy_sru_fwd(const void* x, int64_t x_ld, void* y, int64_t y_ld, int N, int64_t HW, int C, int groups, const double* moments,
               const float* gamma, const float* beta, float eps, int dtype, void* stream);
int dy_sru_bwd(const void* x, int64_t x_ld, const void* dy, int64_t dy_ld, void* dx, int64_t dx_ld, int N, int64_t HW, int C, int groups,
               const double* moments, const float* gamma, const float* beta, float eps, double* red, int dtype, void* stream);
int dy_cru_fuse_fwd(const void* o, int64_t o_ld, void* res, int64_t r_ld, int N, int64_t HW, int C, const double* moments, int dtype,
                    void* stream);
int dy_cru_fuse_bwd(const void* o, int64_t o_ld, const void* dres, int64_t d_ld, void* dout, int64_t do_ld, int N, int64_t HW, int C,
                    const double* moments, double* ds, int dtype, void* stream);
int dy_cru_conv_pack(const float* w3, const float* w1, void* wp, int G, int N, int C3, int C1, int transposed, int dtype, void* stream);
int dy_cru_conv_fwd(const void* x, int64_t x_ld, const void* wp, const float* bias, void* y, int64_t y_ld, int B, int H, int W, int G, int N,
                    int C3, int C1, int dtype, void* stream);
int dy_cru_conv_dgrad(const void* dy, int64_t dy_ld, const void* wp, void* dx, int64_t dx_ld, int B, int H, int W, int G, int N, int C3,
                      int C1, int accumulate, int dtype, void* stream);
int dy_cru_conv_wgrad(const void* x, int64_t x_ld, const void* dy, int64_t dy_ld, float* dw3, float* db, float* dw1, int B, int H, int W,
                      int G, int N, int C3, int C1, float* scratch, int64_t scratch_elems, int dtype, void* stream);
int dy_attn_fwd(const void* q, int64_t q_ld, const void* k, int64_t k_ld, const void* v, int64_t v_ld, void* o, int64_t o_ld, float* lse, int B,
                int L, int H, int D, float scale, int dtype, void* stream);
int dy_attn_bwd(const void* q, int64_t q_ld, const void* k, int64_t k_ld, const void* v, int64_t v_ld, const void* o, int64_t o_ld,
                const void* dout, int64_t do_ld, const float* lse, void* dq, int64_t dq_ld, void* dk, int64_t dk_ld, void* dv, int64_t dv_ld,
                int B, int L, int H, int D, float scale, int dtype, void* stream);
#define DY_LN_MAX_C 2048
#define DY_LN_MAX_PARTS 512
int dy_add_layernorm_fwd(const void* a, int64_t a_ld, const void* b, int64_t b_ld, const float* gamma, const float* beta, void* y,
                         int64_t y_ld, float* stats, int64_t rows, int C, float eps, int dtype, void* stream);
int dy_add_layernorm_bwd(const void* a, int64_t a_ld, const void* b, int64_t b_ld, const float* stats, const float* gamma, const void* dy,
                         int64_t dy_ld, void* dz, int64_t dz_ld, int accumulate, float* dgamma, float* dbeta, float* scratch,
                         int64_t scratch_elems, int64_t rows, int C, int dtype, void* stream);
int dy_gelu_fwd(const void* u, int64_t u_ld, void* y, int64_t y_ld, int64_t pixels, int C, int dtype, void* stream);
int dy_gelu_bwd(const void* u, int64_t u_ld, const void* dy, int64_t dy_ld, void* du, int64_t du_ld, int64_t pixels, int C, int dtype,
                void* stream);
int dy_add_pos(const void* x, int64_t x_ld, const void* pos, void* y, int64_t y_ld, int B, int L, int C, int dtype, void* stream);
int dy_bbox_ciou(const float* b1, const float* b2, int64_t n, float* out, float* grad_b1, void* stream);
int dy_bbox_iou(const float* b1, const float* b2, int64_t n, int xywh, int kind, float eps, float* out, float* grad_b1, void* stream);
int dy_dfl_loss(const float* pred_dist, const float* target, int64_t n_boxes, float* out, float* grad, void* stream);
int dy_loss_fwd(const dy_det_maps* m, const float* pred_boxes, const uint8_t* fg_mask, const float* norm,
                const int32_t* target_label, const float* target_box, double* acc, void* stream);
int dy_loss_finish(const double* acc, const float* recovery, float hyp_box, float hyp_cls, float hyp_dfl, float lrl,
                   int B, float* loss_out, float* items, void* stream);
int dy_loss_bwd(const dy_det_maps* m, void* const* dmap, const int64_t* dmap_ld, const float* pred_boxes,
                const uint8_t* fg_mask, const float* norm, const int32_t* target_label, const float* target_box,
                const double* acc, const float* grad_out, float hyp_box, float hyp_cls, float hyp_dfl, void* stream);
int dy_detect_decode(const dy_det_maps* m, float* y, void* stream);
int dy_detect_decode_rows(const dy_det_maps* m, float* y, int rows, void* stream);
int dy_tta_scale_img(const float* x, int B, int C, int H, int W, int hs, int ws, int Hp, int Wp, int flip, float* out, void* stream);
int dy_detect_decode_tta(const dy_det_maps* m, float* y, int64_t a_total, int col0, int a_lo, int a_hi, float scale, int flip,
                         float img_h, float img_w, void* stream);
int dy_nms_candidates(const float* pred, int B, int nc, int A, float conf_thres, int multi_label, uint64_t* keys, int* counts,
                      int64_t cap, void* stream);
int dy_nms_sort(const uint64_t* keys, uint64_t* keys_sorted, const int* counts, int B, int64_t cap, void* workspace,
                size_t* workspace_bytes, void* stream);
int dy_nms_greedy(const float* pred, const uint64_t* keys_sorted, const int* counts, int B, int nc, int A, int64_t cap,
                  double iou_thres, int max_nms, int max_det, float max_wh, int agnostic, float* boxes_ws, uint8_t* dead_ws,
                  float* out, int64_t* keep_idx, int* out_counts, void* stream);

int dy_preprocess_batch(const uint8_t* img, float* img_out, float* clean_out, float dark_param, int lowlight, int dedark,
                        double* mse_acc, int64_t n, void* stream);

int dy_sumsq(const float* g, int64_t n, double* acc, void* stream);
int dy_sgd_step(float* p, const float* g, float* mom_buf, float* ema, const uint8_t* group_id, float lr0, float lr1, float lr2,
                float wd0, float wd1, float wd2, float momentum, int nesterov, float ema_decay, const double* sumsq,
                float max_norm, float grad_scale, int64_t n, void* stream);
int dy_adamw_step(float* p, const float* g, float* exp_avg, float* exp_avg_sq, float* ema, const uint8_t* group_id, float lr0,
                  float lr1, float lr2, float wd0, float wd1, float wd2, float beta1, float beta2, float eps, int step,
                  float ema_decay, const double* sumsq, float max_norm, float grad_scale, int64_t n, void* stream);
int dy_sgd_step_scaled(float* p, const float* g, float* mom_buf, float* ema, const uint8_t* group_id, float lr0, float lr1, float lr2,
                       float wd0, float wd1, float wd2, float momentum, int nesterov, float ema_decay, const double* sumsq,
                       float max_norm, float grad_scale, const float* loss_scale, int64_t n, void* stream);
int dy_adamw_step_scaled(float* p, const float* g, float* exp_avg, float* exp_avg_sq, float* ema, const uint8_t* group_id, float lr0,
                         float lr1, float lr2, float wd0, float wd1, float wd2, float beta1, float beta2, float eps, int step,
                         float ema_decay, const double* sumsq, float max_norm, float grad_scale, const float* loss_scale, int64_t n,
                         void* stream);
int dy_loss_scale_update(float* state, const double* sumsq, float growth, float backoff, int interval, void* stream);
enum { DY_OPT_ADAM = 0, DY_OPT_ADAMAX = 1, DY_OPT_NADAM = 2, DY_OPT_RADAM = 3, DY_OPT_RMSPROP = 4 };
typedef struct dy_optim_state {
  double step;
  double mu_product;
  float grad_coef;
  int32_t skipped;
  float c[4];
  float reserved[6];
} dy_optim_state;
int dy_optim_step(int rule, float* p, const float* g, float* buf1, float* buf2, float* ema, const uint8_t* group_id, float lr0,
                  float lr1, float lr2, float wd0, float wd1, float wd2, double beta1, double beta2, double eps,
                  double momentum_decay, float ema_decay, const double* sumsq, float max_norm, float grad_scale,
                  const float* loss_scale, dy_optim_state* state, int64_t n, void* stream);
int dy_ema_lerp(float* ema, const float* src, float decay, int64_t n, void* stream);
int dy_grad_accumulate(float* acc, const float* g, int64_t n, void* stream);
int dy_conv2d_bn_act_fwd(const dy_conv_desc* d, int64_t count, const float* gamma, const float* beta, float* running_mean,
                         float* running_var, float momentum, float eps, float* aff, int act, const void* residual, int64_t res_ld,
                         void* y, int64_t y_ld, void* stream);
int dy_bn_act_bwd(const void* dy, int64_t dy_ld, const void* z, int64_t z_ld, const float* aff, const float* gamma, int act,
                  double* sums, void* dz, int64_t dz_ld, float* dgamma, float* dbeta, int64_t pixels, int C, int dtype, void* stream);
int dy_conv2d_bn_act_fwd_valid(const dy_conv_desc* d, int64_t count, const float* gamma, const float* beta, float* running_mean,
                               float* running_var, float momentum, float eps, float* aff, int act, const void* residual,
                               int64_t res_ld, void* y, int64_t y_ld, int C_valid, void* stream);
int dy_bn_act_bwd_valid(const void* dy, int64_t dy_ld, const void* z, int64_t z_ld, const float* aff, const float* gamma, int act,
                        double* sums, void* dz, int64_t dz_ld, float* dgamma, float* dbeta, int64_t pixels, int C, int C_valid,
                        int dtype, void* stream);
int dy_conv2d_wgrad_forked(void* wait_for, const void* x, int64_t x_ld, int N, int Hi, int Wi, int Cin_pad, const void* dz,
                           int64_t dz_ld, int Ho, int Wo, int Cout_pad, int KH, int KW, int stride, int pad, int dil, int Cout,
                           int Cin, float* scratch, int64_t scratch_elems, float* g_oihw, int dtype, void* stream);

int dy_stream_fork(void* from, void* to);
int dy_frontend_init(void);

typedef struct dy_aug_sample {
  const uint8_t* src[4];
  int32_t sh[4], sw[4];
  int64_t pitch[4];
  int32_t rect[4][6];
  int32_t n_src, canvas_h, canvas_w;
  int32_t hsv, flipud, fliplr;
  double minv[6];
  uint8_t lut[3][256];
} dy_aug_sample;
int dy_aug_resize_u8(const uint8_t* src, int sh, int sw, int64_t src_pitch, uint8_t* dst, int dh, int dw, int64_t dst_pitch, void* stream);
int dy_aug_resize_area_u8(const uint8_t* src, int sh, int sw, int64_t src_pitch, uint8_t* dst, int dh, int dw, int64_t dst_pitch, void* stream);
int dy_aug_letterbox(const uint8_t* src, int sh, int sw, int64_t src_pitch, int new_h, int new_w, int top, int left, int out_h, int out_w,
                     uint8_t* out, void* stream);
int dy_aug_mosaic_warp(const dy_aug_sample* samples, int B, int out_h, int out_w, uint8_t* out, void* stream);
typedef struct dy_aug_mix_sample {
  dy_aug_sample a, b;
  double r, r1;
  int32_t mix;
} dy_aug_mix_sample;
int dy_aug_mosaic_warp_mix(const dy_aug_mix_sample* samples, int B, int out_h, int out_w, uint8_t* out, void* stream);
int dy_dark_channel_prior(const float* img, int B, int H, int W, float* A, float* ica, void* stream);


int dy_polymask_raster(const int16_t* polys, int n_total, int P, int h, int w, int ratio, uint8_t* planes, int32_t* area, void* stream);
int dy_polymask_compose(const uint8_t* planes, const int32_t* area, const int32_t* offsets, int B, int n_total, int mh, int mw,
                        const float* rows_in, float* rows_out, int32_t* perm, uint8_t* masks, void* stream);


typedef struct dy_seg_desc {
  const void* mc; int64_t mc_ld;
  const void* proto; int64_t proto_ld;
  int32_t B, A, nm, mh, mw;
  const int32_t* target_gt_idx;
  const uint8_t* fg_mask;
  const float* target_box;
  const void* masks;
  int32_t mask_dtype;
  int32_t mask_h, mask_w;
  int32_t overlap;
  const int32_t* gt_rows; int32_t n_max;
  float img_h, img_w;
  const int32_t* pos; const int32_t* npos;
  int32_t dtype;
} dy_seg_desc;
int dy_seg_positives(const uint8_t* fg_mask, int B, int A, int32_t* pos, int32_t* npos, void* stream);
int dy_seg_gt_rows(const float* batch_idx, int n_targets, int B, int n_max, int32_t* rows, void* stream);
int dy_seg_loss_fwd(const dy_seg_desc* d, float hyp_box, float* lossp, const float* det_out, float* out, void* stream);
int dy_seg_loss_bwd(const dy_seg_desc* d, const float* grad_out, float hyp_box, void* dmc, int64_t dmc_ld, void* dproto,
                    int64_t dproto_ld, void* stream);
int dy_bias_add(void* x, int64_t ld, const float* bias, int64_t pixels, int C, int dtype, void* stream);
#define DY_BIAS_GRAD_CHUNKS 2048
int dy_bias_grad(const void* dy, int64_t ld, int64_t pixels, int C, int dtype, float* scratch, int64_t scratch_elems, float* db,
                 void* stream);

int dy_seg_mask_decode(const void* proto, int64_t proto_ld, int nm, int mh, int mw, const float* det, int64_t det_ld,
                       const int32_t* det_img, int n, float sx, float sy, int dtype, uint8_t* out, void* stream);
int dy_seg_crop_mask(float* masks, const float* boxes, int n, int h, int w, void* stream);
int dy_seg_mask_iou(const uint8_t* pred, int n, const void* gt, int gt_dtype, int overlap, int m, int64_t hw, int32_t* work,
                    float* iou, void* stream);

int dy_seg_mask_upsample(const void* proto, int64_t proto_ld, int nm, int mh, int mw, int dtype, const float* det, int64_t det_ld,
                         const int32_t* img_off, const int32_t* img_ids, int n_groups, int max_group, int det_chunk, int crop_before,
                         float sx, float sy, int top, int left, int bottom, int right, int oh, int ow, int crop_after, uint8_t* out,
                         void* stream);
int dy_mask_resize(const void* src, int src_kind, int m, int h, int w, int top, int left, int bottom, int right, void* out, int out_f32,
                   int oh, int ow, void* stream);

#define DY_POSE_MAX_LEVELS 4
typedef struct dy_pose_desc {
  const void* kpt[DY_POSE_MAX_LEVELS];
  int64_t kpt_ld[DY_POSE_MAX_LEVELS];
  int32_t h[DY_POSE_MAX_LEVELS], w[DY_POSE_MAX_LEVELS];
  float stride[DY_POSE_MAX_LEVELS];
  int32_t n_levels, B, A, K, ndim, dtype;
  const int32_t* target_gt_idx;
  const uint8_t* fg_mask;
  const float* target_box;
  const float* keypoints;
  int32_t n_targets;
  const int32_t* gt_rows; int32_t n_max;
  float img_h, img_w;
  const float* sigma;
  const int32_t* pos; const int32_t* npos;
} dy_pose_desc;
int dy_pose_loss_fwd(const dy_pose_desc* d, float hyp_pose, float hyp_kobj, float* work, const float* det_out, float* out, void* stream);
int dy_pose_loss_bwd(const dy_pose_desc* d, const float* work, const float* grad_out, float hyp_pose, float hyp_kobj,
                     void* const* dkpt, int64_t dk_ld, void* stream);
int dy_pose_kpt_decode(const dy_pose_desc* d, int nc, float* y, void* stream);
int dy_kpt_oks(const float* gt, int N, const float* pred, int M, int pred_dim, const float* area, const float* sigma, int K, float eps,
               float* out, void* stream);

int dy_gap_fwd(const void* x, int64_t x_ld, int N, int HW, int C, int dtype, void* y, int64_t y_ld, void* stream);
int dy_gap_bwd(const void* dy, int64_t dy_ld, int N, int HW, int C, int dtype, void* dx, int64_t dx_ld, void* stream);
int dy_cls_xent_fwd(const void* logits, int64_t ld, int dtype, const int64_t* cls, int B, int nc, float* row_lse, float* loss, void* stream);
int dy_cls_xent_bwd(const void* logits, int64_t ld, int dtype, const int64_t* cls, const float* row_lse, const float* grad_out, int B,
                    int nc, void* dlogits, int64_t dld, void* stream);
int dy_cls_softmax(const void* logits, int64_t ld, int dtype, int B, int nc, float* probs, void* stream);
int dy_cls_topk(const void* scores, int64_t ld, int dtype, int B, int nc, int k, int32_t* idx, void* stream);
int dy_cls_metrics_update(const int32_t* idx, int k, const int64_t* cls, int B, int nc, int64_t* counts, int32_t* confusion, void* stream);

int dy_val_box_match(const float* det, int ld, const int* ocnt, int B, int max_det, const float* lcls, const float* lxywh,
                     const int* loff, int L, int H, int W, const float* rec, const float* iouv, int T, int single_cls, float conf_thres,
                     float iou_thres, int nc, uint8_t* correct, float* predn, float* tboxn, int32_t* confusion, void* workspace,
                     void* stream);
int dy_val_iou_match(const float* iou, int64_t iou_numel, const int64_t* moff, const float* det, int ld, const int* ocnt, int B,
                     int max_det, const float* lcls, const int* loff, int L, const float* iouv, int T, int single_cls, uint8_t* correct,
                     void* workspace, void* stream);

#ifdef __cplusplus
}
#endif
#endif
```

Measured before the change: 1007.

## Batch same-shape weight-gradient convs into grouped v4 wgrad launches on side stream

Adds a grouped wgrad entry point that packs up to 8 same-shape convolutions (different x/dz/grad pointers) into one v4 kernel launch plus one reduce launch, with member index derived from block id. Python side queues eligible wgrad calls by shape signature and flushes when full, aged out, or before gradient all-reduce/join. The aim is to fill the GPU better for small wgrad problems and cut launch count, at the cost of delaying wgrad work and extra host bookkeeping, plus possible scratch-capacity splits.

```diff
diff --git a/dedark_yolo_amd/_C.py b/dedark_yolo_amd/_C.py
--- a/dedark_yolo_amd/_C.py
+++ b/dedark_yolo_amd/_C.py
@@ -25,6 +25,13 @@
 class PackItem(C.Structure):
     _fields_ = [("w", vp), ("packed", vp), ("Cout", i32), ("Cout_pad", i32), ("Cin", i32), ("Cin_pad", i32), ("KH", i32),
                 ("KW", i32), ("transposed", i32), ("dtype", i32), ("first_block", i64)]
+
+
+WGRAD_GROUP_MAX = 8
+
+
+class WgradMember(C.Structure):
+    _fields_ = [("x", vp), ("x_ld", i64), ("dz", vp), ("dz_ld", i64), ("g_oihw", vp)]
 
 
 class DetMaps(C.Structure):
@@ -76,6 +83,11 @@
                         i32, vp],
     "dy_conv2d_wgrad_forked": [vp, vp, i64, i32, i32, i32, i32, vp, i64, i32, i32, i32, i32, i32, i32, i32, i32, i32, i32, vp, i64,
                                vp, i32, vp],
+    "dy_conv2d_wgrad_group": [C.POINTER(WgradMember), i32, i32, i32, i32, i32, i32, i32, i32, i32, i32, i32, i32, i32, i32, i32, vp, i64,
+                              i32, vp],
+    "dy_conv2d_wgrad_group_forked": [vp, C.POINTER(WgradMember), i32, i32, i32, i32, i32, i32, i32, i32, i32, i32, i32, i32, i32, i32,
+                                     i32, vp, i64, i32, vp],
+    "dy_conv2d_wgrad_groupable": [i64, i32, i32, i32, i32, i64, i32, i32, i32, i32, i32, i32, i32, i32, i32, i32, i64, i32],
     "dy_conv2d_bn_act_fwd": [C.POINTER(ConvDesc), i64, vp, vp, vp, vp, f32, f32, vp, i32, vp, i64, vp, i64, vp],
     "dy_bn_act_bwd": [vp, i64, vp, i64, vp, vp, i32, vp, vp, i64, vp, vp, i64, i32, i32, vp],
     "dy_conv2d_bn_act_fwd_valid": [C.POINTER(ConvDesc), i64, vp, vp, vp, vp, f32, f32, vp, i32, vp, i64, vp, i64, i32, vp],
diff --git a/dedark_yolo_amd/csrc/conv.hip b/dedark_yolo_amd/csrc/conv.hip
--- a/dedark_yolo_amd/csrc/conv.hip
+++ b/dedark_yolo_amd/csrc/conv.hip
@@ -1022,15 +1022,35 @@
 struct WgradRoute {
   bool (*eligible)(const DyWgradArgs& a);
   int (*launch)(const DyWgradArgs& a, void* stream);
+  int (*launch_group)(const DyWgradArgs* a, int n, void* stream);
 };
 
 const WgradRoute kWgradRoutes[] = {
-    {dy_dense_wgrad_eligible, dy_dense_wgrad_launch},
-    {dy_wgrad_v3_eligible, dy_wgrad_v3_launch},
-    {dy_wgrad_v4_eligible, dy_wgrad_v4_launch},
-    {dy_wgrad_v2_eligible, dy_wgrad_v2_launch},
-    {[](const DyWgradArgs&) { return true; }, wgrad_generic},
+    {dy_dense_wgrad_eligible, dy_dense_wgrad_launch, nullptr},
+    {dy_wgrad_v3_eligible, dy_wgrad_v3_launch, nullptr},
+    {dy_wgrad_v4_eligible, dy_wgrad_v4_launch, dy_wgrad_v4_launch_group},
+    {dy_wgrad_v2_eligible, dy_wgrad_v2_launch, nullptr},
+    {[](const DyWgradArgs&) { return true; }, wgrad_generic, nullptr},
 };
+
+const WgradRoute& wgrad_route_of(const DyWgradArgs& a) {
+  for (const WgradRoute& r : kWgradRoutes)
+    if (r.eligible(a)) return r;
+  return kWgradRoutes[sizeof(kWgradRoutes) / sizeof(kWgradRoutes[0]) - 1];
+}
+
+int check_wgrad_args(const DyWgradArgs& a) {
+  DY_CHECK(a.x && a.dz && a.scratch && a.g_oihw, "dy_conv2d_wgrad: null pointer");
+  DY_CHECK(a.dtype == DY_F32 || a.dtype == DY_BF16 || a.dtype == DY_F16, "dy_conv2d_wgrad: bad dtype");
+  const int ve = a.dtype == DY_F32 ? 4 : 8, es = a.dtype == DY_F32 ? 4 : 2;
+  DY_CHECK(a.Cin_pad % ve == 0 && a.Cout_pad % ve == 0, "dy_conv2d_wgrad: Cin=%d / Cout=%d must be multiples of %d", a.Cin_pad, a.Cout_pad, ve);
+  DY_CHECK(a.Cout > 0 && a.Cout <= a.Cout_pad && a.Cin > 0 && a.Cin <= a.Cin_pad, "dy_conv2d_wgrad: bad real channel counts");
+  DY_CHECK((a.x_ld * es) % 16 == 0 && (a.dz_ld * es) % 16 == 0, "dy_conv2d_wgrad: ld not 16-byte aligned");
+  DY_CHECK(((uintptr_t)a.x) % 16 == 0 && ((uintptr_t)a.dz) % 16 == 0, "dy_conv2d_wgrad: pointer not 16-byte aligned");
+  const int ho = (a.Hi + 2 * a.pad - a.dil * (a.KH - 1) - 1) / a.stride + 1, wo = (a.Wi + 2 * a.pad - a.dil * (a.KW - 1) - 1) / a.stride + 1;
+  DY_CHECK(ho == a.Ho && wo == a.Wo, "dy_conv2d_wgrad: dz %dx%d does not match conv output %dx%d", a.Ho, a.Wo, ho, wo);
+  return 0;
+}
 }
 
 int dy_wgrad_reduce_co_slabs(const float* part, int splits, const DyCoSlabs& L, int Cout, int Cin, float* g_oihw, void* stream) {
@@ -1043,20 +1063,38 @@
 extern "C" int dy_conv2d_wgrad(const void* x, int64_t x_ld, int N, int Hi, int Wi, int Cin_pad, const void* dz, int64_t dz_ld,
                                int Ho, int Wo, int Cout_pad, int KH, int KW, int stride, int pad, int dil, int Cout, int Cin,
                                float* scratch, int64_t scratch_elems, float* g_oihw, int dtype, void* stream) {
-  DY_CHECK(x && dz && scratch && g_oihw, "dy_conv2d_wgrad: null pointer");
-  DY_CHECK(dtype == DY_F32 || dtype == DY_BF16 || dtype == DY_F16, "dy_conv2d_wgrad: bad dtype");
-  const int ve = dtype == DY_F32 ? 4 : 8, es = dtype == DY_F32 ? 4 : 2;
-  DY_CHECK(Cin_pad % ve == 0 && Cout_pad % ve == 0, "dy_conv2d_wgrad: Cin=%d / Cout=%d must be multiples of %d", Cin_pad, Cout_pad, ve);
-  DY_CHECK(Cout > 0 && Cout <= Cout_pad && Cin > 0 && Cin <= Cin_pad, "dy_conv2d_wgrad: bad real channel counts");
-  DY_CHECK((x_ld * es) % 16 == 0 && (dz_ld * es) % 16 == 0, "dy_conv2d_wgrad: ld not 16-byte aligned");
-  DY_CHECK(((uintptr_t)x) % 16 == 0 && ((uintptr_t)dz) % 16 == 0, "dy_conv2d_wgrad: pointer not 16-byte aligned");
-  const int ho = (Hi + 2 * pad - dil * (KH - 1) - 1) / stride + 1, wo = (Wi + 2 * pad - dil * (KW - 1) - 1) / stride + 1;
-  DY_CHECK(ho == Ho && wo == Wo, "dy_conv2d_wgrad: dz %dx%d does not match conv output %dx%d", Ho, Wo, ho, wo);
   const DyWgradArgs a = {x, x_ld, N, Hi, Wi, Cin_pad, dz, dz_ld, Ho, Wo, Cout_pad, KH, KW, stride, pad, dil, Cout, Cin,
                          scratch, scratch_elems, g_oihw, dtype};
-  for (const WgradRoute& r : kWgradRoutes)
-    if (r.eligible(a)) return r.launch(a, stream);
+  if (int e = check_wgrad_args(a)) return e;
+  return wgrad_route_of(a).launch(a, stream);
+}
+
+extern "C" int dy_conv2d_wgrad_group(const dy_wgrad_member* members, int n, int N, int Hi, int Wi, int Cin_pad, int Ho, int Wo,
+                                     int Cout_pad, int KH, int KW, int stride, int pad, int dil, int Cout, int Cin, float* scratch,
+                                     int64_t scratch_elems, int dtype, void* stream) {
+  DY_CHECK(members && n >= 1 && n <= DY_WGRAD_GROUP_MAX, "dy_conv2d_wgrad_group: %d members (1..%d)", n, DY_WGRAD_GROUP_MAX);
+  DyWgradArgs a[DY_WGRAD_GROUP_MAX];
+  for (int i = 0; i < n; ++i) {
+    const dy_wgrad_member& m = members[i];
+    a[i] = {m.x, m.x_ld, N, Hi, Wi, Cin_pad, m.dz, m.dz_ld, Ho, Wo, Cout_pad, KH, KW, stride, pad, dil, Cout, Cin,
+            scratch, scratch_elems, m.g_oihw, dtype};
+    if (int e = check_wgrad_args(a[i])) return e;
+  }
+  const WgradRoute& r0 = wgrad_route_of(a[0]);
+  bool same = r0.launch_group != nullptr;
+  for (int i = 1; i < n && same; ++i) same = &wgrad_route_of(a[i]) == &r0;
+  if (same) return r0.launch_group(a, n, stream);
+  for (int i = 0; i < n; ++i)
+    if (int e = wgrad_route_of(a[i]).launch(a[i], stream)) return e;
   return 0;
+}
+
+extern "C" int dy_conv2d_wgrad_groupable(int64_t x_ld, int N, int Hi, int Wi, int Cin_pad, int64_t dz_ld, int Ho, int Wo, int Cout_pad,
+                                         int KH, int KW, int stride, int pad, int dil, int Cout, int Cin, int64_t scratch_elems,
+                                         int dtype) {
+  const DyWgradArgs a = {nullptr, x_ld, N, Hi, Wi, Cin_pad, nullptr, dz_ld, Ho, Wo, Cout_pad, KH, KW, stride, pad, dil, Cout, Cin,
+                         nullptr, scratch_elems, nullptr, dtype};
+  return wgrad_route_of(a).launch_group != nullptr ? 1 : 0;
 }
 
 extern "C" int dy_pack_weight(const float* w, void* packed, int Cout, int Cout_pad, int Cin, int Cin_pad, int KH, int KW,
@@ -1114,3 +1152,12 @@
   return dy_conv2d_wgrad(x, x_ld, N, Hi, Wi, Cin_pad, dz, dz_ld, Ho, Wo, Cout_pad, KH, KW, stride, pad, dil, Cout, Cin, scratch,
                          scratch_elems, g_oihw, dtype, stream);
 }
+
+extern "C" int dy_conv2d_wgrad_group_forked(void* wait_for, const dy_wgrad_member* members, int n, int N, int Hi, int Wi, int Cin_pad,
+                                            int Ho, int Wo, int Cout_pad, int KH, int KW, int stride, int pad, int dil, int Cout,
+                                            int Cin, float* scratch, int64_t scratch_elems, int dtype, void* stream) {
+  if (wait_for != stream)
+    if (int e = dy_stream_fork(wait_for, stream)) return e;
+  return dy_conv2d_wgrad_group(members, n, N, Hi, Wi, Cin_pad, Ho, Wo, Cout_pad, KH, KW, stride, pad, dil, Cout, Cin, scratch,
+                               scratch_elems, dtype, stream);
+}
diff --git a/dedark_yolo_amd/csrc/conv_route.h b/dedark_yolo_amd/csrc/conv_route.h
--- a/dedark_yolo_amd/csrc/conv_route.h
+++ b/dedark_yolo_amd/csrc/conv_route.h
@@ -172,13 +172,20 @@
 template <typename P> struct HasPointwise<P, std::void_t<decltype(std::declval<P&>().pointwise)>> : std::true_type {};
 
 template <typename P>
-inline void fill_wgrad_problem(P& p, const DyWgradArgs& a) {
-  p.x = (const char*)a.x; p.x_ld = a.x_ld; p.N = a.N; p.Hi = a.Hi; p.Wi = a.Wi; p.Cin = a.Cin_pad;
-  p.dz = (const char*)a.dz; p.dz_ld = a.dz_ld; p.Ho = a.Ho; p.Wo = a.Wo; p.Cout = a.Cout_pad;
+inline void fill_wgrad_shape(P& p, const DyWgradArgs& a) {
+  p.N = a.N; p.Hi = a.Hi; p.Wi = a.Wi; p.Cin = a.Cin_pad;
+  p.Ho = a.Ho; p.Wo = a.Wo; p.Cout = a.Cout_pad;
   p.KH = a.KH; p.KW = a.KW; p.stride = a.stride; p.pad = a.pad; p.dil = a.dil; p.part = a.scratch;
   p.M = (long)a.N * a.Ho * a.Wo;
   p.Ktot = a.KH * a.KW * a.Cin_pad;
   if constexpr (HasPointwise<P>::value) p.pointwise = (a.KH == 1 && a.KW == 1 && a.stride == 1 && a.pad == 0) ? 1 : 0;
+}
+
+template <typename P>
+inline void fill_wgrad_problem(P& p, const DyWgradArgs& a) {
+  p.x = (const char*)a.x; p.x_ld = a.x_ld;
+  p.dz = (const char*)a.dz; p.dz_ld = a.dz_ld;
+  fill_wgrad_shape(p, a);
 }
 
 struct WgradSplits {
@@ -214,5 +221,6 @@
 int dy_wgrad_v3_launch(const DyWgradArgs& a, void* stream);
 bool dy_wgrad_v4_eligible(const DyWgradArgs& a);
 int dy_wgrad_v4_launch(const DyWgradArgs& a, void* stream);
+int dy_wgrad_v4_launch_group(const DyWgradArgs* a, int n, void* stream);
 bool dy_wgrad_v2_eligible(const DyWgradArgs& a);
 int dy_wgrad_v2_launch(const DyWgradArgs& a, void* stream);
diff --git a/dedark_yolo_amd/csrc/wgrad_v4.hip b/dedark_yolo_amd/csrc/wgrad_v4.hip
--- a/dedark_yolo_amd/csrc/wgrad_v4.hip
+++ b/dedark_yolo_amd/csrc/wgrad_v4.hip
@@ -18,17 +18,23 @@
 typedef __attribute__((address_space(3))) s16x4* lds_s16x4_ptr;
 typedef __attribute__((ext_vector_type(8))) __bf16 bf16x8;
 
-struct P {
+constexpr int MAXG = DY_WGRAD_GROUP_MAX;
+
+struct Member {
   const char* x;
   const char* dz;
+  long x_ld, dz_ld;
   unsigned x_bytes, dz_bytes;
-  long x_ld, dz_ld;
+};
+
+struct P {
+  Member m[MAXG];
   int N, Hi, Wi, Cin;
   int Ho, Wo, Cout;
   int KH, KW, stride, pad, dil;
   float* part;
   long M;
-  int Ktot, tiles_q, tiles, nblk;
+  int Ktot, tiles_q, tiles, nblk, splits;
   long chunk;
   int q64_w, r64_w;
   int q_h, r_h;
@@ -43,7 +49,9 @@
   const int wave = __builtin_amdgcn_readfirstlane(tid >> 6);
   const int wr = wave >> 2, wc = wave & 3;
   const int bid = xcd_remap(blockIdx.x, p.nblk);
-  const int split = bid / p.tiles, tile = bid - split * p.tiles;
+  const int ms = bid / p.tiles, tile = bid - ms * p.tiles;
+  const int member = ms / p.splits, split = ms - member * p.splits;
+  const Member o = p.m[member];
   const int tile_p = tile / p.tiles_q, tile_q = tile - tile_p * p.tiles_q;
   const int kp0 = tile_p * BP, q0 = tile_q * BQ;
   const bool has_b1 = q0 + 128 < p.Cout;
@@ -52,7 +60,7 @@
   const long m_end = (m_begin + p.chunk < p.M) ? m_begin + p.chunk : p.M;
   const int nk = m_begin < m_end ? (int)((m_end - m_begin + BKP - 1) / BKP) : 0;
 
-  unsigned nrec_a = nk > 0 ? p.x_bytes : 0, nrec_b = nk > 0 ? p.dz_bytes : 0;
+  unsigned nrec_a = nk > 0 ? o.x_bytes : 0, nrec_b = nk > 0 ? o.dz_bytes : 0;
 
   const int lrow = lane >> 4, slot = lane & 15;
   const int chunk = slot ^ ((lrow << 2) | (wave & 3));
@@ -67,7 +75,7 @@
     const int kh = tap / p.KW, kw = tap - kh * p.KW;
     a_dh[u] = kh * p.dil - p.pad;
     a_dw[u] = kw * p.dil - p.pad;
-    a_tap[u] = (unsigned)(((long)a_dh[u] * p.Wi + a_dw[u]) * p.x_ld * 2 + ci * 2);
+    a_tap[u] = (unsigned)(((long)a_dh[u] * p.Wi + a_dw[u]) * o.x_ld * 2 + ci * 2);
     if (!kok) a_dh[u] = 0x40000000;
   }
   int ph[2], pw[2];
@@ -76,7 +84,7 @@
   for (int j = 0; j < 2; ++j) {
     const long m = m_begin + 4 * (wave + 8 * j) + lrow;
     if (POINTWISE) {
-      a_pix[j] = (unsigned)(m * p.x_ld * 2);
+      a_pix[j] = (unsigned)(m * o.x_ld * 2);
       ph[j] = pw[j] = 0;
     } else {
       const unsigned mu = (unsigned)m;
@@ -86,7 +94,7 @@
       const int oh = (int)(rem / (unsigned)p.Wo), ow = (int)(rem - (unsigned)oh * (unsigned)p.Wo);
       ph[j] = oh * p.stride;
       pw[j] = ow * p.stride;
-      a_pix[j] = (unsigned)((((long)pn * p.Hi + ph[j]) * p.Wi + pw[j]) * p.x_ld * 2);
+      a_pix[j] = (unsigned)((((long)pn * p.Hi + ph[j]) * p.Wi + pw[j]) * o.x_ld * 2);
     }
   }
   unsigned b_off[2][2];
@@ -95,25 +103,25 @@
     const int co = q0 + 128 * u + 8 * chunk;
 #pragma unroll
     for (int j = 0; j < 2; ++j)
-      b_off[u][j] = co < p.Cout ? (unsigned)((long)(4 * (wave + 8 * j) + lrow) * p.dz_ld * 2 + co * 2) : B_COL_OOB;
-  }
-  int b_koff = nk > 0 ? (int)(m_begin * p.dz_ld * 2) : 0;
+      b_off[u][j] = co < p.Cout ? (unsigned)((long)(4 * (wave + 8 * j) + lrow) * o.dz_ld * 2 + co * 2) : B_COL_OOB;
+  }
+  int b_koff = nk > 0 ? (int)(m_begin * o.dz_ld * 2) : 0;
   if (nk > 0) nrec_b -= (unsigned)b_koff;
   int sk = 0;
   auto advance_scalar = [&]() {
     ++sk;
-    b_koff += (int)(BKP * p.dz_ld * 2);
-    const unsigned step = (unsigned)(BKP * p.dz_ld * 2);
+    b_koff += (int)(BKP * o.dz_ld * 2);
+    const unsigned step = (unsigned)(BKP * o.dz_ld * 2);
     nrec_b = nrec_b > step ? nrec_b - step : 0;
     if (sk >= nk) { nrec_a = 0; nrec_b = 0; b_koff = 0; }
   };
-  const int e_w = p.stride * (int)p.x_ld * 2, e_h = p.stride * p.Wi * (int)p.x_ld * 2, e_n = p.Hi * p.Wi * (int)p.x_ld * 2;
+  const int e_w = p.stride * (int)o.x_ld * 2, e_h = p.stride * p.Wi * (int)o.x_ld * 2, e_n = p.Hi * p.Wi * (int)o.x_ld * 2;
   const int d_base = p.q_h * e_n + p.r_h * e_h + p.r64_w * e_w, d_cw = e_h - p.Wo * e_w, d_ch = e_n - p.Ho * e_h;
   const int s_rw = p.r64_w * p.stride, s_rh = p.r_h * p.stride, s_Wo = p.Wo * p.stride, s_Ho = p.Ho * p.stride;
   auto advance_rows = [&]() {
     if (POINTWISE) {
 #pragma unroll
-      for (int j = 0; j < 2; ++j) a_pix[j] += (unsigned)(BKP * p.x_ld * 2);
+      for (int j = 0; j < 2; ++j) a_pix[j] += (unsigned)(BKP * o.x_ld * 2);
       return;
     }
 #pragma unroll
@@ -146,14 +154,14 @@
     }
   };
   auto stage_a = [&](int buf, int u) {
-    const __amdgpu_buffer_rsrc_t rs = __builtin_amdgcn_make_buffer_rsrc((void*)p.x, 0, nrec_a, 0x00020000);
+    const __amdgpu_buffer_rsrc_t rs = __builtin_amdgcn_make_buffer_rsrc((void*)o.x, 0, nrec_a, 0x00020000);
 #pragma unroll
     for (int j = 0; j < 2; ++j)
       __builtin_amdgcn_raw_ptr_buffer_load_lds(rs, (lds_ptr_t)(smem + buf * BUF + (u ? OFF_A1 : OFF_A0) + (wave + 8 * j) * 1024), 16,
                                                (int)a_v[u][j], 0, 0, 0);
   };
   auto stage_b = [&](int buf, int u) {
-    const __amdgpu_buffer_rsrc_t rs = __builtin_amdgcn_make_buffer_rsrc((void*)(p.dz + b_koff), 0, nrec_b, 0x00020000);
+    const __amdgpu_buffer_rsrc_t rs = __builtin_amdgcn_make_buffer_rsrc((void*)(o.dz + b_koff), 0, nrec_b, 0x00020000);
 #pragma unroll
     for (int j = 0; j < 2; ++j)
       __builtin_amdgcn_raw_ptr_buffer_load_lds(rs, (lds_ptr_t)(smem + buf * BUF + (u ? OFF_B1 : OFF_B0) + (wave + 8 * j) * 1024), 16,
@@ -348,12 +356,18 @@
     }
 }
 
+struct Grads {
+  float* g[MAXG];
+};
+
 __global__ __launch_bounds__(256) void reduce_kernel(const float* __restrict__ part, int splits, int tiles, int tiles_q, int Cout, int Cin,
-                                                     int Cin_pad, int taps, float* __restrict__ g) {
+                                                     int Cin_pad, int taps, const Grads gs) {
   const int ci = blockIdx.x * 256 + threadIdx.x;
   const int co = blockIdx.y;
-  const int t = blockIdx.z;
+  const int member = blockIdx.z / taps, t = blockIdx.z - member * taps;
   if (ci >= Cin) return;
+  part += (long)member * splits * tiles * (BP * BQ);
+  float* __restrict__ g = gs.g[member];
   const int tq = co / BQ, cq = co - tq * BQ;
   const long sstride = (long)tiles * BP * BQ;
   const int k = t * Cin_pad + ci;
@@ -388,28 +402,37 @@
   return a.scratch_elems >= tp * tq * 65536L * 2;
 }
 
-int dy_wgrad_v4_launch(const DyWgradArgs& a, void* stream) {
-  using namespace wg4;
-  P p;
-  dy_route::fill_wgrad_problem(p, a);
-  p.x_bytes = (unsigned)((((long)a.N * a.Hi * a.Wi - 1) * a.x_ld + a.Cin_pad) * 2);
-  p.dz_bytes = (unsigned)(((p.M - 1) * a.dz_ld + a.Cout_pad) * 2);
-  p.tiles_q = dy_cdiv(a.Cout_pad, BQ);
+namespace wg4 {
+
+static int launch_members(const DyWgradArgs* a, int n, void* stream) {
+  P p = {};
+  dy_route::fill_wgrad_shape(p, a[0]);
+  for (int i = 0; i < n; ++i) {
+    Member& m = p.m[i];
+    m.x = (const char*)a[i].x; m.x_ld = a[i].x_ld;
+    m.dz = (const char*)a[i].dz; m.dz_ld = a[i].dz_ld;
+    m.x_bytes = (unsigned)((((long)a[i].N * a[i].Hi * a[i].Wi - 1) * a[i].x_ld + a[i].Cin_pad) * 2);
+    m.dz_bytes = (unsigned)(((p.M - 1) * a[i].dz_ld + a[i].Cout_pad) * 2);
+  }
+  const DyWgradArgs& s = a[0];
+  p.tiles_q = dy_cdiv(s.Cout_pad, BQ);
   p.tiles = dy_cdiv(p.Ktot, BP) * p.tiles_q;
-  const long fit = a.scratch_elems / ((long)p.tiles * BP * BQ);
-  const dy_route::WgradSplits plan = dy_route::plan_wgrad_splits(p.M, 256 / p.tiles, 8L * BKP, BKP, fit, dy_route::kNoGridCap);
+  const long fit = s.scratch_elems / ((long)p.tiles * BP * BQ * n);
+  const long want = 256 / ((long)p.tiles * n);
+  const dy_route::WgradSplits plan = dy_route::plan_wgrad_splits(p.M, want > 1 ? want : 1, 8L * BKP, BKP, fit, dy_route::kNoGridCap);
   p.chunk = plan.chunk;
-  p.nblk = (int)(plan.splits * p.tiles);
-  p.q64_w = BKP / a.Wo; p.r64_w = BKP % a.Wo;
-  p.q_h = p.q64_w / a.Ho; p.r_h = p.q64_w % a.Ho;
-  const bool pointwise = a.KH == 1 && a.KW == 1 && a.stride == 1 && a.pad == 0;
+  p.splits = (int)plan.splits;
+  p.nblk = (int)(plan.splits * p.tiles * n);
+  p.q64_w = BKP / s.Wo; p.r64_w = BKP % s.Wo;
+  p.q_h = p.q64_w / s.Ho; p.r_h = p.q64_w % s.Ho;
+  const bool pointwise = s.KH == 1 && s.KW == 1 && s.stride == 1 && s.pad == 0;
   constexpr int SHMEM = 2 * BUF;
   if (int e = dy_raise_lds_limit("wgrad_v4", {{&wgrad_kernel<false, bf16_t>, SHMEM}, {&wgrad_kernel<true, bf16_t>, SHMEM},
                                               {&wgrad_kernel<false, f16_t>, SHMEM}, {&wgrad_kernel<true, f16_t>, SHMEM}}))
     return e;
   hipStream_t st = (hipStream_t)stream;
   dy_note_kernel("wg4::wgrad_kernel+reduce_kernel");
-  if (int e = dy_dispatch_16bit("wgrad_v4", a.dtype, [&](auto tag) {
+  if (int e = dy_dispatch_16bit("wgrad_v4", s.dtype, [&](auto tag) {
         using T = typename decltype(tag)::type;
         if (pointwise) wgrad_kernel<true, T><<<p.nblk, 512, SHMEM, st>>>(p);
         else wgrad_kernel<false, T><<<p.nblk, 512, SHMEM, st>>>(p);
@@ -417,7 +440,31 @@
         return 0;
       }))
     return e;
-  reduce_kernel<<<dim3(dy_cdiv(a.Cin, 256), a.Cout, a.KH * a.KW), 256, 0, st>>>(a.scratch, (int)plan.splits, p.tiles, p.tiles_q, a.Cout, a.Cin, a.Cin_pad, a.KH * a.KW, a.g_oihw);
+  Grads gs = {};
+  for (int i = 0; i < n; ++i) gs.g[i] = a[i].g_oihw;
+  reduce_kernel<<<dim3(dy_cdiv(s.Cin, 256), s.Cout, s.KH * s.KW * n), 256, 0, st>>>(s.scratch, (int)plan.splits, p.tiles, p.tiles_q, s.Cout,
+                                                                                   s.Cin, s.Cin_pad, s.KH * s.KW, gs);
   DY_LAUNCH_CHECK();
   return 0;
 }
+
+}
+
+int dy_wgrad_v4_launch(const DyWgradArgs& a, void* stream) { return wg4::launch_members(&a, 1, stream); }
+
+int dy_wgrad_v4_launch_group(const DyWgradArgs* a, int n, void* stream) {
+  using namespace wg4;
+  const long tiles = (long)dy_cdiv(a[0].KH * a[0].KW * a[0].Cin_pad, BP) * dy_cdiv(a[0].Cout_pad, BQ);
+  long cap = 256 / tiles;
+  const long fit = a[0].scratch_elems / (tiles * BP * BQ);
+  if (cap > fit) cap = fit;
+  if (cap > MAXG) cap = MAXG;
+  if (cap < 1) cap = 1;
+  const int launches = (int)((n + cap - 1) / cap);
+  for (int l = 0, i = 0; l < launches; ++l) {
+    const int take = (n - i + (launches - l) - 1) / (launches - l);
+    if (int e = launch_members(a + i, take, stream)) return e;
+    i += take;
+  }
+  return 0;
+}
diff --git a/dedark_yolo_amd/engine/trainer.py b/dedark_yolo_amd/engine/trainer.py
--- a/dedark_yolo_amd/engine/trainer.py
+++ b/dedark_yolo_amd/engine/trainer.py
@@ -191,6 +191,7 @@
         b["left"] -= 1
         if b["left"] == 0:
             g = self.flat.g[b["start"]:b["end"]]
+            ops.wgrad_flush()
             side = ops.wgrad_side_stream() if ops.wgrad_pending() else None
             if side is None:
                 self.works.append(dist.all_reduce(g, op=dist.ReduceOp.SUM, async_op=True))
diff --git a/dedark_yolo_amd/ops.py b/dedark_yolo_amd/ops.py
--- a/dedark_yolo_amd/ops.py
+++ b/dedark_yolo_amd/ops.py
@@ -197,6 +197,8 @@
 
     def reset(self):
         self.main_raw = stream() if torch.cuda.is_available() else None
+        if _wg_side.queues:
+            wgrad_flush()
         self.retired.clear()
         if self.chunks > 1 and self.buf is not None:
             self.buf = torch.zeros(int(self.used * 1.25) + 1024, dtype=torch.float64, device=self.buf.device)
@@ -479,6 +481,11 @@
         self.groups = []
         self.free_events = []
         self.cb_queued = False
+        self.group_size = max(1, min(_C.WGRAD_GROUP_MAX, int(os.environ.get("DY_WGRAD_GROUP", "8"))))
+        self.age = max(1, int(os.environ.get("DY_WGRAD_GROUP_AGE", "6")))
+        self.queues = {}
+        self.tick = 0
+        self.groupable = {}
 
 
 _wg_side = _WgradSide()
@@ -520,12 +527,65 @@
         s.free_events.append(s.groups.pop(0)[0])
 
 
+def _wg_launch_group(sig, items):
+    s = _wg_side
+    st, dev, did, B, H, W, cin_pad, Ho, Wo, cout_pad, KH, KW, stride, pad, dil, Cout, Cin = sig
+    scratch = wgrad_scratch(dev, tag=s.raw)
+    for i in range(0, len(items), _C.WGRAD_GROUP_MAX):
+        part = items[i:i + _C.WGRAD_GROUP_MAX]
+        members = (_C.WgradMember * len(part))(*[(ptr(x), ld_of(x), ptr(dz), ld_of(dz), ptr(gw)) for x, dz, gw in part])
+        call("dy_conv2d_wgrad_group_forked", st, members, len(part), B, H, W, cin_pad, Ho, Wo, cout_pad, KH, KW, stride, pad, dil,
+             Cout, Cin, ptr(scratch), scratch.numel(), did, s.raw)
+        for x, dz, _ in part:
+            _wg_track(x, dz)
+
+
+def _wg_enqueue(sig, x, dz, gw):
+    s = _wg_side
+    s.tick += 1
+    q = s.queues.get(sig)
+    if q is None:
+        q = s.queues[sig] = [s.tick, []]
+    q[0] = s.tick
+    q[1].append((x, dz, gw))
+    if len(q[1]) >= s.group_size:
+        del s.queues[sig]
+        _wg_launch_group(sig, q[1])
+    _wg_flush_aged()
+
+
+def _wg_flush_aged():
+    s = _wg_side
+    if s.queues:
+        for k in [k for k, q in s.queues.items() if s.tick - q[0] >= s.age]:
+            _wg_launch_group(k, s.queues.pop(k)[1])
+
+
+def wgrad_flush():
+    s = _wg_side
+    while s.queues:
+        k = next(iter(s.queues))
+        _wg_launch_group(k, s.queues.pop(k)[1])
+
+
+def _wg_groupable(sig, x_ld, dz_ld, scratch_elems):
+    s = _wg_side
+    key = (sig, x_ld, dz_ld)
+    hit = s.groupable.get(key)
+    if hit is None:
+        st, dev, did, B, H, W, cin_pad, Ho, Wo, cout_pad, KH, KW, stride, pad, dil, Cout, Cin = sig
+        hit = s.groupable[key] = bool(_C.lib().dy_conv2d_wgrad_groupable(x_ld, B, H, W, cin_pad, dz_ld, Ho, Wo, cout_pad, KH, KW, stride, pad,
+                                                                         dil, Cout, Cin, scratch_elems, did))
+    return hit
+
+
 def wgrad_pending():
-    return bool(_wg_side.cur or _wg_side.groups)
+    return bool(_wg_side.cur or _wg_side.groups or _wg_side.queues)
 
 
 def wgrad_join():
     s = _wg_side
+    wgrad_flush()
     if s.cur or s.groups:
         call("dy_stream_fork", s.raw, stream())
         s.free_events.extend(g[0] for g in s.groups)
@@ -666,14 +726,24 @@
                     bytes=float((B * H * W * Cin + pixels * Cout) * x.element_size() + Cout * KH * KW * Cin * 4))
         wargs = (ptr(x), ld_of(x), B, H, W, cin_pad, ptr(dz), ld_of(dz), Ho, Wo, cout_pad, KH, KW, ctx.stride, ctx.pad, ctx.dil, Cout, Cin,
                  ptr(scratch), scratch.numel(), ptr(gw), did)
+        queued = False
         if side is not None and _C._prof is not None:
             with torch.cuda.stream(side):
                 call("dy_conv2d_wgrad", *wargs, st_w)
         elif side is not None:
-            call("dy_conv2d_wgrad_forked", st, *wargs, st_w)
+            if _wg_side.group_size > 1 and not any(st == b.cuda_stream for b in _branch["streams"]):
+                sig = (st, dev, did, B, H, W, cin_pad, Ho, Wo, cout_pad, KH, KW, ctx.stride, ctx.pad, ctx.dil, Cout, Cin)
+                if _wg_groupable(sig, ld_of(x), ld_of(dz), scratch.numel()):
+                    _wg_enqueue(sig, x, dz, gw)
+                    queued = True
+                else:
+                    _wg_side.tick += 1
+                    _wg_flush_aged()
+            if not queued:
+                call("dy_conv2d_wgrad_forked", st, *wargs, st_w)
         else:
             call("dy_conv2d_wgrad", *wargs, st_w)
-        if side is not None:
+        if side is not None and not queued:
             _wg_track(x, dz)
         if not direct:
             _add_pgrad(tape, ctx.owner, gw.view(ctx.owner.shape))
diff --git a/include/dedark_yolo.h b/include/dedark_yolo.h
--- a/include/dedark_yolo.h
+++ b/include/dedark_yolo.h
@@ -51,6 +51,19 @@
 int dy_conv2d_wgrad(const void* x, int64_t x_ld, int N, int Hi, int Wi, int Cin_pad, const void* dz, int64_t dz_ld, int Ho,
                     int Wo, int Cout_pad, int KH, int KW, int stride, int pad, int dil, int Cout, int Cin, float* scratch,
                     int64_t scratch_elems, float* g_oihw, int dtype, void* stream);
+#define DY_WGRAD_GROUP_MAX 8
+typedef struct {
+  const void* x;
+  int64_t x_ld;
+  const void* dz;
+  int64_t dz_ld;
+  float* g_oihw;
+} dy_wgrad_member;
+int dy_conv2d_wgrad_group(const dy_wgrad_member* members, int n, int N, int Hi, int Wi, int Cin_pad, int Ho, int Wo, int Cout_pad,
+                          int KH, int KW, int stride, int pad, int dil, int Cout, int Cin, float* scratch, int64_t scratch_elems,
+                          int dtype, void* stream);
+int dy_conv2d_wgrad_groupable(int64_t x_ld, int N, int Hi, int Wi, int Cin_pad, int64_t dz_ld, int Ho, int Wo, int Cout_pad, int KH,
+                              int KW, int stride, int pad, int dil, int Cout, int Cin, int64_t scratch_elems, int dtype);
 int dy_pack_weight(const float* w_oihw, void* packed, int Cout, int Cout_pad, int Cin, int Cin_pad, int KH, int KW,
                    int transposed, int dtype, void* stream);
 typedef struct {
@@ -273,6 +286,9 @@
 int dy_conv2d_wgrad_forked(void* wait_for, const void* x, int64_t x_ld, int N, int Hi, int Wi, int Cin_pad, const void* dz,
                            int64_t dz_ld, int Ho, int Wo, int Cout_pad, int KH, int KW, int stride, int pad, int dil, int Cout,
                            int Cin, float* scratch, int64_t scratch_elems, float* g_oihw, int dtype, void* stream);
+int dy_conv2d_wgrad_group_forked(void* wait_for, const dy_wgrad_member* members, int n, int N, int Hi, int Wi, int Cin_pad, int Ho,
+                                 int Wo, int Cout_pad, int KH, int KW, int stride, int pad, int dil, int Cout, int Cin, float* scratch,
+                                 int64_t scratch_elems, int dtype, void* stream);
 
 int dy_stream_fork(void* from, void* to);
 int dy_frontend_init(void);
```

Measured after the change: 1015, median of 6. About the same (+0.8%).
